# ini/multigrid

Hardware: AMD Instinct MI355X
Metric: agent-steps/sec (higher is better)
Workload: dtype u8

## Files before the change

### include/mgx.h

```cpp
#ifndef MGX_H
#define MGX_H

#if !defined(__HIPCC_RTC__)
#include <stddef.h>
#include <stdint.h>
#endif

#ifdef __cplusplus
extern "C" {
#endif

#define MGX_ABI_VERSION 11

enum {
    MGX_OK = 0,
    MGX_ERR_INVALID_ARGUMENT = -1,
    MGX_ERR_UNKNOWN_ACTION = -2,
    MGX_ERR_UNSUPPORTED = -3,
    MGX_ERR_LAUNCH = -4
};

enum { MGX_KIND_EMPTY = 0, MGX_KIND_BLOCKEDUNLOCKPICKUP = 1, MGX_KIND_REDBLUEDOORS = 2, MGX_KIND_LOCKEDHALLWAY = 3,
       MGX_KIND_RULES = 4 };

// ... 107 lines not shown
                          uint8_t *obs, uint8_t *dir, double *reward, uint8_t *terminated, uint8_t *truncated,
                          int32_t *err, void *stream);

enum { MGX_GEN_EMPTY_FIXED = 0, MGX_GEN_EMPTY_RANDOM = 1, MGX_GEN_BLOCKEDUNLOCKPICKUP = 2, MGX_GEN_REDBLUEDOORS = 3,
       MGX_GEN_LOCKEDHALLWAY = 4, MGX_GEN_PLAYGROUND = 5 };

typedef struct MgxGenStage {
    MgxCell *grid;
    uint8_t *agents;
    uint8_t *aux;
    uint64_t *words;
    int32_t *tag;
    int32_t phase;
    int32_t lead;
    int32_t external;
    int32_t candidates;
} MgxGenStage;

typedef struct MgxLayoutGen {
    int32_t kind;
    int32_t room_size;
    int32_t start_x, start_y, start_dir;
    int32_t max_hallway_keys;
    int32_t max_keys_per_room;
    const MgxCell *blank;
    uint64_t *gen_state;
    MgxGenStage stage;
} MgxLayoutGen;

int mgx_reset_generate(const MgxSpec *spec, int64_t batch, const MgxLayoutGen *gen, MgxCell *grid, uint8_t *agents,
                       uint64_t *rng, int32_t *step_count, uint8_t *aux, int32_t *episode, uint8_t *was_reset, void *stream);

typedef struct MgxResetSelect {
    const uint8_t  *select;
    const uint64_t *rng_words;
} MgxResetSelect;

int mgx_reset_select(const MgxSpec *spec, int64_t batch, const MgxResetSelect *sel, const MgxAutoReset *pool, MgxCell *grid,
                     uint8_t *agents, uint64_t *rng, int32_t *step_count, uint8_t *aux, void *stream);
int mgx_reset_generate_select(const MgxSpec *spec, int64_t batch, const MgxResetSelect *sel, const MgxLayoutGen *gen, MgxCell *grid,
                              uint8_t *agents, uint64_t *rng, int32_t *step_count, uint8_t *aux, int32_t *episode,
                              uint8_t *was_reset, void *stream);

int mgx_stage_generate(const MgxSpec *spec, int64_t batch, const MgxLayoutGen *gen, const uint64_t *rng, const int32_t *episode,
                       void *stream);

int mgx_step_generate(const MgxSpec *spec, int64_t batch, const MgxLayoutGen *gen, MgxCell *grid, uint8_t *agents,
                      uint64_t *rng, int32_t *step_count, const int8_t *actions, uint8_t *aux,
                      uint8_t *obs, uint8_t *dir, double *reward, uint8_t *terminated, uint8_t *truncated,
                      int32_t *err, int32_t *episode, uint8_t *was_reset, void *stream);

int mgx_gen_obs_one_hot(const MgxSpec *spec, int64_t batch, const MgxCell *grid, const uint8_t *agents,
                        uint8_t *obs_one_hot, uint8_t *dir, void *stream);
int mgx_step_one_hot(const MgxSpec *spec, int64_t batch, const MgxAutoReset *ar, MgxCell *grid, uint8_t *agents,
                     uint64_t *rng, int32_t *step_count, const int8_t *actions, uint8_t *aux,
                     uint8_t *obs_one_hot, uint8_t *dir, double *reward, uint8_t *terminated, uint8_t *truncated,
                     int32_t *err, void *stream);

typedef struct MgxStepArgs {
    MgxCell *grid;
    uint8_t *agents;
    uint64_t *rng;
    int32_t *step_count;
    uint8_t *aux;
    const int8_t *actions;
    const uint8_t *hook_order;
    uint8_t *obs;
    uint8_t *dir;
    double *reward;
    uint8_t *terminated;
    uint8_t *truncated;
    int32_t *err;
    int32_t steps;
    int32_t one_hot;
    const MgxAutoReset *auto_reset;
    const MgxLayoutGen *generate;
    int32_t *episode;
    uint8_t *was_reset;
    int32_t *grid_bad;
} MgxStepArgs;

int mgx_step_ex(const MgxSpec *spec, int64_t batch, const MgxStepArgs *args, void *stream);

int mgx_step_chains(const MgxSpec *spec, int64_t batch, const MgxStepArgs *args, int32_t parts, void *const *streams,
                    void *fork_event);
int mgx_sub_shards(const MgxSpec *spec, int64_t batch, const MgxStepArgs *args, int32_t *parts);

#define MGX_SHAPE_RUNTIME_COMPILED 100
typedef struct MgxShapeKey {
    int32_t width, height, num_agents, envs_per_wavefront, hooks, view_size, dma, stream;
    int32_t kernel_args_bytes;
    int32_t built_in;
    int32_t registered;
} MgxShapeKey;
int mgx_shape_key(const MgxSpec *spec, int64_t batch, MgxShapeKey *key);
int mgx_shape_register(const MgxShapeKey *key, const void *code_object, size_t bytes);

#define MGX_PERSIST_CTRL_WORDS 8
typedef struct MgxPersistent {
    const uint64_t *action_granules;
    uint32_t *done;
    uint32_t *ctrl;
    int32_t max_steps;
    int32_t timeout_ms;
} MgxPersistent;

int mgx_persistent_waves(const MgxSpec *spec, int64_t batch, const MgxStepArgs *args, int32_t *waves);
int mgx_step_persistent(const MgxSpec *spec, int64_t batch, const MgxStepArgs *args, const MgxPersistent *p, void *stream);
int mgx_persistent_post(const MgxSpec *spec, int64_t batch, const int8_t *actions, uint32_t step, uint64_t *action_granules,
                        void *stream);
int mgx_persistent_wait(const uint32_t *done, int32_t waves, uint32_t step, uint32_t *ctrl, int32_t timeout_ms, void *stream);
int mgx_persistent_feed(const MgxSpec *spec, int64_t batch, const int8_t *actions, int32_t steps, const MgxPersistent *p,
                        int32_t waves, uint64_t *trace, void *stream);

int mgx_render_atlas(int32_t tile_size, uint8_t *atlas, void *stream);
int mgx_render(const MgxSpec *spec, int64_t n, const MgxCell *grid, const uint8_t *agents, const uint8_t *obs, const uint8_t *atlas,
               int32_t tile_size, uint8_t *frames, void *stream);

#ifdef __cplusplus
}
#endif
#endif
```

### multigrid_amd/_lib.py

```python
from __future__ import annotations

import ctypes as C
import os

from .spec import MgxSpecC

HERE = os.path.dirname(os.path.abspath(__file__))
PRODUCT_LIB_PATH = os.path.join(HERE, "lib", "libmgx.so")
LIB_PATH = os.environ.get("MGX_LIBMGX") or PRODUCT_LIB_PATH


def is_product_lib() -> bool:
    return os.path.realpath(LIB_PATH) == os.path.realpath(PRODUCT_LIB_PATH)

ABI_VERSION = 11
OK, ERR_INVALID_ARGUMENT, ERR_UNKNOWN_ACTION, ERR_UNSUPPORTED, ERR_LAUNCH = 0, -1, -2, -3, -4

EXPORTS = ("mgx_abi_version", "mgx_error_string", "mgx_last_hip_error", "mgx_gen_obs", "mgx_step",
           "mgx_launch_info", "mgx_one_hot", "mgx_full_obs", "mgx_reset_done", "mgx_rollout", "mgx_step_autoreset",
           "mgx_rollout_autoreset", "mgx_gen_obs_one_hot", "mgx_step_one_hot",
           "mgx_reset_generate", "mgx_step_generate", "mgx_pack_grid", "mgx_unpack_grid",
           "mgx_step_ex", "mgx_step_chains", "mgx_sub_shards",
           "mgx_pack_grid_env", "mgx_check_grid", "mgx_pack_grid8_env", "mgx_unpack_grid8", "mgx_shape_key", "mgx_shape_register", "mgx_stage_generate",
           "mgx_persistent_waves", "mgx_step_persistent", "mgx_persistent_post", "mgx_persistent_wait", "mgx_persistent_feed",
           "mgx_rollout_info", "mgx_render_atlas", "mgx_render", "mgx_reset_select", "mgx_reset_generate_select")


class MgxLaunchInfo(C.Structure):
    _fields_ = [(n, C.c_int32) for n in ("envs_per_wavefront", "envs_per_workgroup", "threads_per_workgroup", "workgroups",
                                          "lds_bytes", "slots_per_group", "fixed_shape")]


class MgxRolloutInfo(C.Structure):
    _fields_ = [(n, C.c_int32) for n in ("envs_per_slice", "slices", "wavefronts", "threads_per_workgroup", "workgroups", "lds_bytes",
                                          "resident_shape")]


class MgxAutoReset(C.Structure):
    _fields_ = [("first_env", C.c_int64), ("pool_size", C.c_int32), ("pool_grid", C.c_void_p),
                ("pool_agents", C.c_void_p), ("pool_aux", C.c_void_p), ("episode", C.c_void_p), ("was_reset", C.c_void_p)]


class MgxResetSelect(C.Structure):
    _fields_ = [("select", C.c_void_p), ("rng_words", C.c_void_p)]


class MgxGenStage(C.Structure):
    _fields_ = [("grid", C.c_void_p), ("agents", C.c_void_p), ("aux", C.c_void_p), ("words", C.c_void_p), ("tag", C.c_void_p),
                ("phase", C.c_int32), ("lead", C.c_int32), ("external", C.c_int32), ("candidates", C.c_int32)]


class MgxLayoutGen(C.Structure):
    _fields_ = [("kind", C.c_int32), ("room_size", C.c_int32), ("start_x", C.c_int32), ("start_y", C.c_int32),
                ("start_dir", C.c_int32), ("max_hallway_keys", C.c_int32), ("max_keys_per_room", C.c_int32),
                ("blank", C.c_void_p), ("gen_state", C.c_void_p), ("stage", MgxGenStage)]


class MgxStepArgs(C.Structure):
    _fields_ = [("grid", C.c_void_p), ("agents", C.c_void_p), ("rng", C.c_void_p), ("step_count", C.c_void_p),
                ("aux", C.c_void_p), ("actions", C.c_void_p), ("hook_order", C.c_void_p),
                ("obs", C.c_void_p), ("dir", C.c_void_p), ("reward", C.c_void_p), ("terminated", C.c_void_p),
                ("truncated", C.c_void_p), ("err", C.c_void_p),
                ("steps", C.c_int32), ("one_hot", C.c_int32),
                ("auto_reset", C.POINTER(MgxAutoReset)), ("generate", C.POINTER(MgxLayoutGen)),
                ("episode", C.c_void_p), ("was_reset", C.c_void_p), ("grid_bad", C.c_void_p)]


class MgxPersistent(C.Structure):
    _fields_ = [("action_granules", C.c_void_p), ("done", C.c_void_p), ("ctrl", C.c_void_p), ("max_steps", C.c_int32),
                ("timeout_ms", C.c_int32)]


PERSIST_CTRL_WORDS = 8

GEN_KINDS = {"empty_fixed": 0, "empty_random": 1, "blockedunlockpickup": 2, "redbluedoors": 3, "lockedhallway": 4, "playground": 5}


class MgxError(RuntimeError):
    def __init__(self, code: int, what: str):
        self.code = code
        super().__init__(f"{what}: {error_string(code)} (code {code}, hip error {lib().mgx_last_hip_error()})")


_lib = None


def lib() -> C.CDLL:
    global _lib
    if _lib is not None:
        return _lib
    if not os.path.exists(LIB_PATH):
        raise ImportError(
            f"{LIB_PATH} is missing: the HIP extension has not been built. Run `python -m multigrid_amd.build` "
            "(or __graft_entry__.build()). multigrid_amd has no CPU fallback.")
    L = C.CDLL(LIB_PATH)
    vp, i64 = C.c_void_p, C.c_int64
    L.mgx_abi_version.restype = C.c_int
    L.mgx_error_string.restype = C.c_char_p
    L.mgx_error_string.argtypes = [C.c_int]
    L.mgx_last_hip_error.restype = C.c_int
    L.mgx_gen_obs.restype = C.c_int
    L.mgx_gen_obs.argtypes = [C.POINTER(MgxSpecC), i64, vp, vp, vp, vp, vp]
    L.mgx_step.restype = C.c_int
    L.mgx_step.argtypes = [C.POINTER(MgxSpecC), i64] + [vp] * 13
    L.mgx_rollout.restype = C.c_int
    L.mgx_rollout.argtypes = [C.POINTER(MgxSpecC), i64, C.c_int32] + [vp] * 13
    L.mgx_step_autoreset.restype = C.c_int
    L.mgx_step_autoreset.argtypes = [C.POINTER(MgxSpecC), i64, C.POINTER(MgxAutoReset)] + [vp] * 13
    L.mgx_rollout_autoreset.restype = C.c_int
    L.mgx_rollout_autoreset.argtypes = [C.POINTER(MgxSpecC), i64, C.c_int32, C.POINTER(MgxAutoReset)] + [vp] * 13
    L.mgx_gen_obs_one_hot.restype = C.c_int
    L.mgx_gen_obs_one_hot.argtypes = [C.POINTER(MgxSpecC), i64, vp, vp, vp, vp, vp]
    L.mgx_step_one_hot.restype = C.c_int
    L.mgx_step_one_hot.argtypes = [C.POINTER(MgxSpecC), i64, C.POINTER(MgxAutoReset)] + [vp] * 13
    L.mgx_one_hot.restype = C.c_int
    L.mgx_one_hot.argtypes = [vp, i64, C.POINTER(C.c_int32), vp, vp]
    L.mgx_full_obs.restype = C.c_int
    L.mgx_full_obs.argtypes = [C.POINTER(MgxSpecC), i64, vp, vp, vp, vp]
    L.mgx_reset_done.restype = C.c_int
    L.mgx_reset_done.argtypes = [C.POINTER(MgxSpecC), i64, i64, C.c_int32] + [vp] * 10
    L.mgx_reset_generate.restype = C.c_int
    L.mgx_reset_generate.argtypes = [C.POINTER(MgxSpecC), i64, C.POINTER(MgxLayoutGen)] + [vp] * 8
    L.mgx_reset_select.restype = C.c_int
    L.mgx_reset_select.argtypes = [C.POINTER(MgxSpecC), i64, C.POINTER(MgxResetSelect), C.POINTER(MgxAutoReset)] + [vp] * 6
    L.mgx_reset_generate_select.restype = C.c_int
    L.mgx_reset_generate_select.argtypes = [C.POINTER(MgxSpecC), i64, C.POINTER(MgxResetSelect), C.POINTER(MgxLayoutGen)] + [vp] * 8
    L.mgx_stage_generate.restype = C.c_int
    L.mgx_stage_generate.argtypes = [C.POINTER(MgxSpecC), i64, C.POINTER(MgxLayoutGen), vp, vp, vp]
    L.mgx_step_generate.restype = C.c_int
    L.mgx_step_generate.argtypes = [C.POINTER(MgxSpecC), i64, C.POINTER(MgxLayoutGen)] + [vp] * 15
    L.mgx_pack_grid.restype = C.c_int
    L.mgx_pack_grid.argtypes = [vp, i64, vp, vp, vp]
    L.mgx_unpack_grid.restype = C.c_int
    L.mgx_unpack_grid.argtypes = [vp, i64, vp, vp]
    L.mgx_pack_grid_env.restype = C.c_int
    L.mgx_pack_grid_env.argtypes = [vp, i64, C.c_int32, C.c_int32, vp, vp, vp]
    L.mgx_pack_grid8_env.restype = C.c_int
    L.mgx_pack_grid8_env.argtypes = [vp, i64, C.c_int32, C.c_int32, vp, vp, vp]
    L.mgx_unpack_grid8.restype = C.c_int
    L.mgx_unpack_grid8.argtypes = [vp, i64, vp, vp]
    L.mgx_check_grid.restype = C.c_int
    L.mgx_check_grid.argtypes = [C.POINTER(MgxSpecC), i64, vp, vp, vp, vp]
    L.mgx_launch_info.restype = C.c_int
    L.mgx_launch_info.argtypes = [C.POINTER(MgxSpecC), i64, C.POINTER(MgxLaunchInfo)]
    L.mgx_step_ex.restype = C.c_int
    L.mgx_step_ex.argtypes = [C.POINTER(MgxSpecC), i64, C.POINTER(MgxStepArgs), vp]
    L.mgx_step_chains.restype = C.c_int
    L.mgx_step_chains.argtypes = [C.POINTER(MgxSpecC), i64, C.POINTER(MgxStepArgs), C.c_int32, C.POINTER(vp), vp]
    L.mgx_sub_shards.restype = C.c_int
    L.mgx_sub_shards.argtypes = [C.POINTER(MgxSpecC), i64, C.POINTER(MgxStepArgs), C.POINTER(C.c_int32)]
    L.mgx_persistent_waves.restype = C.c_int
    L.mgx_persistent_waves.argtypes = [C.POINTER(MgxSpecC), i64, C.POINTER(MgxStepArgs), C.POINTER(C.c_int32)]
    L.mgx_step_persistent.restype = C.c_int
    L.mgx_step_persistent.argtypes = [C.POINTER(MgxSpecC), i64, C.POINTER(MgxStepArgs), C.POINTER(MgxPersistent), vp]
    L.mgx_persistent_post.restype = C.c_int
    L.mgx_persistent_post.argtypes = [C.POINTER(MgxSpecC), i64, vp, C.c_uint32, vp, vp]
    L.mgx_persistent_wait.restype = C.c_int
    L.mgx_persistent_wait.argtypes = [vp, C.c_int32, C.c_uint32, vp, C.c_int32, vp]
    L.mgx_persistent_feed.restype = C.c_int
    L.mgx_persistent_feed.argtypes = [C.POINTER(MgxSpecC), i64, vp, C.c_int32, C.POINTER(MgxPersistent), C.c_int32, vp, vp]
    L.mgx_render_atlas.restype = C.c_int
    L.mgx_render_atlas.argtypes = [C.c_int32, vp, vp]
    L.mgx_render.restype = C.c_int
    L.mgx_render.argtypes = [C.POINTER(MgxSpecC), i64, vp, vp, vp, vp, C.c_int32, vp, vp]
    if L.mgx_abi_version() != ABI_VERSION:
        raise ImportError(f"{LIB_PATH}: ABI version {L.mgx_abi_version()} != {ABI_VERSION}; rebuild it")
    _lib = L
    return L


def error_string(code: int) -> str:
    return lib().mgx_error_string(code).decode()


def check(code: int, what: str):
    if code != OK:
        raise MgxError(code, what)


def launch_info(spec, batch: int, roll: bool = False, persistent: bool = False) -> dict:
    sc = spec.to_c()
    if roll or persistent:
        ri = MgxRolloutInfo()
        L = lib()
        L.mgx_rollout_info.restype = C.c_int
        L.mgx_rollout_info.argtypes = [C.POINTER(MgxSpecC), C.c_int64, C.c_int32, C.POINTER(MgxRolloutInfo)]
        check(L.mgx_rollout_info(C.byref(sc), batch, int(bool(persistent)), C.byref(ri)), "mgx_rollout_info")
        out = {n: getattr(ri, n) for n, _ in MgxRolloutInfo._fields_}
        out["envs_per_wavefront"] = ri.envs_per_slice * ri.slices
        return out
    info = MgxLaunchInfo()
    check(lib().mgx_launch_info(C.byref(sc), batch, C.byref(info)), "mgx_launch_info")
    return {n: getattr(info, n) for n, _ in MgxLaunchInfo._fields_}
```

### multigrid_amd/batched.py

```python
from __future__ import annotations

import os

import numpy as np
import torch

from . import _lib, layouts, rng as rnglib
from .constants import NO_ACTION, Action, Type
from .spec import EnvSpec

INT32_MAX = 2 ** 31 - 1


class StepGraph:

    def __init__(self, env, graph, sub_shards, keep):
        self.env, self.graph, self.sub_shards = env, graph, sub_shards
        self._version = env._layout_version
        self._keep = keep

    def replay(self):
        if self.env._layout_version != self._version:
            raise RuntimeError("this graph was captured before set_layout_pool() / set_layout_generator() replaced the layout "
                               "tensors it holds pointers to: capture_steps() again")
        self.graph.replay()


class PersistentSession:

    def __init__(self, env, max_steps: int, auto_reset: bool, timeout_ms: int):
        be = env.backend
        if not hasattr(be, "persistent_launch"):
            raise RuntimeError("persistent stepping needs the HIP backend")
        if auto_reset and getattr(env, "_gen", None) is not None:
            raise RuntimeError("persistent stepping restarts finished envs from a layout pool (set_layout_pool), not from the "
                               "device generator")
        self.env, self.max_steps, self.timeout_ms = env, int(max_steps), int(timeout_ms)
        self.auto_reset = bool(auto_reset)
        B, A, dev = env.batch, env.spec.num_agents, env.device
        self.waves = be.persistent_waves(B, self.auto_reset)
        self.granules = torch.zeros((B, (A + 3) // 4), dtype=torch.int64, device=dev)
        self.done = torch.zeros((self.waves,), dtype=torch.int32, device=dev)
        self.ctrl = torch.tensor([0, 0, 0, -1] + [0] * 4, dtype=torch.int32, device=dev)
        self.stream = torch.cuda.Stream(dev, priority=-1)
        self.t = 0
        self.waited = 0
        self.open = False
        ar = env._auto_reset_args(self.auto_reset, getattr(env, "was_reset", None))
        self._sa, self._keep = be.step_args(env.cells, env.agents, env.rng, env.step_count,
                                            env.aux if env.spec.env_kind != "empty" else None, env.err, env.obs, env.dir,
                                            env.reward, env.terminated, env.truncated, auto_reset=ar)
        self._pers = be.persistent_struct(self.granules, self.done, self.ctrl, self.max_steps, self.timeout_ms)

    def __enter__(self):
        env = self.env
        env._need_state()
        env.join()
        if env._session is not None:
            raise RuntimeError("this env already has a persistent session open")
        cur = torch.cuda.current_stream(env.device)
        self.stream.wait_stream(cur)
        env.backend.persistent_launch(env.batch, self._sa, self._pers, self.stream.cuda_stream)
        env._session = self
        self.open = True
        return self

    def post(self, actions: torch.Tensor):
        env = self.env
        if not self.open or self.t >= self.max_steps:
            raise RuntimeError("the persistent session is closed or has used up its max_steps")
        if actions.dtype is not torch.int8 or actions.shape != env._act_shape or actions.device != env.cells.device \
                or not actions.is_contiguous():
            raise ValueError(f"actions must be a contiguous int8 tensor of shape {tuple(env._act_shape)} on {env.cells.device}")
        self.t += 1
        env.backend.persistent_post(env.batch, actions, self.t, self.granules)

    def wait(self):
        self.env.backend.persistent_wait(self.done, self.waves, self.t, self.ctrl, self.timeout_ms)
        self.waited = self.t
        env = self.env
        return env.obs, env.dir, env.reward, env.terminated, env.truncated

    def step(self, actions: torch.Tensor):
        self.post(actions)
        return self.wait()

    def feed(self, actions: torch.Tensor, trace: bool = False):
        env = self.env
        T = int(actions.shape[0])
        if self.t != 0 or T != self.max_steps:
            raise RuntimeError("feed() plays a whole session: max_steps == len(actions), nothing posted before")
        if actions.dtype is not torch.int8 or tuple(actions.shape[1:]) != tuple(env._act_shape) or not actions.is_contiguous():
            raise ValueError("actions must be a contiguous int8 tensor [T,B,A]")
        tr = torch.zeros((2 * T + 1,), dtype=torch.int64, device=env.device) if trace else None
        env.backend.persistent_feed(env.batch, actions, T, self._pers, self.waves, tr, torch.cuda.current_stream(env.device).cuda_stream)
        self.t = self.waited = T
        return tr

    def close(self):
        if not self.open:
            return
        env = self.env
        cur = torch.cuda.current_stream(env.device)
        if self.t < self.max_steps:
            if self.waited < self.t:
                self.wait()
            self.ctrl[0:1].fill_(1)
        cur.wait_stream(self.stream)
        self.open = False
        env._session = None
        c = [int(v) & 0xFFFFFFFF for v in self.ctrl.cpu()]
        self.timeouts, self.waves_left, self.steps_completed = c[1], c[2], c[3]
        if c[1]:
            raise RuntimeError(f"persistent stepping: {c[1]} wait(s) timed out after {self.timeout_ms} ms "
                               f"(steps completed by every wavefront: {c[3]})")

    def __exit__(self, *exc):
        try:
            self.close()
        except RuntimeError:
            if exc[0] is None:
                raise
        return False

    def __del__(self):
        try:
            if getattr(self, "open", False):
                self.ctrl[0:1].fill_(1)
        except Exception:
            pass


class BatchedMultiGridEnv:
    def __init__(self, spec: EnvSpec, batch: int, device="cuda", *, first_env: int = 0, backend=None, specialise=None):
        self.spec = spec
        self.batch = int(batch)
        self.first_env = int(first_env)
        self.device = torch.device(device)
        if backend is None:
            from .ops import HipBackend
            backend = HipBackend(spec, self.device)
        self.backend = backend
        B, A, dev = self.batch, spec.num_agents, self.device
        self.cells = torch.zeros(spec.cells_shape(B), dtype=torch.uint8 if spec.cell_bytes != 2 else torch.int16, device=dev)
        self.agents = torch.zeros(spec.agents_shape(B), dtype=torch.uint8, device=dev)
        self.rng = torch.zeros((B, 4), dtype=torch.int64, device=dev)
        self.step_count = torch.zeros((B,), dtype=torch.int32, device=dev)
        self.aux = torch.zeros((B, 16), dtype=torch.uint8, device=dev)
        obs_shape = tuple(spec.obs_shape(B))
        parts = (("reward", torch.float64, (B, A)), ("obs", torch.uint8, obs_shape), ("dir", torch.uint8, (B, A)),
                 ("terminated", torch.uint8, (B, A)), ("truncated", torch.uint8, (B,)), ("err", torch.int32, (2,)))
        offs, total = {}, 0
        for name, dt, shape in parts:
            offs[name] = total
            total += (int(np.prod(shape)) * torch.empty((), dtype=dt).element_size() + 15) & ~15
        self._out = torch.zeros(max(total, 16), dtype=torch.uint8, device=dev)
        self._out_parts, self._out_host = [(n, dt, sh, offs[n]) for n, dt, sh in parts], None
        for name, dt, shape in parts:
            nbytes = int(np.prod(shape)) * torch.empty((), dtype=dt).element_size()
            setattr(self, name, self._out[offs[name]:offs[name] + nbytes].view(dt).view(shape))
        self.err.copy_(torch.tensor([0, INT32_MAX], dtype=torch.int32))
        self._loaded = False
        self._seeded = False
        self._act_shape = torch.Size((B, A))
        self._bound = {}
        self._layout_version = 0
        self._parent = None
        self._chain_streams = []
        self._chains_pending, self._chains_P = False, 1
        self._session = None
        self.shape_kernel = None
        if specialise is None:
            specialise = os.environ.get("MGX_JIT", "0") not in ("", "0")
        if specialise and self.device.type == "cuda" and getattr(self.backend, "name", "") == "hip":
            self.specialise()

    def specialise(self) -> str:
        from . import jit
        self.shape_kernel = jit.ensure_shape(self.spec, self.batch, self.device)
        return self.shape_kernel

    @property
    def grid(self) -> torch.Tensor:
        if self.spec.cell_bytes == 3:
            return self.cells
        c = self.cells.to(torch.int32)
        if self.spec.cell_bytes == 1:
            tc = c & 0xF
            door = (tc == 11) | (tc == 12)
            t = torch.where(tc <= 10, tc, torch.where(door, torch.full_like(tc, 4), torch.full_like(tc, 10)))
            st = torch.where(tc <= 10, torch.zeros_like(tc), torch.where(door, tc - 10, tc - 12))
            return torch.stack((t, (c >> 4) & 0x7, st), dim=-1).to(torch.uint8)
        content = ((c >> 4) & 0xF) | (((c >> 11) & 1) << 4) | (((c >> 14) & 1) << 5)
        return torch.stack((c & 0xF, (c >> 8) & 0x7, ((c >> 12) & 0x3) | (content << 2)), dim=-1).to(torch.uint8)

    def load_state(self, grid, agents, rng=None, aux=None, step_count=None, validate: bool = True, target=None):
        self._no_session("load_state")
        sp, B = self.spec, self.batch

        def prep(x, shape, dtype):
            t = torch.as_tensor(np.asarray(x) if not torch.is_tensor(x) else x)
            if t.dim() == len(shape) - 1:
                t = t.unsqueeze(0).expand(shape)
            if tuple(t.shape) != tuple(shape):
                raise ValueError(f"expected shape {tuple(shape)}, got {tuple(t.shape)}")
            return t.to(dtype=dtype).contiguous()

        self.join()
        g = prep(grid, sp.grid_shape(B), torch.uint8)
        a = prep(agents, sp.agents_shape(B), torch.uint8)
        if validate:
            layouts.check_walled(g.cpu().numpy() if g.device.type != "cpu" else g.numpy())
            an = a.cpu().numpy()
            if (an[..., 2] >= sp.width).any() or (an[..., 3] >= sp.height).any() or (an[..., 1] > 3).any():
                raise ValueError("agent position / direction out of range")
        self._refuse_carried_contents(a)
        self.cells.copy_(torch.from_numpy(layouts.pack_cells_for(sp, g.cpu().numpy())))
        self.agents.copy_(a)
        if rng is not None:
            r = np.asarray(rng.cpu() if torch.is_tensor(rng) else rng)
            if r.dtype == np.uint64:
                r = r.view(np.int64)
            self.rng.copy_(prep(r, (B, 4), torch.int64))
            self._seeded = True
        if aux is None and target is not None:
            t = np.zeros(np.asarray(target).shape[:-1] + (16,), dtype=np.uint8)
            t[..., :min(4, np.asarray(target).shape[-1])] = np.asarray(target)[..., :4]
            aux = t
        if aux is not None:
            self.aux.copy_(prep(aux, (B, 16), torch.uint8))
        elif self.spec.env_kind != "empty":
            raise ValueError(f"env_kind {self.spec.env_kind!r} needs `aux` (the env's hook state, include/mgx.h)")
        if step_count is None:
            self.step_count.zero_()
        else:
            self.step_count.copy_(prep(step_count, (B,), torch.int32))
        self._reset_err()
        self._state_written()
        self._loaded = True

    def _refuse_carried_contents(self, agent_rows):
        if self.spec.cell_bytes == 1:
            rows = agent_rows.cpu().numpy() if torch.is_tensor(agent_rows) else np.asarray(agent_rows)
            if (rows[..., 7] >> 2).any():
                raise ValueError("compact cells (cell_bytes = 1) cannot hold a box's content: an agent carries a filled box; "
                                 "use cell_bytes = 2 for envs with Box(contains=...)")

    def seed(self, seed: int):
        self._no_session("seed")
        self.join()
        idx = self.first_env + np.arange(self.batch)
        self.rng.copy_(torch.from_numpy(rnglib.words_from_seed_and_index(seed, idx).view(np.int64)))
        self._seeded = True
        self._state_written()

    def seed_synthetic(self, seed: int):
        self._no_session("seed_synthetic")
        self.join()
        words = rnglib.synthetic_words(self.batch, seed, self.first_env)
        self.rng.copy_(torch.from_numpy(words.view(np.int64)))
        self._seeded = True
        self._state_written()

    def _reset_err(self):
        self.err.copy_(torch.tensor([0, INT32_MAX], dtype=torch.int32))

    def _state_written(self):
        st = (getattr(self, "_gen", None) or {}).get("stage")
        if st is not None and st.get("candidates"):
            st["tag"].fill_(-1)
        elif st is not None:
            st["tag"][:, 0] = -1
            st["tag"][:, 3] = 0

    def gen_obs(self, one_hot: bool = False):
        self._need_state()
        self.join()
        if one_hot:
            if self.spec.cell_bytes == 1:
                self.backend.gen_obs(self.batch, self.cells, self.agents, self.obs, self.dir)
                self.backend.one_hot(self.obs, self._one_hot_buffer())
                return self._one_hot, self.dir
            self._need_wide_cells("one-hot output")
            self.backend.gen_obs(self.batch, self.cells, self.agents, self._one_hot_buffer(), self.dir, one_hot=True)
            return self._one_hot, self.dir
        self.backend.gen_obs(self.batch, self.cells, self.agents, self.obs, self.dir)
        return self.obs, self.dir

    def _one_hot_buffer(self):
        if getattr(self, "_one_hot", None) is None:
            self._one_hot = torch.zeros(tuple(self.obs.shape[:-1]) + (21,), dtype=torch.uint8, device=self.device)
        return self._one_hot

    def _auto_reset_args(self, auto_reset, was_reset):
        if not auto_reset:
            return None
        if getattr(self, "_pool", None) is None:
            raise RuntimeError("auto_reset needs set_layout_pool() first")
        return (self.first_env, self._pool, self.episode, was_reset)

    def step(self, actions: torch.Tensor, auto_reset: bool = False, one_hot: bool = False, hook_order=None, sub_shards=1):
        if not self._loaded or self._session is not None:
            self._need_state()
        if self._parent is not None:
            self._check_fresh()
        if actions.dtype is not torch.int8 or actions.shape != self._act_shape or actions.device != self.cells.device \
                or not actions.is_contiguous():
            raise ValueError(f"actions must be a contiguous int8 tensor of shape {tuple(self._act_shape)} "
                             f"on {self.cells.device}")
        if sub_shards == 1 and hook_order is None and not self._chains_pending:
            fast = self._bound.get((auto_reset, one_hot))
            if fast is not None:
                fast[0](actions)
                return fast[1]
        if hook_order is not None and (hook_order.dtype is not torch.uint8 or hook_order.shape != self._act_shape
                                       or hook_order.device != self.cells.device or not hook_order.is_contiguous()):
            raise ValueError(f"hook_order must be a contiguous uint8 tensor of shape {tuple(self._act_shape)} on {self.cells.device}")
        if one_hot and not (self.spec.cell_bytes == 1 and self.spec.env_kind == "empty"):
            self._need_wide_cells("one-hot output")
        generate = bool(auto_reset) and getattr(self, "_gen", None) is not None
        if generate:
            auto_reset = False
        P = 1
        if sub_shards != 1:
            P = self.sub_shards_hint(auto_reset or generate, one_hot, form="eager") if sub_shards == "auto" else int(sub_shards)
            P = max(1, min(P, self.batch // self.SUB_SHARD_ALIGN))
        if self._chains_pending and P != self._chains_P:
            self.join()
        key = (bool(auto_reset), bool(one_hot), generate, P)
        if one_hot:
            self._one_hot_buffer()
        fast = self._bound.get(key)
        if fast is None:
            fast = self._bind_step(*key)
        out = (self._one_hot if one_hot else self.obs), self.dir, self.reward, self.terminated, self.truncated
        if fast is not False:
            if P > 1:
                ev = self._fork_event
                ev.record(torch.cuda.current_stream(self.device))
                fast(actions, ev.cuda_event, hook_order)
                for st in self._chain_streams[:P]:
                    actions.record_stream(st)
                    if hook_order is not None:
                        hook_order.record_stream(st)
                self._chains_pending, self._chains_P = True, P
                return out
            if isinstance(auto_reset, bool) and isinstance(one_hot, bool):
                self._bound[(auto_reset or generate, one_hot)] = (fast, out)
            fast(actions, hook_order)
            return out
        sp = self.spec
        ar = self._auto_reset_args(auto_reset, getattr(self, "was_reset", None))
        kw = {}
        if ar is not None:
            kw["auto_reset"] = ar
        if one_hot:
            kw["one_hot"] = True
        if hook_order is not None:
            kw["hook_order"] = hook_order
        obs = self._one_hot_buffer() if one_hot else self.obs
        self.backend.step(self.batch, self.cells, self.agents, self.rng, self.step_count, actions,
                          self.aux if sp.env_kind != "empty" else None, self.err,
                          obs, self.dir, self.reward, self.terminated, self.truncated, **kw)
        if generate:
            self.reset_done()
        return obs, self.dir, self.reward, self.terminated, self.truncated

    def join(self):
        if self._chains_pending:
            cur = torch.cuda.current_stream(self.device)
            for st in self._chain_streams:
                cur.wait_stream(st)
            self._chains_pending = False

    def sub_shards_hint(self, auto_reset: bool = False, one_hot: bool = False, form: str = "graph") -> int:
        if form not in ("graph", "eager"):
            raise ValueError("form must be 'graph' or 'eager'")
        if form == "eager":
            return 1
        hint = getattr(self.backend, "sub_shards", None)
        if hint is None:
            return 1
        generate = bool(auto_reset) and getattr(self, "_gen", None) is not None
        return hint(self.batch, bool(auto_reset), bool(one_hot), generate)

    def _bind_step(self, auto_reset: bool, one_hot: bool, generate: bool = False, parts: int = 1):
        key = (auto_reset, one_hot, generate, parts)
        bind = getattr(self.backend, "bind_step" if parts == 1 else "bind_chains", None)
        if bind is None:
            self._bound[key] = False
            return False
        ar = self._auto_reset_args(auto_reset, getattr(self, "was_reset", None))
        head = (self.batch,)
        if parts > 1:
            while len(self._chain_streams) < parts:
                self._chain_streams.append(torch.cuda.Stream(self.device))
            if getattr(self, "_fork_event", None) is None:
                self._fork_event = torch.cuda.Event()
                self._fork_event.record(torch.cuda.current_stream(self.device))
            head = (self.batch, parts, self._chain_streams[:parts])
        f = bind(*head, self.cells, self.agents, self.rng, self.step_count,
                 self.aux if self.spec.env_kind != "empty" else None, self.err,
                 self._one_hot_buffer() if one_hot else self.obs, self.dir, self.reward, self.terminated, self.truncated,
                 auto_reset=ar, one_hot=one_hot,
                 **({"generate": (self._gen, self.episode, self.was_reset)} if generate else {}))
        self._bound[key] = f
        return f

    def _check_fresh(self):
        if self._parent is not None and self._parent._layout_version != self._made_version:
            raise RuntimeError("this sub-shard was split off before its parent's set_layout_pool() / set_layout_generator() "
                               "replaced the layout tensors: split() / capture_steps() again")

    SUB_SHARD_ALIGN = 64

    def split(self, parts: int) -> list:
        self._need_state()
        self.join()
        B, al = self.batch, self.SUB_SHARD_ALIGN
        parts = max(1, min(int(parts), max(1, B // al)))
        cuts = [0] + [min(B, ((B * i // parts + al - 1) // al) * al) for i in range(1, parts)] + [B]
        out = []
        for lo, hi in zip(cuts[:-1], cuts[1:]):
            if hi <= lo:
                continue
            c = object.__new__(BatchedMultiGridEnv)
            c.spec, c.batch, c.first_env, c.device, c.backend = self.spec, hi - lo, self.first_env + lo, self.device, self.backend
            for name in ("cells", "agents", "rng", "step_count", "aux", "obs", "dir", "reward", "terminated", "truncated"):
                setattr(c, name, getattr(self, name)[lo:hi])
            c.err = self.err
            c._loaded, c._act_shape, c._bound = True, torch.Size((hi - lo, self.spec.num_agents)), {}
            c._parent, c._made_version, c._layout_version = self, self._layout_version, 0
            c._chain_streams, c._chains_pending, c._chains_P, c._session = [], False, 1, None
            c._seeded = self._seeded
            c._one_hot = self._one_hot[lo:hi] if getattr(self, "_one_hot", None) is not None else None
            c._pool = getattr(self, "_pool", None)
            c._gen = None
            if getattr(self, "_gen", None) is not None:
                c._gen = dict(self._gen, gen_state=self._gen["gen_state"][lo:hi])
                if self._gen.get("stage") is not None:
                    st = self._gen["stage"]
                    c._gen["stage"] = {k: (v[lo:hi] if torch.is_tensor(v) else v) for k, v in st.items()}
                    if st.get("external") and st.get("stream") is not None:
                        c._gen["stage"]["stream"] = torch.cuda.Stream(self.device)
                    c._gen["stage"]["phase"] = [st["phase"][0]]
            if getattr(self, "episode", None) is not None:
                c.episode, c.was_reset = self.episode[lo:hi], self.was_reset[lo:hi]
            c._range = (lo, hi)
            out.append(c)
        return out

    def capture_steps(self, actions: torch.Tensor, auto_reset: bool = False, one_hot: bool = False, sub_shards=1,
                      hook_order=None):
        self._need_state()
        self.join()
        if sub_shards == "auto":
            sub_shards = self.sub_shards_hint(auto_reset, one_hot)
        stream = torch.cuda.current_stream(self.device)
        graph = torch.cuda.CUDAGraph()
        side = torch.cuda.Stream(self.device)
        side.wait_stream(stream)
        if one_hot:
            self._one_hot_buffer()
        shards = self.split(sub_shards) if sub_shards > 1 else [self]
        others = [torch.cuda.Stream(self.device) for _ in shards[1:]]
        with torch.cuda.stream(side):
            with torch.cuda.graph(graph, stream=side):
                for s in others:
                    s.wait_stream(side)
                for i, sh in enumerate(shards):
                    lo, hi = getattr(sh, "_range", (0, self.batch))
                    with torch.cuda.stream(side if i == 0 else others[i - 1]):
                        st = (getattr(sh, "_gen", None) or {}).get("stage") if auto_reset else None
                        before = st.get("launches", 0) if st else 0
                        for t in range(actions.shape[0]):
                            ho = None if hook_order is None else (hook_order[t] if sh is self else hook_order[t, lo:hi])
                            sh.step(actions[t] if sh is self else actions[t, lo:hi], auto_reset=auto_reset, one_hot=one_hot,
                                    hook_order=ho)
                        if st and st.get("candidates") and st.get("launches", 0) == before:
                            sh.backend.stage_generate(sh.batch, sh._gen, sh.rng, sh.episode)
                for i, sh in enumerate(shards):
                    gs = ((getattr(sh, "_gen", None) or {}).get("stage") or {}).get("stream")
                    if gs is not None:
                        (side if i == 0 else others[i - 1]).wait_stream(gs)
                for s in others:
                    side.wait_stream(s)
        stream.wait_stream(side)
        return StepGraph(self, graph, len(shards), (shards, others, actions, hook_order))

    def rollout(self, actions: torch.Tensor, out: dict | None = None, auto_reset: bool = False, one_hot: bool = False) -> dict:
        self._need_state()
        generate = bool(auto_reset) and getattr(self, "_gen", None) is not None
        if not (self.spec.cell_bytes == 1 and self.spec.env_kind == "empty" and not one_hot and not generate):
            self._need_wide_cells("rollout (the steps of one launch)")
        self.join()
        sp, B = self.spec, self.batch
        if actions.dtype != torch.int8 or actions.dim() != 3 or tuple(actions.shape[1:]) != (B, sp.num_agents) \
                or actions.device != self.cells.device or not actions.is_contiguous():
            raise ValueError(f"actions must be a contiguous int8 tensor of shape (T, {B}, {sp.num_agents}) on {self.cells.device}")
        T, A, v, dev = actions.shape[0], sp.num_agents, sp.view_size, self.device
        if out is None:
            out = {"obs": torch.empty((T, B, A, v, v, 21 if one_hot else 3), dtype=torch.uint8, device=dev),
                   "dir": torch.empty((T, B, A), dtype=torch.uint8, device=dev),
                   "reward": torch.empty((T, B, A), dtype=torch.float64, device=dev),
                   "terminated": torch.empty((T, B, A), dtype=torch.uint8, device=dev),
                   "truncated": torch.empty((T, B), dtype=torch.uint8, device=dev)}
        if auto_reset and "was_reset" not in out:
            out["was_reset"] = torch.empty((T, B), dtype=torch.uint8, device=dev)
        generate = bool(auto_reset) and getattr(self, "_gen", None) is not None
        if generate:
            self.backend.rollout(B, T, self.cells, self.agents, self.rng, self.step_count, actions,
                                 self.aux if sp.env_kind != "empty" else None, self.err, out["obs"], out["dir"],
                                 out["reward"], out["terminated"], out["truncated"],
                                 generate=(self._gen, self.episode, out["was_reset"]), **({"one_hot": True} if one_hot else {}))
            return out
        ar = self._auto_reset_args(auto_reset, out.get("was_reset"))
        self.backend.rollout(B, T, self.cells, self.agents, self.rng, self.step_count, actions,
                             self.aux if sp.env_kind != "empty" else None, self.err, out["obs"], out["dir"],
                             out["reward"], out["terminated"], out["truncated"],
                             **({"auto_reset": ar} if ar is not None else {}), **({"one_hot": True} if one_hot else {}))
        return out

    def one_hot_obs(self) -> torch.Tensor:
        self.join()
        self.backend.one_hot(self.obs, self._one_hot_buffer())
        return self._one_hot

    def full_obs(self) -> torch.Tensor:
        self._need_state()
        self.join()
        if getattr(self, "_full", None) is None:
            self._full = torch.zeros((self.batch, self.spec.width, self.spec.height, 3), dtype=torch.uint8,
                                     device=self.device)
        try:
            self.backend.full_obs(self.batch, self.cells, self.agents, self._full)
        except _lib.MgxError as e:
            if e.code != _lib.ERR_UNSUPPORTED:
                raise
            img = self.grid.permute(0, 2, 1, 3) & torch.tensor([255, 255, 3], dtype=torch.uint8, device=self.device)
            ag = self.agents.long()
            env = torch.arange(self.batch, device=self.device)
            for a in range(self.spec.num_agents):
                img[env, ag[:, a, 2], ag[:, a, 3]] = torch.stack(
                    (torch.full_like(ag[:, a, 0], int(Type.agent)), ag[:, a, 0], ag[:, a, 1]), dim=-1).to(torch.uint8)
            self._full.copy_(img)
        return self._full

    def render(self, env_ids=None, tile_size: int = 32, highlight: bool = True, out: torch.Tensor | None = None) -> torch.Tensor:
        self._no_session("render")
        self._need_state()
        self.join()
        ts = int(tile_size)
        if not 1 <= ts <= 64:
            raise ValueError(f"render: tile_size must be in 1..64, got {tile_size}")
        cells, agents = self.cells, self.agents
        if env_ids is not None:
            ids = torch.as_tensor(env_ids)
            if ids.dtype.is_floating_point or ids.dtype.is_complex or ids.dtype == torch.bool:
                raise TypeError(f"render: env_ids must be an integer tensor, got {ids.dtype}")
            if ids.dim() != 1:
                raise ValueError(f"render: env_ids must be one-dimensional, got shape {tuple(ids.shape)}")
            if ids.numel():
                lo, hi = (int(v) for v in torch.stack((ids.min(), ids.max())).tolist())
                if lo < 0 or hi >= self.batch:
                    raise ValueError(f"render: env_ids must lie in [0, {self.batch}), got {lo}..{hi}")
            ids = ids.to(device=self.device, dtype=torch.long)
            cells, agents = cells.index_select(0, ids), agents.index_select(0, ids)
        n, sp = cells.shape[0], self.spec
        shape = (n, sp.height * ts, sp.width * ts, 3)
        if out is None:
            out = torch.empty(shape, dtype=torch.uint8, device=self.device)
        elif (tuple(out.shape) != shape or out.dtype != torch.uint8 or out.device != self.device or not out.is_contiguous()):
            raise ValueError(f"render: out must be a contiguous uint8 tensor of shape {shape} on {self.device}")
        if n == 0:
            return out
        obs = None
        if highlight:
            scratch = getattr(self, "_render_scratch", None)
            if scratch is None or scratch[0].shape[0] < n:
                scratch = (torch.empty((n,) + tuple(self.obs.shape[1:]), dtype=torch.uint8, device=self.device),
                           torch.empty((n, sp.num_agents), dtype=torch.uint8, device=self.device))
                self._render_scratch = scratch
            obs, dirs = scratch[0][:n], scratch[1][:n]
            self.backend.gen_obs(n, cells, agents, obs, dirs)
        self.backend.render(n, cells, agents, obs, ts, out)
        return out

    def set_layout_pool(self, grids, agents, auxs=None):
        self._no_session("set_layout_pool")
        sp = self.spec
        g = torch.as_tensor(np.asarray(grids), dtype=torch.uint8)
        a = torch.as_tensor(np.asarray(agents), dtype=torch.uint8)
        K = g.shape[0]
        if tuple(g.shape) != (K, sp.height, sp.width, 3) or tuple(a.shape) != (K, sp.num_agents, 8) or K < 1:
            raise ValueError("layout pool has the wrong shape")
        layouts.check_walled(g.numpy())
        self._refuse_carried_contents(a)
        t = None
        if auxs is not None:
            t = torch.as_tensor(np.asarray(auxs), dtype=torch.uint8)
            if tuple(t.shape) != (K, 16):
                raise ValueError("layout pool aux must be u8[K,16]")
            t = t.to(self.device).contiguous()
        elif sp.env_kind != "empty":
            raise ValueError(f"env_kind {sp.env_kind!r} needs per-layout aux")
        self.join()
        cells = torch.from_numpy(layouts.pack_cells_for(sp, g.numpy()))
        old = getattr(self, "_pool", None)
        if (getattr(self, "_gen", None) is None and old is not None and old[0].shape == cells.shape and old[1].shape == a.shape
                and (old[2] is None) == (t is None)):
            old[0].copy_(cells); old[1].copy_(a)
            if t is not None:
                old[2].copy_(t)
            self.episode.zero_(); self.was_reset.zero_()
            return
        self._gen = None
        self._pool = (cells.to(self.device).contiguous(), a.to(self.device).contiguous(), t)
        self.episode = torch.zeros((self.batch,), dtype=torch.int32, device=self.device)
        self.was_reset = torch.zeros((self.batch,), dtype=torch.uint8, device=self.device)
        self._bound.clear()
        self._layout_version += 1

    def set_layout_generator(self, kind: str, layout_seed: int = 0, *, room_size: int = 0, start=(1, 1, 0),
                             max_hallway_keys: int = 1, max_keys_per_room: int = 2, staged=True, lead: int | None = None):
        self._no_session("set_layout_generator")
        sp = self.spec
        self._need_wide_cells("set_layout_generator (device-side episode generation)")
        if kind == "blockedunlockpickup":
            if sp.env_kind != "blockedunlockpickup" or (sp.width, sp.height) != (2 * room_size - 1, room_size):
                raise ValueError("blockedunlockpickup generator: the spec must be a BlockedUnlockPickup grid of (2*room_size-1) x room_size")
            blank = layouts.roomgrid_blank(room_size, 1, 2)
        elif kind == "redbluedoors":
            if sp.env_kind != "redbluedoors" or sp.width != 2 * sp.height:
                raise ValueError("redbluedoors generator: the spec must be a RedBlueDoors grid of (2*size) x size")
            blank = layouts.redbluedoors_blank(sp.height)
        elif kind == "lockedhallway":
            rs = int(room_size)
            if sp.env_kind != "lockedhallway" or rs < 4 or sp.width != 3 * (rs - 1) + 1 or (sp.height - 1) % (rs - 1):
                raise ValueError("lockedhallway generator: the spec must be 3 columns of `room_size` rooms")
            blank = layouts.lockedhallway_blank(2 * ((sp.height - 1) // (rs - 1)), rs)
        elif kind == "playground":
            rs = int(room_size)
            if sp.env_kind != "empty" or rs < 4 or (sp.width - 1) % (rs - 1) or (sp.height - 1) % (rs - 1):
                raise ValueError("playground generator: the spec must be a hook-free grid of `room_size` rooms")
            blank = layouts.roomgrid_blank(rs, (sp.height - 1) // (rs - 1), (sp.width - 1) // (rs - 1))
        elif kind in ("empty_fixed", "empty_random"):
            if sp.env_kind != "empty" or sp.width != sp.height:
                raise ValueError("empty generator: the spec must be a square Empty grid")
            blank = layouts.empty_blank(sp.width)
        else:
            raise ValueError(f"unknown layout generator {kind!r}")
        self.join()
        idx = self.first_env + np.arange(self.batch)
        self._gen = {"kind": kind, "room_size": int(room_size), "start": tuple(int(v) for v in start),
                     "max_hallway_keys": int(max_hallway_keys), "max_keys_per_room": int(max_keys_per_room),
                     "blank": torch.from_numpy(layouts.pack_cells(blank).view(np.int16)).to(self.device).contiguous(),
                     "gen_state": torch.from_numpy(rnglib.layout_gen_state(layout_seed, idx).view(np.int64)).to(self.device)}
        cand = {"blockedunlockpickup": int(room_size) - 2, "redbluedoors": 1, "lockedhallway": 1, "empty_fixed": 1,
                "empty_random": 1}.get(kind, 0)
        if staged is True:
            staged = "candidates" if 1 <= cand <= 4 else "between"
        if staged not in (False, "candidates", "between", "side", "in_launch"):
            raise ValueError(f"staged must be True / 'candidates' / 'between' / 'side' / 'in_launch' / False, got {staged!r}")
        if staged == "candidates" and not 1 <= cand <= 4:
            raise ValueError(f"staged='candidates': the {kind!r} generator draws from env.np_random more than once (or has more than "
                             f"4 possible draws): use 'between'")
        if staged == "candidates" and sp.num_agents > 1:
            B, dev = self.batch, self.device
            lead = int(lead) if lead is not None else max(4, min(512, 2 * sp.max_steps // 3))
            lead = max(2, min(lead, sp.max_steps - 1))
            self._gen["stage"] = {"lead": lead, "external": 2, "stream": None, "candidates": cand,
                                  "grid": torch.zeros((B, cand, sp.height, sp.width), dtype=torch.int16, device=dev),
                                  "agents": torch.zeros((B, cand, sp.num_agents, 8), dtype=torch.uint8, device=dev),
                                  "aux": torch.zeros((B, cand, 16), dtype=torch.uint8, device=dev) if sp.env_kind != "empty" else None,
                                  "words": torch.zeros((B, cand, 6), dtype=torch.int64, device=dev),
                                  "tag": torch.full((B, 4), -1, dtype=torch.int32, device=dev), "phase": [0]}
        elif staged and sp.num_agents > 1:
            B, dev = self.batch, self.device
            tag = torch.zeros((B, 4), dtype=torch.int32, device=dev)
            tag[:, 0] = -1
            side = staged in ("side", "between")
            lead = int(lead) if lead is not None else (max(2, min(128, sp.max_steps // 4)) if side else 2)
            if not 2 <= lead < sp.max_steps or (side and lead < 4):
                side, lead, staged = False, 2, "in_launch"
            self._gen["stage"] = {"lead": lead, "external": (2 if staged == "between" else 1) if side else 0, "stream": torch.cuda.Stream(dev) if side and staged == "side" and dev.type == "cuda" else None,
                                  "grid": torch.zeros((B, sp.height, sp.width), dtype=torch.int16, device=dev),
                                  "agents": torch.zeros((B, sp.num_agents, 8), dtype=torch.uint8, device=dev),
                                  "aux": torch.zeros((B, 16), dtype=torch.uint8, device=dev) if sp.env_kind != "empty" else None,
                                  "words": torch.zeros((B, 12), dtype=torch.int64, device=dev), "tag": tag, "phase": [0]}
        self._pool = None
        self.episode = torch.zeros((self.batch,), dtype=torch.int32, device=self.device)
        self.was_reset = torch.zeros((self.batch,), dtype=torch.uint8, device=self.device)
        self._bound.clear()
        self._layout_version += 1

    def reset_done(self) -> torch.Tensor:
        self._need_state()
        self.join()
        if getattr(self, "_gen", None) is not None:
            self.backend.reset_generate(self.batch, self._gen, self.cells, self.agents, self.rng, self.step_count,
                                        self.aux if self.spec.env_kind != "empty" else None, self.episode, self.was_reset)
            return self.was_reset
        if getattr(self, "_pool", None) is None:
            raise RuntimeError("call set_layout_pool() or set_layout_generator() first")
        self.backend.reset_done(self.batch, self.first_env, self._pool, self.cells, self.agents, self.step_count,
                                self.aux, self.episode, self.was_reset)
        return self.was_reset

    def reset(self, seed: int | None = None, mask: torch.Tensor | None = None, one_hot: bool = False):
        self._no_session("reset")
        gen, pool = getattr(self, "_gen", None), getattr(self, "_pool", None)
        if gen is None and pool is None:
            raise RuntimeError("call set_layout_pool() or set_layout_generator() first")
        sel = None
        if mask is not None:
            self._need_state()
            if not torch.is_tensor(mask) or mask.dtype not in (torch.bool, torch.uint8) or tuple(mask.shape) != (self.batch,) \
                    or mask.device != self.cells.device or not mask.is_contiguous():
                raise ValueError(f"mask must be a contiguous bool or uint8 tensor of shape ({self.batch},) on {self.cells.device}")
            sel = mask.view(torch.uint8) if mask.dtype is torch.bool else mask
        if seed is None and not self._loaded and not self._seeded:
            raise ValueError("reset(): np_random has never been seeded (all-zero PCG64 words are not a generator): pass seed=, or "
                             "call seed() / seed_synthetic() first")
        self.join()
        words = None
        if seed is not None:
            idx = self.first_env + np.arange(self.batch)
            words = torch.from_numpy(rnglib.words_from_seed_and_index(int(seed), idx).view(np.int64)).to(self.device)
        aux = self.aux if self.spec.env_kind != "empty" else None
        if gen is not None:
            side = (gen.get("stage") or {}).get("stream")
            if side is not None:
                torch.cuda.current_stream(self.device).wait_stream(side)
            self.backend.reset_generate_select(self.batch, gen, sel, words, self.cells, self.agents, self.rng, self.step_count,
                                               aux, self.episode, self.was_reset)
        else:
            self.backend.reset_select(self.batch, self.first_env, pool, sel, words, self.cells, self.agents, self.rng,
                                      self.step_count, self.aux, self.episode, self.was_reset)
        if seed is not None:
            self._seeded = True
        self._loaded = True
        return self.gen_obs(one_hot)

    def outputs_to_host(self) -> dict:
        self.join()
        if self._out.device.type == "cpu":
            host = self._out
        else:
            if self._out_host is None:
                self._out_host = torch.empty(self._out.shape, dtype=torch.uint8, pin_memory=True)
            self._out_host.copy_(self._out, non_blocking=True)
            torch.cuda.current_stream(self.device).synchronize()
            host = self._out_host
        arr = host.numpy()
        out = {}
        for name, dt, shape, off in self._out_parts:
            npdt = {torch.float64: np.float64, torch.uint8: np.uint8, torch.int32: np.int32}[dt]
            n = int(np.prod(shape)) * np.dtype(npdt).itemsize
            out[name] = arr[off:off + n].view(npdt).reshape(shape)
        return out

    def check_errors(self):
        self.join()
        gb = getattr(self.backend, "_grid_bad", None)
        if gb is not None:
            unpackable, ring = (int(v) for v in gb.cpu())
            if unpackable or ring:
                gb.zero_()
                raise ValueError(f"the byte grid held {ring} outer-ring cell(s) that are not WALL = (wall, grey, 0) and {unpackable} "
                                 f"cell value(s) the packed format cannot hold (include/mgx.h)")
        count, first = (int(v) for v in self.err.cpu())
        if count:
            self._reset_err()
            raise ValueError(f"Unknown action in {count} env(s); first at local env {first} "
                             f"(valid: {int(Action.left)}..{int(Action.done)}, or {NO_ACTION} for no action)")

    def is_done(self) -> torch.Tensor:
        self._no_session("is_done")
        truncated = self.step_count >= self.spec.max_steps
        return truncated | (self.agents[:, :, 4] != 0).all(dim=1)

    def _no_session(self, what: str):
        if self._session is not None:
            raise RuntimeError(f"{what}: a persistent session is open -- the env state lives in its launch until it is closed")

    def _need_wide_cells(self, what: str):
        if self.spec.compact:
            raise NotImplementedError(f"{what} is not available on compact cells / byte grids (EnvSpec.cell_bytes = 1 or 3: step / "
                                      f"gen_obs / auto-reset from a layout pool / full_obs); build the env with cell_bytes = 2 for it")

    def _need_state(self):
        if not self._loaded:
            raise RuntimeError("no state loaded: call load_state() / reset() first")
        if self._session is not None:
            raise RuntimeError("a persistent session is open: the env state lives in its launch until it is closed")

    def persistent(self, max_steps: int, auto_reset: bool = False, timeout_ms: int = 2000) -> "PersistentSession":
        if not (self.spec.cell_bytes == 1 and self.spec.env_kind == "empty"):
            self._need_wide_cells("persistent stepping")
        return PersistentSession(self, max_steps, auto_reset, timeout_ms)

    def state_dict(self) -> dict:
        self._no_session("state_dict")
        self.join()
        sd = {"spec": self.spec.as_dict(), "first_env": self.first_env,
              "grid": self.grid.cpu().clone(), "agents": self.agents.cpu().clone(),
              "rng": self.rng.cpu().clone(), "step_count": self.step_count.cpu().clone(),
              "aux": self.aux.cpu().clone()}
        if getattr(self, "_gen", None) is not None:
            sd["generator"] = {"kind": self._gen["kind"], "room_size": self._gen["room_size"], "start": self._gen["start"],
                               "max_hallway_keys": self._gen["max_hallway_keys"], "max_keys_per_room": self._gen["max_keys_per_room"],
                               "gen_state": self._gen["gen_state"].cpu().clone()}
            sd["episode"] = self.episode.cpu().clone()
            sd["was_reset"] = self.was_reset.cpu().clone()
        if getattr(self, "_pool", None) is not None:
            pg, pa, pt = self._pool
            sd["pool"] = {"grid": torch.from_numpy(layouts.unpack_cells_for(self.spec, pg.cpu().numpy())), "agents": pa.cpu().clone(),
                          "aux": pt.cpu().clone() if pt is not None else None}
            sd["episode"] = self.episode.cpu().clone()
            sd["was_reset"] = self.was_reset.cpu().clone()
        return sd
# ... 22 lines not shown
```

### multigrid_amd/csrc/mgx_fused.h

```cpp
#pragma once
#if !defined(__HIPCC_RTC__)
#include <hip/hip_runtime.h>
#include <limits.h>
#include <stdint.h>
#else
namespace __hip_internal {}
using namespace __hip_internal;
typedef unsigned long uintptr_t;
#ifndef offsetof
#define offsetof(t, m) __builtin_offsetof(t, m)
#endif
#ifndef INT_MAX
#define INT_MAX 2147483647
#endif
#ifndef INT64_MAX
#define INT64_MAX 9223372036854775807LL
#endif
#endif

#include "mgx_rules.h"
#include "mgx_layout_gen.h"

namespace mgx_fused {

using namespace mgx;

constexpr int kMaxThreads = 256;

struct KernelArgs {
    MgxSpec sp;
    int64_t batch;
    uint8_t *grid;
    uint8_t *agents;
    uint64_t *rng;
    int32_t *step_count;
    const int8_t *actions;
    const uint8_t *hook_order;
    uint8_t *aux;
    uint8_t *obs;
    uint8_t *dir;
    double *reward;
    uint8_t *terminated;
    uint8_t *truncated;
    int32_t *err;
    int32_t Gw;
    int32_t dbg;
    int32_t flags;
    int32_t T;
    int32_t wave_lds;
    int32_t vpw;
    int32_t grp;
    int32_t inv_A;
    int32_t ns;
    int32_t rshape;
    int32_t pool_size;
    int64_t first_env;
    uint64_t pool_magic;
    const uint8_t *pool_grid;
    const uint8_t *pool_agents;
    const uint8_t *pool_aux;
    int32_t *episode;
    uint8_t *was_reset;
    MgxLayoutGen gen;
    int64_t gen_first_wg;
    const uint64_t *granules;
    uint32_t *done;
    uint32_t *pctrl;
    uint32_t timeout_ticks;
    int32_t *grid_bad;
    int32_t *bounds;
    int32_t span_base;
};

#ifndef MGX_DEBUG_KNOBS
#define MGX_DEBUG_KNOBS 0
#endif
#if MGX_DEBUG_KNOBS
#define MGX_DBG(bits) (a.dbg & (bits))
#else
#define MGX_DBG(bits) 0
#endif

#ifndef MGX_BOUNDS_CHECK
#define MGX_BOUNDS_CHECK 0
#endif
#if MGX_BOUNDS_CHECK
#define MGX_CHECK_LDS_ADDR(site, addr, bytes)                                                              \
    do {                                                                                                   \
        const uint32_t a_ = (uint32_t)(addr), lo_ = (uint32_t)(wave * a.wave_lds);                         \
        if (a_ < lo_ || a_ + (uint32_t)(bytes) > lo_ + (uint32_t)a.wave_lds) {                             \
            atomicAdd(a.bounds, 1); a.bounds[1] = (site);                                                  \
        }                                                                                                  \
    } while (0)
#define MGX_CHECK_LDS_PTR(site, ptr, bytes) MGX_CHECK_LDS_ADDR(site, (uint32_t)(uintptr_t)(lds_u32_ptr)(const void *)(ptr) - (uint32_t)(uintptr_t)(lds_u32_ptr)(const void *)lds, bytes)
#else
#define MGX_CHECK_LDS_ADDR(site, addr, bytes) ((void)0)
#define MGX_CHECK_LDS_PTR(site, ptr, bytes) ((void)0)
#endif

template <typename T>
__device__ __forceinline__ T kernarg_at(size_t offset) {
    typedef const char __attribute__((address_space(4))) *cptr;
    typedef const T __attribute__((address_space(4))) *tptr;
    return *(tptr)((cptr)__builtin_amdgcn_kernarg_segment_ptr() + offset);
}
#define MGX_LATE(field) kernarg_at<decltype(KernelArgs::field)>(offsetof(KernelArgs, field))

#define MGX_RARE_PATH_PRIO() __builtin_amdgcn_s_setprio(3)

struct alignas(16) ViewRec { int32_t origin; uint32_t steps, lo, hi; };

typedef const uint32_t __attribute__((address_space(3))) *lds_u32_ptr;
typedef const uint16_t __attribute__((address_space(3))) *lds_u16_ptr;
typedef const int8_t __attribute__((address_space(3))) *lds_i8_ptr;
typedef uint32_t __attribute__((aligned(1))) u32_unaligned;
typedef const u32_unaligned __attribute__((address_space(3))) *lds_u32_ua_ptr;

#ifndef MGX_NO_BIG_PERSIST
#define MGX_NO_BIG_PERSIST 0
#endif
#ifndef MGX_NO_FIXED_SHAPES
#define MGX_NO_FIXED_SHAPES 0
#endif
constexpr int kSlotsSmallView = 64;
constexpr int kInAux = 0;
constexpr int kObsAux = 2;
constexpr int kOhAux = 0;
constexpr int kSmallOutAux = 2;
constexpr int kRound = 16;

inline int slots_per_wave(int view_size, bool narrow = false) { return (view_size <= 7 && !narrow) ? kSlotsSmallView : 32; }
constexpr int kSlotsLatency = 32;

constexpr int kLutBytes = 256 * 4;
struct LdsCarve {
    int vpw, nw, Gw, A, tile_bytes, round_bytes;
    bool roll;
    bool has_aux;
    bool c8;
    int ns = 1;
    bool sliced = false;
    __host__ __device__ __attribute__((always_inline)) int tile_pad() const { return (tile_bytes & 15) ? 32 : 0; }
    __host__ __device__ __attribute__((always_inline)) int sh_end() const { return 22 * vpw + 32 * A + 16; }
    __host__ __device__ __attribute__((always_inline)) int pstride() const {
        return 8 * vpw + 32 * Gw + ((4 * Gw + 15) & ~15) + (has_aux ? 16 * Gw : 0) + tile_bytes + tile_pad();
    }
    __host__ __device__ __attribute__((always_inline)) int pers(int s) const { return sh_end() + s * pstride(); }
    __host__ __device__ __attribute__((always_inline)) int rows(int s = 0) const { return sliced ? pers(s) : 0; }
    __host__ __device__ __attribute__((always_inline)) int rec() const { return sliced ? 0 : 8 * vpw; }
    __host__ __device__ __attribute__((always_inline)) int rnd() const { return rec(); }
    __host__ __device__ __attribute__((always_inline)) int rew() const { return rec() + 8 * vpw; }
    __host__ __device__ __attribute__((always_inline)) int woff() const { return rec() + 16 * vpw; }
    __host__ __device__ __attribute__((always_inline)) int temps_end() const { return woff() + 4 * vpw; }
    __host__ __device__ __attribute__((always_inline)) int act() const { return temps_end(); }
// ... 673 lines not shown
```

### multigrid_amd/csrc/mgx_fused_body.inc

```
    constexpr bool DO_STEP = MODE != 0;
    const int env_kind = HOOKS ? a.sp.env_kind : (int)MGX_KIND_EMPTY;
    constexpr bool PERSIST = MODE == 3;
    constexpr bool ROLL = MODE == 2 || PERSIST;
    constexpr int kOutAux = PERSIST ? 16 : kSmallOutAux;
#define MGX_PUB_STORE_U8(base, idx, n, val)                                                                            \
    do {                                                                                                               \
        if constexpr (PERSIST) __builtin_amdgcn_raw_buffer_store_b8((uint8_t)(val), make_rsrc((base), (n)), (idx), 0, 16); \
        else (base)[idx] = (uint8_t)(val);                                                                           \
    } while (0)
    constexpr int V2 = V * V;
    constexpr int NW = (V2 + 63) / 64;
    constexpr int CB = C8 ? 1 : kCellBytes;
    static_assert(!C8 || (!GEN && !DMA && (MODE < 2 ? (!OH || (MODE == 1 && !HOOKS)) : (!OH && !HOOKS))),
                  "compact cells: the plain step / gen_obs kernels, the step with one-hot output, the hook-free rollout / persistent kernels");
    static_assert(SHAPE == 0 || kShapes[SHAPE].cb == CB, "shape table entry of the other cell format");
    static_assert(!B3 || (!C8 && !OH && !GEN && !DMA && MODE < 2 && SHAPE == 0), "byte grids: the plain step / gen_obs kernels only");
    constexpr int CBG = B3 ? 3 : CB;
    constexpr bool RSHAPE = SHAPE != 0 && kShapes[SHAPE].ns > 0;
    constexpr int NS = RSHAPE ? kShapes[SHAPE].ns : 1;
    constexpr int PITCH = RSHAPE ? kShapes[SHAPE].pitch : 0;
    constexpr bool SLICED = RSHAPE && shape_sliced(kShapes[SHAPE]);
    static_assert(!RSHAPE || ((MODE == 2 || MODE == 3) && !OH && !GEN && !STREAM && !DMA && !C8 && !B3 && V <= 7), "resident shapes: rollout / persistent kernels");
    static_assert(NS <= 2, "slices: the (step, slice) sequence below is written for one or two");
    constexpr bool HALF = !DMA && (MODE == 1 || RSHAPE) && !C8;
    constexpr bool PK3 = kPack3<V>;
    constexpr bool LINES = view_line_lanes(V, ROLL, OH, C8, GRP);
    constexpr int kG = GRP, kR = SLICED ? kRoundResident : GRP;
    constexpr int kG4 = kR < kG ? kR : kG;
    constexpr int VPW = (DMA && GRP < kGroup) ? GRP : ((V <= 7 && HALF) ? kSlotsSmallView : 32);
    extern __shared__ __align__(16) uint8_t lds[];

    int lane_ = threadIdx.x & 63;
#define lane lane_

    const int wave = __builtin_amdgcn_readfirstlane(threadIdx.x >> 6);
    if constexpr (V <= 7) {
        const int64_t e_batch = a.batch;
        const uint8_t *e_grid = a.grid, *e_agents = a.agents, *e_aux = a.aux, *e_hord = a.hook_order;
        const uint64_t *e_rng = a.rng;
        const int32_t *e_sc = a.step_count;
        const int8_t *e_act = a.actions;
        const unsigned e_bd = blockDim.x;
        const int32_t *e_ep = (AR || GEN) ? a.episode : nullptr;
        const uint8_t *e_trunc = DO_STEP ? a.truncated : nullptr;
        const uint64_t *e_gs = GEN ? a.gen.gen_state : nullptr;
        const int32_t *e_tag = GEN ? a.gen.stage.tag : nullptr;
        asm volatile("" :: "s"(e_batch), "s"(e_grid), "s"(e_agents), "s"(e_rng), "s"(e_sc), "s"(e_act), "s"(e_hord), "s"(e_aux),
                     "s"(e_bd), "s"(e_ep), "s"(e_trunc), "s"(e_gs), "s"(e_tag));
    }
    constexpr bool FIXED = SHAPE != 0;
    constexpr bool PREFIX = FIXED ? (kShapes[SHAPE].A > 4) : (V > 7 && MODE == 1);
    constexpr bool BIGCOPY = FIXED ? (kShapes[SHAPE].W * kShapes[SHAPE].H * CB >= 4096) : (V > 7 && MODE == 1);
    const int W = FIXED ? kShapes[SHAPE].W : a.sp.width, H = FIXED ? kShapes[SHAPE].H : a.sp.height,
              A = FIXED ? kShapes[SHAPE].A : a.sp.num_agents;
    const int Gw_ = FIXED ? kShapes[SHAPE].Gw : a.Gw;
    const int vpw_ = FIXED ? shape_slots(kShapes[SHAPE]) : a.vpw;
    const int inv_A_ = FIXED ? (65536 + kShapes[SHAPE].A - 1) / (FIXED ? kShapes[SHAPE].A : 1) : a.inv_A;
    const int HWB = H * W * CB;
    const int HWG = H * W * CBG;
#define MGX_LATE_GEN(f) kernarg_at<decltype(MgxLayoutGen::f)>(offsetof(KernelArgs, gen) + offsetof(MgxLayoutGen, f))
#define MGX_LATE_STAGE(f) kernarg_at<decltype(MgxGenStage::f)>(offsetof(KernelArgs, gen) + offsetof(MgxLayoutGen, stage) + offsetof(MgxGenStage, f))
    if constexpr (GEN && MODE == 1) {
        if ((int64_t)blockIdx.x >= a.gen_first_wg) {
            const int64_t gw = ((int64_t)blockIdx.x - a.gen_first_wg) * (blockDim.x >> 6) + wave;
            const int64_t b = gw * 64 + lane;
            int32_t *const tag = MGX_LATE_STAGE(tag);
            const int32_t phase1 = MGX_LATE_STAGE(phase) + 1;
            const bool serial = MGX_LATE_STAGE(external) == 2;
            int32_t req = b >= a.batch ? 0 : serial ? tag[b * 4 + 3]
                                                    : __hip_atomic_load(tag + b * 4 + 3, __ATOMIC_ACQUIRE, __HIP_MEMORY_SCOPE_AGENT);
            if (req != 0 && req != phase1 && tag[b * 4 + 1] != a.episode[b]) { tag[b * 4 + 3] = 0; req = 0; }
            const bool go = req != 0 && req != phase1;
            const uint64_t gom = __builtin_amdgcn_ballot_w64(go);
#if MGX_SPANS
            const int64_t wid_g = a.gen_first_wg * (blockDim.x >> 6) + gw;
            const unsigned long long t_g0 = __builtin_amdgcn_s_memrealtime();
            if (gom == 0 && lane == 0 && a.span_base + wid_g < kSpanCap) {
                g_span[2 * (a.span_base + wid_g)] = t_g0;
                g_span[2 * (a.span_base + wid_g) + 1] = __builtin_amdgcn_s_memrealtime() & 0x0fffffffffffffffull;
            }
#endif
            if (gom == 0) return;
            MGX_RARE_PATH_PRIO();
            MgxLayoutGen gen;
            gen.kind = MGX_LATE_GEN(kind); gen.room_size = MGX_LATE_GEN(room_size);
            gen.start_x = MGX_LATE_GEN(start_x); gen.start_y = MGX_LATE_GEN(start_y); gen.start_dir = MGX_LATE_GEN(start_dir);
            gen.max_hallway_keys = MGX_LATE_GEN(max_hallway_keys); gen.max_keys_per_room = MGX_LATE_GEN(max_keys_per_room);
            gen.blank = MGX_LATE_GEN(blank); gen.gen_state = MGX_LATE_GEN(gen_state);
            uint8_t *const st_grid = reinterpret_cast<uint8_t *>(MGX_LATE_STAGE(grid));
            mgx_gen::copy_blank(gen, st_grid, gw * 64, HWB, gom, lane);
            __builtin_amdgcn_fence(__ATOMIC_RELEASE, "wavefront");
            __builtin_amdgcn_s_waitcnt(0x0F70);
            wave_sync();
            if (go) {
                const int32_t ep_s = tag[b * 4 + 1], sc_s = tag[b * 4 + 2];
                uint64_t *const words = MGX_LATE_STAGE(words) + b * 12;
                const uint64_t *gs = gen.gen_state + b * 6, *rg = a.rng + b * 4;
                mgx_gen::NpGen lay, npr;
                for (int k = 0; k < 4; ++k) lay.s[k] = gs[k];
                lay.buf = gs[4]; npr.buf = gs[5];
                uint64_t s0 = words[10], s1 = words[11];
                const uint64_t i0 = rg[2], i1 = rg[3];
                const uint64_t jA[4] = {kJump.w[A][0], kJump.w[A][1], kJump.w[A][2], kJump.w[A][3]};
                if (A > 1 && a.sp.max_steps > sc_s) pcg64_advance(s0, s1, i0, i1, jA, (uint32_t)(a.sp.max_steps - sc_s));
                npr.s[0] = s0; npr.s[1] = s1; npr.s[2] = i0; npr.s[3] = i1;
                uint8_t *apos = lds + wave * a.wave_lds + lane * (2 * A);
                const uint4 naux = mgx_gen::generate_episode(gen, W, H, A, lay, npr, apos, st_grid + b * HWB,
                                                             reinterpret_cast<uint64_t *>(MGX_LATE_STAGE(agents)) + b * A);
                uint8_t *const st_aux = MGX_LATE_STAGE(aux);
                if (st_aux) reinterpret_cast<uint4 *>(st_aux)[b] = naux;
                for (int k = 0; k < 4; ++k) { words[k] = lay.s[k]; words[6 + k] = npr.s[k]; }
                words[4] = lay.buf; words[5] = npr.buf;
                if (serial) {
                    tag[b * 4 + 3] = 0;
                    tag[b * 4] = ep_s;
                } else {
                    const bool same = __hip_atomic_load(tag + b * 4 + 3, __ATOMIC_ACQUIRE, __HIP_MEMORY_SCOPE_AGENT) == req
                                      && tag[b * 4 + 1] == ep_s && tag[b * 4 + 2] == sc_s;
                    if (same) {
                        tag[b * 4 + 3] = 0;
                        __builtin_amdgcn_fence(__ATOMIC_RELEASE, "agent");
                        __hip_atomic_store(tag + b * 4, ep_s, __ATOMIC_RELEASE, __HIP_MEMORY_SCOPE_AGENT);
                    }
                }
            }
#if MGX_SPANS
            if (lane == 0 && a.span_base + wid_g < kSpanCap) {
                g_span[2 * (a.span_base + wid_g)] = t_g0;
                g_span[2 * (a.span_base + wid_g) + 1] = (__builtin_amdgcn_s_memrealtime() & 0x0fffffffffffffffull) | (8ull << 60);
            }
#endif
            return;
        }
    }
    const int64_t wid = (int64_t)blockIdx.x * (blockDim.x >> 6) + wave;
    const int64_t e0w = wid * (Gw_ * NS);
    const int64_t e0 = e0w;
    if (e0 >= a.batch) return;
    [[maybe_unused]] const int ns_act = NS > 1 ? (int)min((int64_t)NS, (a.batch - e0w + Gw_ - 1) / Gw_) : 1;
    const int Gc = (int)min((int64_t)Gw_, a.batch - e0);
    const int NVc = Gc * A;
    const int64_t v0 = e0 * A;

#if MGX_TIMESTAMPS
    int stamp_i = 0;
    MGX_MARK("start");
#endif
#if MGX_SPANS
    if (!PERSIST && lane == 0 && a.span_base + wid < kSpanCap) g_span[2 * (a.span_base + wid)] = __builtin_amdgcn_s_memrealtime();
    unsigned long long span_flags = 0;
#define MGX_SPAN_FLAG(bit, cond) do { if (!GEN && (cond)) span_flags |= (unsigned long long)(bit); } while (0)
#define MGX_SPAN_GFLAG(bit, cond) do { if (cond) span_flags |= (unsigned long long)(bit); } while (0)
#else
#define MGX_SPAN_FLAG(bit, cond) ((void)0)
#define MGX_SPAN_GFLAG(bit, cond) ((void)0)
#endif
#if MGX_DEBUG_KNOBS
    if (a.dbg >> 16) {
        const uint32_t hw = __builtin_amdgcn_s_getreg((31 << 11) | 4);
        const int k = ((a.dbg >> 24) & 1) ? (int)(hw & 1u) : (int)(hw & 3u);
        for (int i = 0; i < k * ((a.dbg >> 16) & 0xff); ++i) __builtin_amdgcn_s_sleep(1);
    }
    if (a.dbg & (3 << 25)) {
        const uint32_t hw = __builtin_amdgcn_s_getreg((31 << 11) | 4);
        const uint32_t pr = (a.dbg & (1 << 26)) ? (hw & 3u) : ((hw & 1u) * 2u);
        if (pr == 1) __builtin_amdgcn_s_setprio(1); else if (pr == 2) __builtin_amdgcn_s_setprio(2); else if (pr == 3) __builtin_amdgcn_s_setprio(3);
    }
#endif
    const LdsCarve cv = make_carve(W, H, A, V, Gw_, vpw_, ROLL, HOOKS, OH, kR, CB, NS, SLICED, PITCH);
    const int TSB = PITCH ? PITCH * (H - 1) * CB : HWB;
    const int wave_lds_ = FIXED ? cv.total() : a.wave_lds;
    uint8_t *L = lds + wave * wave_lds_;
    uint64_t *rows = reinterpret_cast<uint64_t *>(L + cv.rows());
    ViewRec *rec = reinterpret_cast<ViewRec *>(L + cv.rec());
    int8_t *acts = reinterpret_cast<int8_t *>(L + cv.act());
    uint64_t *rngs = reinterpret_cast<uint64_t *>(L + cv.rng());
    uint64_t *rnd = reinterpret_cast<uint64_t *>(L + cv.rnd());
    uint8_t *ord = L + cv.ord();
    double *rew = reinterpret_cast<double *>(L + cv.rew());
    int32_t *scnt = reinterpret_cast<int32_t *>(L + cv.scnt());
    uint4 *auxl = reinterpret_cast<uint4 *>(L + cv.aux());
    uint64_t *jump = reinterpret_cast<uint64_t *>(L + cv.jump());

    [[maybe_unused]] int32_t *const stage_tag = (GEN && MODE == 1 && A > 1) ? a.gen.stage.tag : nullptr;
    [[maybe_unused]] const int cand_K = (GEN && MODE == 1 && A > 1 && a.gen.stage.tag) ? a.gen.stage.candidates : 0;
    [[maybe_unused]] uint64_t *const gen_state_p = GEN ? a.gen.gen_state : nullptr;

    MGX_MARK("P0");
    const int64_t g0 = e0 * HWB, g1 = g0 + (int64_t)Gc * HWB;
    const int64_t gtotal = a.batch * (int64_t)HWB;
    const int64_t ga = B3 ? g0 : (g0 & ~(int64_t)15);
    uint8_t *tile_raw = L + cv.tile();
    const int tile_skew = (int)(g0 - ga);
    [[maybe_unused]] uint8_t *tile = tile_raw + tile_skew;
    constexpr int U = 8;
    const uint8_t *gsrc = a.grid + ga;
    const int len = (int)(g1 - ga);
    const int avail = (int)min(gtotal - ga, (int64_t)INT_MAX);
    const int grec = MGX_DBG(1) ? 0 : MGX_DBG(1024) ? min((len / 2 + 15) & ~15, avail) : min((len + 15) & ~15, avail);
    const __amdgpu_buffer_rsrc_t grsrc = make_rsrc(gsrc, grec);
    const int lane16 = 16 * lane;
    const int env_of_lane = (lane * inv_A_) >> 16, agent_of_lane = lane - env_of_lane * A;
    u32x4 in_rngA = {0, 0, 0, 0}, in_rngB = {0, 0, 0, 0};
    u32x4 in_jmpA = {0, 0, 0, 0}, in_jmpB = {0, 0, 0, 0};
    if (DO_STEP && A > 1) {
        const __amdgpu_buffer_rsrc_t rr = make_rsrc(a.rng + e0 * 4, Gc * 32);
        if (ROLL) {
            in_rngA = __builtin_amdgcn_raw_buffer_load_b128(rr, lane16, 0,kInAux);
            for (int t = lane; t < A * 4; t += 64) jump[t] = kJump.w[1][t];
        } else {
            in_rngA = __builtin_amdgcn_raw_buffer_load_b128(rr, env_of_lane * 32, 0,kInAux);
            in_rngB = __builtin_amdgcn_raw_buffer_load_b128(rr, env_of_lane * 32 + 16, 0,kInAux);
            const u32x4 *jk = reinterpret_cast<const u32x4 *>(&kJump.w[1 + agent_of_lane][0]);
            in_jmpA = jk[0]; in_jmpB = jk[1];
        }
    }
    u32x2 in_row = {0, 0};
    uint32_t in_scnt = 0;
    u32x4 in_aux = {0, 0, 0, 0};
    uint8_t in_act = 0;
    [[maybe_unused]] uint8_t in_hord = 0;
    in_row = __builtin_amdgcn_raw_buffer_load_b64(make_rsrc(a.agents + v0 * 8, NVc * 8), lane * 8, 0,kInAux);
    uint32_t in_ep = 0;
    [[maybe_unused]] int32_t in_tag = -1, in_tag_sc = -1;
    [[maybe_unused]] u32x4 in_tags = {0, 0, 0, 0};
    [[maybe_unused]] u32x2 in_nbuf = {0, 0};
    if (DO_STEP) {
        if ((AR || GEN) && !ROLL) in_ep = __builtin_amdgcn_raw_buffer_load_b32(make_rsrc(a.episode + e0, Gc * 4), lane * 4, 0, 0);
        in_scnt = __builtin_amdgcn_raw_buffer_load_b32(make_rsrc(a.step_count + e0, Gc * 4), lane * 4, 0,kInAux);
        if (!PERSIST) in_act = __builtin_amdgcn_raw_buffer_load_b8(make_rsrc(a.actions + v0, NVc), lane, 0,kInAux);
        if (HOOKS && !ROLL && a.hook_order) in_hord = __builtin_amdgcn_raw_buffer_load_b8(make_rsrc(a.hook_order + v0, NVc), lane, 0, 0);
        if (cv.has_aux) in_aux = __builtin_amdgcn_raw_buffer_load_b128(make_rsrc(a.aux + e0 * MGX_AUX_BYTES, Gc * MGX_AUX_BYTES), lane16, 0, 0);
    }
    [[maybe_unused]] u32x4 tv[U], tv2[U];
    const bool big_tile = len > 1024 * U;
    constexpr int kTileAux = STREAM ? 2 : 0;
    typedef __attribute__((address_space(3))) void *lds_void_ptr;
#define MGX_TILE_BURST(dst, base)                                                                                     \
    if constexpr (DMA) {                                                                                              \
        _Pragma("unroll") for (int u = 0; u < U; ++u)                                                                 \
            if (lane16 + (base) + 1024 * u < len)                                                                     \
                __builtin_amdgcn_raw_ptr_buffer_load_lds(grsrc, (lds_void_ptr)(tile_raw + (base) + 1024 * u), 16, lane16, \
                                                         (base) + 1024 * u, 0, kTileAux);                            \
    } else {                                                                                                          \
        _Pragma("unroll") for (int u = 0; u < U; ++u)                                                                 \
            dst[u] = __builtin_amdgcn_raw_buffer_load_b128(grsrc, lane16 + 1024 * (u & 3), (base) + 4096 * (u >> 2), kTileAux); \
    }
    if constexpr (!B3 && PITCH == 0) { MGX_TILE_BURST(tv, 0) }
    typedef uint32_t u32x3 __attribute__((ext_vector_type(3)));
    constexpr int NR3 = 16;
    [[maybe_unused]] u32x3 w3[B3 ? NR3 : 1];
    [[maybe_unused]] const __amdgpu_buffer_rsrc_t brs3 =
        make_rsrc(a.grid + e0 * (int64_t)HWG, !B3 ? 0 : (e0 + Gc == a.batch) ? Gc * HWG : ((Gc * HWG + 3) & ~3));
    if constexpr (B3) {
#pragma unroll
        for (int k = 0; k < NR3; ++k) w3[k] = __builtin_amdgcn_raw_buffer_load_b96(brs3, 3 * (4 * lane + 256 * k), 0, kTileAux);
    }
    uint64_t my_rng[4];
    my_rng[0] = ((uint64_t)in_rngA.y << 32) | in_rngA.x; my_rng[1] = ((uint64_t)in_rngA.w << 32) | in_rngA.z;
    my_rng[2] = ((uint64_t)in_rngB.y << 32) | in_rngB.x; my_rng[3] = ((uint64_t)in_rngB.w << 32) | in_rngB.z;
    uint64_t my_draw = 0;
    [[maybe_unused]] uint64_t post_lo = 0, post_hi = 0;
    if (DO_STEP && !ROLL && A > 1 && !MGX_DBG((2 | 128)) && lane < NVc) {
        uint64_t jk[4];
        jk[0] = ((uint64_t)in_jmpA.y << 32) | in_jmpA.x; jk[1] = ((uint64_t)in_jmpA.w << 32) | in_jmpA.z;
        jk[2] = ((uint64_t)in_jmpB.y << 32) | in_jmpB.x; jk[3] = ((uint64_t)in_jmpB.w << 32) | in_jmpB.z;
        uint64_t s_lo, s_hi;
        my_draw = pcg64_draw_at(my_rng, jk, s_lo, s_hi);
        if (GEN) { post_lo = s_lo; post_hi = s_hi; }
        if (agent_of_lane == A - 1) { uint64_t *dst = a.rng + (e0 + env_of_lane) * 4; dst[0] = s_lo; dst[1] = s_hi; }
    }
    if (big_tile && !B3) {
        MGX_TILE_BURST(tv2, 1024 * U)
    }
#undef MGX_TILE_BURST
    if constexpr (GEN && MODE == 1) {
        const bool on = DO_STEP && stage_tag != nullptr;
        asm volatile("" ::: "memory");
        const u32x4 tg = __builtin_amdgcn_raw_buffer_load_b128(make_rsrc(stage_tag + e0 * 4, on ? Gc * 16 : 0), lane * 16, 0, 0);
        in_nbuf = __builtin_amdgcn_raw_buffer_load_b64(make_rsrc(gen_state_p + e0 * 6, (on && cand_K > 1) ? Gc * 48 : 0), lane * 48 + 40, 0, 0);
        asm volatile("" ::: "memory");
        in_tag = on ? (int32_t)tg.x : -1; in_tag_sc = on ? (int32_t)tg.z : -1;
        in_tags = tg;
    }
    uint64_t reset_mask0 = 0;
    if (AR && DO_STEP && !ROLL) {
        const uint64_t row0 = ((uint64_t)in_row.y << 32) | in_row.x;
        const uint64_t alive = __builtin_amdgcn_ballot_w64(lane < NVc && !row_term(row0));
        bool done = false;
        if (lane < Gc) {
            const uint64_t amask = (A >= 64) ? ~0ull : ((1ull << A) - 1ull);
            done = (((alive >> mad24(lane, A, 0)) & amask) == 0) | ((int32_t)in_scnt >= a.sp.max_steps);
            if (a.was_reset) a.was_reset[e0 + lane] = (uint8_t)done;
        }
        reset_mask0 = __builtin_amdgcn_ballot_w64(done);
    }
    const uint32_t wall_addr = (uint32_t)(wave * wave_lds_ + cv.wall());
    if (lane == 0) *reinterpret_cast<uint32_t *>(L + cv.wall()) = C8 ? CELL8_WALL : CELL16_WALL;
    if constexpr (C8) {
        u32x4 e;
        e.x = cell8_unpack(4u * lane); e.y = cell8_unpack(4u * lane + 1u); e.z = cell8_unpack(4u * lane + 2u); e.w = cell8_unpack(4u * lane + 3u);
        if constexpr (OH) {
            e.x = one_hot_mask21(e.x); e.y = one_hot_mask21(e.y); e.z = one_hot_mask21(e.z); e.w = one_hot_mask21(e.w);
        }
        *reinterpret_cast<u32x4 *>(L + cv.lut() + ((16 * lane + 512) & 1023)) = e;
    }
    if (lane < NVc) {
        if (DO_STEP && !ROLL && A > 1) rnd[lane] = my_draw;
        reinterpret_cast<u32x2 *>(rows)[lane] = in_row;
        rew[lane] = 0.0;
        if (DO_STEP) acts[lane] = (int8_t)in_act;
    }
    if (DO_STEP) {
        if (A > 1 && ROLL && lane < Gc * 2) reinterpret_cast<u32x4 *>(rngs)[lane] = in_rngA;
        if (lane < Gc) { scnt[lane] = (int32_t)in_scnt; if (cv.has_aux) reinterpret_cast<u32x4 *>(auxl)[lane] = in_aux; }
    }
    __builtin_amdgcn_s_waitcnt(0x0F70);
    if constexpr (B3) {
        const int ncell = Gc * H * W;
        const bool tensor_end = e0 + Gc == a.batch;
        int nbad = 0;
        constexpr int NR = NR3;
        for (int c0 = 4 * lane; c0 < ncell; c0 += 256 * NR) {
            if (c0 != 4 * lane) {
#pragma unroll
                for (int k = 0; k < NR; ++k) w3[k] = __builtin_amdgcn_raw_buffer_load_b96(brs3, 3 * (c0 + 256 * k), 0, kTileAux);
            }
            uint32_t cont = 0;
#pragma unroll
            for (int k = 0; k < NR; ++k) {
                if (c0 + 256 * k - 4 * lane >= ncell) break;
                const uint32_t w0 = w3[k].x, w1 = w3[k].y, w2 = w3[k].z;
                const uint32_t T4 = __builtin_amdgcn_perm(w2, __builtin_amdgcn_perm(w1, w0, 0x00060300u), 0x05020100u);
                const uint32_t C4 = __builtin_amdgcn_perm(w2, __builtin_amdgcn_perm(w1, w0, 0x00070401u), 0x06020100u);
                const uint32_t S4 = __builtin_amdgcn_perm(w2, __builtin_amdgcn_perm(w1, w0, 0x00000502u), 0x07040100u);
                auto zero80 = [](const uint32_t x) { return ~(((x & 0x7f7f7f7fu) + 0x7f7f7f7fu) | x | 0x7f7f7f7fu); };
                const uint32_t S3 = S4 & 0x03030303u;
                const uint32_t shut = (S3 + 0x7f7f7f7fu) & 0x80808080u;
                const uint32_t opq = zero80(T4 ^ (0x01010101u * (uint32_t)T_WALL))
                                   | (zero80(T4 ^ (0x01010101u * (uint32_t)T_DOOR)) & shut);
                const uint32_t L4 = T4 & 0x0f0f0f0fu;
                const uint32_t H4 = (C4 & 0x07070707u) | (S3 << 4) | opq;
                nbad += ((T4 & 0xf0f0f0f0u) | (C4 & 0xf8f8f8f8u)) != 0;
                cont |= S4 & 0xfcfcfcfcu;
                const int cc = c0 + 256 * k;
                if (2 * cc < Gc * HWB) {
                    MGX_CHECK_LDS_PTR(1, tile_raw + 2 * cc, 8);
                    *reinterpret_cast<u32x2 *>(tile_raw + 2 * cc) =
                        u32x2{__builtin_amdgcn_perm(H4, L4, 0x05010400u), __builtin_amdgcn_perm(H4, L4, 0x07030602u)};
                }
            }
            if (MGX_ANY_LANE(cont != 0)) {
#pragma unroll
                for (int k = 0; k < NR; ++k) {
                    if (c0 + 256 * k - 4 * lane >= ncell) break;
                    const uint32_t w0 = w3[k].x, w1 = w3[k].y, w2 = w3[k].z;
                    const uint32_t c[4] = {w0 & 0xffffffu, __builtin_amdgcn_alignbyte(w1, w0, 3) & 0xffffffu,
                                           __builtin_amdgcn_alignbyte(w2, w1, 2) & 0xffffffu, w2 >> 8};
                    if (!MGX_ANY_LANE(((c[0] | c[1] | c[2] | c[3]) >> 18) != 0)) continue;
                    uint32_t p[4];
#pragma unroll
                    for (int j = 0; j < 4; ++j) {
                        p[j] = cell_pack(c[j]);
                        nbad += ((c[j] >> 18) != 0) & (((c[j] & 0xffu) != (uint32_t)T_BOX) | (((c[j] >> 18) & 7u) == 0) | ((c[j] >> 21) > 5u));
                    }
                    const int cc = c0 + 256 * k;
                    if (2 * cc < Gc * HWB) *reinterpret_cast<u32x2 *>(tile_raw + 2 * cc) = u32x2{p[0] | (p[1] << 16), p[2] | (p[3] << 16)};
                }
            }
        }
        if (tensor_end && ((Gc * HWG) & 3) != 0 && lane < 2) {
            const int cell = ncell - 1 - lane;
            if (cell >= 0) store_cell16(tile_raw + 2 * cell, cell_pack(load_obs_cell(a.grid + e0 * (int64_t)HWG + 3 * cell)));
        }
        int32_t *const gbad = MGX_LATE(grid_bad);
        if (gbad) {
            wave_sync();
            int nring = 0;
            const int ringN = 2 * W + 2 * (H - 2);
            for (int p = lane; p < ringN; p += 64) {
                const int q = p - 2 * W;
                const int y = p < W ? 0 : (q < 0 ? H - 1 : 1 + (q >> 1));
                const int x = p < W ? p : (q < 0 ? p - W : ((q & 1) ? W - 1 : 0));
                const uint8_t *cp = tile_raw + 2 * (y * W + x);
                int e = 0;
                for (; e + 4 <= Gc; e += 4) {
                    const uint32_t r0 = load_cell16(cp + e * HWB), r1 = load_cell16(cp + (e + 1) * HWB),
                                   r2 = load_cell16(cp + (e + 2) * HWB), r3 = load_cell16(cp + (e + 3) * HWB);
                    nring += (r0 != CELL16_WALL) + (r1 != CELL16_WALL) + (r2 != CELL16_WALL) + (r3 != CELL16_WALL);
                }
                for (; e < Gc; ++e) nring += load_cell16(cp + e * HWB) != CELL16_WALL;
            }
            if (nbad) atomicAdd(gbad, nbad);
            if (nring) atomicAdd(gbad + 1, nring);
        }
    } else
    if constexpr (!DMA && PITCH == 0) {
#pragma unroll
        for (int u = 0; u < U; ++u)
            if (lane16 + 1024 * u < len) {
                MGX_CHECK_LDS_PTR(1, tile_raw + lane16 + 1024 * u, 16);
                *reinterpret_cast<u32x4 *>(tile_raw + lane16 + 1024 * u) = tv[u];
            }
    }
    if (big_tile && !B3) {
        if constexpr (!DMA) {
#pragma unroll
            for (int u = 0; u < U; ++u)
                if (lane16 + 1024 * (U + u) < len) *reinterpret_cast<u32x4 *>(tile_raw + lane16 + 1024 * (U + u)) = tv2[u];
        }
        for (int rel = lane16 + 2048 * U; rel < len; rel += 1024)
            *reinterpret_cast<u32x4 *>(tile_raw + rel) = __builtin_amdgcn_raw_buffer_load_b128(grsrc, rel, 0, kTileAux);
    }
    if (!B3 && g1 == gtotal && (gtotal & 15)) {
        const int64_t t0 = gtotal & ~(int64_t)15;
        for (int k = lane; k < (int)(gtotal & 15); k += 64) tile_raw[(int)(t0 - ga) + k] = a.grid[t0 + k];
    }
    if (GEN && MODE == 1 && cand_K > 0) __builtin_amdgcn_s_waitcnt(0x0F72);
    else __builtin_amdgcn_s_waitcnt(0x0F70);
    wave_sync();

#define MGX_SLICE_VARS(S)                                                                                               \
    [[maybe_unused]] const int64_t e0 = e0w + (int64_t)(S) * Gw_;                                                       \
    [[maybe_unused]] const int Gc = (int)min((int64_t)Gw_, a.batch - e0);                                               \
    [[maybe_unused]] const int NVc = Gc * A;                                                                            \
    [[maybe_unused]] const int64_t v0 = e0 * A;                                                                         \
    [[maybe_unused]] uint64_t *const rows = reinterpret_cast<uint64_t *>(L + cv.rows(S));                               \
    [[maybe_unused]] uint64_t *const rngs = reinterpret_cast<uint64_t *>(L + cv.rng(S));                                \
    [[maybe_unused]] int32_t *const scnt = reinterpret_cast<int32_t *>(L + cv.scnt(S));                                 \
    [[maybe_unused]] uint4 *const auxl = reinterpret_cast<uint4 *>(L + cv.aux(S));                                      \
    [[maybe_unused]] const int64_t g0 = e0 * HWB, g1 = g0 + (int64_t)Gc * HWB;                                          \
    [[maybe_unused]] const int64_t ga = B3 ? g0 : (g0 & ~(int64_t)15);                                                  \
    [[maybe_unused]] uint8_t *const tile_raw = L + cv.tile(S);                                                          \
    [[maybe_unused]] const int tile_skew = (int)(g0 - ga);                                                              \
    [[maybe_unused]] uint8_t *const tile = tile_raw + tile_skew;                                                        \
    [[maybe_unused]] const int len = (int)(g1 - ga);
    [[maybe_unused]] auto load_pitch_tile = [&](uint8_t *const t_raw, const int64_t env0, const int nenv) {
        const uint16_t *src = reinterpret_cast<const uint16_t *>(a.grid + env0 * HWB);
        const int HW = H * W;
        for (int c = lane; c < nenv * HW; c += 64) {
            const int e = c / HW, r = c - e * HW, y = r / W, x = r - y * W;
            reinterpret_cast<uint16_t *>(t_raw)[e * PITCH * (H - 1) + y * PITCH + x] = src[c];
        }
    };
    if constexpr (PITCH != 0) {
        static_assert(PITCH == 0 || (CB == 2 && ROLL), "ring-sharing tiles: 16-bit cells, rollout / persistent kernels");
        load_pitch_tile(tile_raw, e0, Gc);
        wave_sync();
    }
    if constexpr (NS > 1) {
        static_assert(NS == 1 || (kShapes[SHAPE].W * kShapes[SHAPE].H * CB * kShapes[SHAPE].Gw) % 16 == 0, "slices: whole 16-byte vectors per slice");
        for (int s1 = 1; s1 < ns_act; ++s1) {
            MGX_SLICE_VARS(s1)
            if constexpr (PITCH != 0) {
                load_pitch_tile(tile_raw, e0, Gc);
            } else {
                const __amdgpu_buffer_rsrc_t gr1 = make_rsrc(a.grid + g0, Gc * HWB);
                for (int rel = lane16; rel < len; rel += 1024)
                    *reinterpret_cast<u32x4 *>(tile_raw + rel) = __builtin_amdgcn_raw_buffer_load_b128(gr1, rel, 0, 0);
            }
            if (lane < NVc) rows[lane] = reinterpret_cast<const uint64_t *>(a.agents)[v0 + lane];
            if (DO_STEP) {
                if (A > 1 && lane < Gc * 2)
                    reinterpret_cast<u32x4 *>(rngs)[lane] = __builtin_amdgcn_raw_buffer_load_b128(make_rsrc(a.rng + e0 * 4, Gc * 32), lane16, 0, 0);
                if (lane < Gc) {
                    scnt[lane] = a.step_count[e0 + lane];
                    if (cv.has_aux) auxl[lane] = reinterpret_cast<const uint4 *>(a.aux)[e0 + lane];
                }
            }
        }
        wave_sync();
    }

    [[maybe_unused]] int pre_e = -1;
    [[maybe_unused]] uint32_t pre_grid[4] = {0, 0, 0, 0};
    [[maybe_unused]] uint64_t pre_row = 0, pre_word = 0;
    [[maybe_unused]] uint4 pre_aux = {0, 0, 0, 0};
    if constexpr (GEN && MODE == 1) {
        if (stage_tag && cand_K == 0) {
            const int32_t lead0 = MGX_LATE_STAGE(lead);
            const bool will = lane < Gc && in_tag == (int32_t)in_ep && (int32_t)in_scnt + 1 == a.sp.max_steps
                              && in_tag_sc == a.sp.max_steps - lead0;
            const uint64_t pm = __builtin_amdgcn_ballot_w64(will);
            if (pm != 0 && (HWB & 3) == 0 && HWB <= 1024) {
                pre_e = __builtin_ctzll(pm);
                const int64_t b = e0 + pre_e;
// ... 73 lines not shown
    const int64_t tv0 = (PERSIST ? (int64_t)t_out : (int64_t)t * BA) + v0;
    const int64_t tb0 = PERSIST ? (int64_t)t_out : (int64_t)t * a.batch;
    if constexpr (PERSIST) {
        const int gpe = (A + 3) >> 2, ng = Gc * gpe;
        const uint64_t *gr = a.granules + e0 * gpe;
        const uint32_t want = (uint32_t)t + 1u;
        uint64_t g = 0;
        bool leave = false;
        const uint64_t t_wait0 = __builtin_amdgcn_s_memrealtime();
        for (uint32_t spin = 1;; ++spin) {
            if (lane < ng) g = __hip_atomic_load(gr + lane, __ATOMIC_RELAXED, __HIP_MEMORY_SCOPE_AGENT);
            if (__builtin_amdgcn_ballot_w64(lane < ng && (uint32_t)(g >> 32) != want) == 0) break;
            if ((spin & 15u) == 0) {
                const uint32_t stop = __hip_atomic_load(a.pctrl + 0, __ATOMIC_RELAXED, __HIP_MEMORY_SCOPE_AGENT);
                const bool late = __builtin_amdgcn_s_memrealtime() - t_wait0 > (uint64_t)a.timeout_ticks;
                if (__builtin_amdgcn_readfirstlane(stop) != 0 || late) {
                    if (late && lane == 0) atomicAdd(a.pctrl + 1, 1u);
                    leave = true;
                    break;
                }
            }
            __builtin_amdgcn_s_sleep(1);
        }
        if (leave) break;
#if MGX_SPANS
        const int64_t span_rec = a.span_base + (int64_t)t * gridDim.x * (blockDim.x >> 6) + wid;
        if (lane == 0 && span_rec < kSpanCap) g_span[2 * span_rec] = __builtin_amdgcn_s_memrealtime();
#endif
        if (lane < ng) {
            const int e = lane / gpe, q = lane - e * gpe;
#pragma unroll
            for (int j = 0; j < 4; ++j)
                if (4 * q + j < A) acts[e * A + 4 * q + j] = (int8_t)(g >> (8 * j));
        }
        if (lane < NVc) rew[lane] = 0.0;
        wave_sync();
    } else if (ROLL) {
        if (lane < NVc) { acts[lane] = next_act; rew[lane] = 0.0; }
        if constexpr (NS > 1) {
            const bool wrap = sl_s + 1 >= ns_act;
            const int t_n = wrap ? t + 1 : t;
            const int64_t e0_n = e0w + (wrap ? 0 : (int64_t)(sl_s + 1) * Gw_);
            const int NVc_n = (int)min((int64_t)Gw_, a.batch - e0_n) * A;
            if (t_n < T && lane < NVc_n) next_act = a.actions[(int64_t)t_n * BA + e0_n * A + lane];
        } else {
            if (t + 1 < T && lane < NVc) next_act = a.actions[(int64_t)(t + 1) * BA + v0 + lane];
        }
        wave_sync();
    }
    uint32_t ovl_saved = 0;
    int ovl_off = -1;
    uint64_t cur_row = ROLL ? (lane < NVc ? rows[lane] : 0ull) : (((uint64_t)in_row.y << 32) | in_row.x);
    MGX_MARK("AR");
    uint64_t reset_mask = 0;
    if (AR && DO_STEP) {
        if (ROLL) {
            const uint64_t alive = __builtin_amdgcn_ballot_w64(lane < NVc && !row_term(cur_row));
            bool done = false;
            if (lane < Gc) {
                const uint64_t amask = (A >= 64) ? ~0ull : ((1ull << A) - 1ull);
                done = (((alive >> mad24(lane, A, 0)) & amask) == 0) | (scnt[lane] >= cf.max_steps);
                if (a.was_reset) MGX_PUB_STORE_U8(a.was_reset + tb0 + e0, lane, Gc, done);
            }
            reset_mask = __builtin_amdgcn_ballot_w64(done);
        } else {
            reset_mask = reset_mask0;
        }
        MGX_SPAN_FLAG(1, reset_mask != 0);
        if (reset_mask != 0) {
            MGX_RARE_PATH_PRIO();
            int32_t *p_ep = MGX_LATE(episode);
            int32_t my_ep = 0, my_lay = 0;
            if (lane < Gc && ((reset_mask >> lane) & 1ull)) {
                my_ep = ROLL ? p_ep[e0 + lane] : (int32_t)in_ep;
                my_lay = pool_index(MGX_LATE(first_env), e0 + lane, my_ep, MGX_LATE(pool_size), MGX_LATE(pool_magic));
            }
            for (uint64_t m = reset_mask; m != 0; m &= m - 1) {
                const int e = __builtin_ctzll(m);
                const int64_t b = e0 + e;
                const int32_t ep = (int32_t)__builtin_amdgcn_readlane(my_ep, e);
                const int lay = (int)__builtin_amdgcn_readlane(my_lay, e);
                wave_sync();
                if (lane == 0) p_ep[b] = ep + 1;
                const uint8_t *sg = MGX_LATE(pool_grid) + (int64_t)lay * HWG;
                uint8_t *etile = tile + e * TSB;
                uint8_t *gg = MGX_LATE(grid) + b * HWG;
                const uint32_t etile_addr = (uint32_t)(uintptr_t)(lds_u32_ptr)etile;
                const uint64_t *sa = reinterpret_cast<const uint64_t *>(MGX_LATE(pool_agents)) + (int64_t)lay * A;
                const uint64_t nrow = lane < A ? sa[lane] : 0ull;
                uint4 naux = {0, 0, 0, 0};
                if (HOOKS) naux = reinterpret_cast<const uint4 *>(MGX_LATE(pool_aux))[lay];
                if constexpr (PITCH != 0) {
                    for (int i = lane; i < H * W; i += 64) {
                        const int y = i / W, x = i - y * W;
                        reinterpret_cast<uint16_t *>(etile)[y * PITCH + x] = reinterpret_cast<const uint16_t *>(sg)[i];
                    }
                } else
                if constexpr (B3) {
                    if (((HWG | (uint32_t)reinterpret_cast<uintptr_t>(sg) | (uint32_t)reinterpret_cast<uintptr_t>(gg)) & 3u) == 0) {
                        const int nd = HWG / 4;
                        for (int i = lane; i < nd; i += 64) reinterpret_cast<uint32_t *>(gg)[i] = reinterpret_cast<const uint32_t *>(sg)[i];
                    } else {
                        for (int i = lane; i < HWG; i += 64) gg[i] = sg[i];
                    }
                    for (int i = lane; i < H * W; i += 64) store_cell16(etile + 2 * i, cell_pack(load_obs_cell(sg + 3 * i)));
                } else
                if (BIGCOPY && HWB >= 4096 && ((HWB | etile_addr | (uint32_t)reinterpret_cast<uintptr_t>(sg) | (uint32_t)reinterpret_cast<uintptr_t>(gg)) & 15u) == 0) {
                    const int nv = HWB / 16;
                    for (int base = lane; base < nv; base += 256) {
                        uint4 v4[4];
#pragma unroll
                        for (int k = 0; k < 4; ++k)
                            v4[k] = (base + 64 * k < nv) ? reinterpret_cast<const uint4 *>(sg)[base + 64 * k] : uint4{0, 0, 0, 0};
#pragma unroll
                        for (int k = 0; k < 4; ++k)
                            if (base + 64 * k < nv) {
                                reinterpret_cast<uint4 *>(etile)[base + 64 * k] = v4[k];
                                if (!ROLL) reinterpret_cast<uint4 *>(gg)[base + 64 * k] = v4[k];
                            }
                    }
                } else if (((HWB | etile_addr | (uint32_t)reinterpret_cast<uintptr_t>(sg) | (uint32_t)reinterpret_cast<uintptr_t>(gg)) & 3u) == 0) {
                    const int nd = HWB / 4;
                    uint32_t v[4];
#pragma unroll
                    for (int k = 0; k < 4; ++k) v[k] = (lane + 64 * k < nd) ? reinterpret_cast<const uint32_t *>(sg)[lane + 64 * k] : 0u;
#pragma unroll
                    for (int k = 0; k < 4; ++k)
                        if (lane + 64 * k < nd) {
                            reinterpret_cast<uint32_t *>(etile)[lane + 64 * k] = v[k];
                            if (!ROLL) reinterpret_cast<uint32_t *>(gg)[lane + 64 * k] = v[k];
                        }
#pragma unroll 4
                    for (int i = lane + 256; i < nd; i += 64) {
                        const uint32_t w = reinterpret_cast<const uint32_t *>(sg)[i];
                        reinterpret_cast<uint32_t *>(etile)[i] = w;
                        if (!ROLL) reinterpret_cast<uint32_t *>(gg)[i] = w;
                    }
                } else {
                    for (int i = lane; i < HWB; i += 64) {
                        const uint8_t w = sg[i];
                        etile[i] = w;
                        if (!ROLL) gg[i] = w;
                    }
                }
                if (lane < A) rows[e * A + lane] = nrow;
                if (lane == 0) {
                    scnt[e] = 0;
                    if (HOOKS) {
                        auxl[e] = naux;
                        if (!ROLL) reinterpret_cast<uint4 *>(MGX_LATE(aux))[b] = naux;
                    }
                }
            }
            wave_sync();
            if (!ROLL && lane < Gc && ((reset_mask >> lane) & 1ull)) in_scnt = 0;
        }
    }
    if (AR && reset_mask != 0 && lane < NVc) cur_row = rows[lane];
    double my_rew = 0.0;
    if (DO_STEP && !MGX_DBG(2)) {
        const bool in = lane < NVc;
        int32_t *const p_step_count = ROLL ? nullptr : MGX_LATE(step_count);
        uint8_t *const p_truncated = MGX_LATE(truncated);
        MGX_MARK("P1a");
        if (ROLL && A > 1 && !MGX_DBG(128)) {
            if (in) {
                const int e = env_of_lane, ai = agent_of_lane;
                uint64_t s_lo, s_hi;
                rnd[lane] = pcg64_draw_at(rngs + e * 4, jump + ai * 4, s_lo, s_hi);
                if (ai == A - 1) { rngs[e * 4 + 0] = s_lo; rngs[e * 4 + 1] = s_hi; }
            }
        }
        MGX_MARK("P1s");
        int32_t *woff = reinterpret_cast<int32_t *>(L + cv.woff());
        AgentEval ev{};
        uint8_t *mytile = tile + env_of_lane * TSB;
        if (in) MGX_CHECK_LDS_PTR(2, mytile, TSB);
        if (in && !MGX_DBG(64)) {
            const int so = (env_kind == MGX_KIND_REDBLUEDOORS)
                               ? stale_offset(cf, reinterpret_cast<const uint8_t *>(auxl + env_of_lane), env_kind) : -1;
            ev = eval_agent(cf, mytile, rows + env_of_lane * A, ROLL ? (int)acts[lane] : (int)(int8_t)in_act, cur_row, true, so);
        }
        bool conf = false;
        MGX_SPAN_FLAG(8, __builtin_amdgcn_ballot_w64(in && ev.writes) != 0);
        const bool any_writes = __builtin_amdgcn_ballot_w64(in && ev.writes) != 0;
        if (any_writes) {
            if (in) woff[lane] = ev.writes ? ev.off : -1;
            wave_sync();
            conf = in && spec_cell_conflict(woff + env_of_lane * A, A, agent_of_lane, ev);
        }
        bool fb = false, does_act = in;
        uint64_t m_ends = 0, m_evt = 0, genv = 0;
        if (__builtin_amdgcn_ballot_w64(in && (ev.bad | conf | ev.used_presence | ev.success | ev.failure)) != 0) {
            MGX_RARE_PATH_PRIO();
            const uint64_t m_bad = __builtin_amdgcn_ballot_w64(in && ev.bad);
            const uint64_t m_conf = __builtin_amdgcn_ballot_w64(conf);
            const uint64_t m_pres = __builtin_amdgcn_ballot_w64(in && ev.used_presence);
            const uint64_t m_moved = __builtin_amdgcn_ballot_w64(in && ev.moved);
            m_ends = __builtin_amdgcn_ballot_w64(in && event_ends_all(cf, ev));
            m_evt = __builtin_amdgcn_ballot_w64(in && (ev.success | ev.failure));
            const uint64_t amask = (A >= 64) ? ~0ull : ((1ull << A) - 1ull);
            genv = in ? (amask << (env_of_lane * A)) : 0ull;
            fb = in && spec_needs_fallback(m_bad & genv, m_conf & genv, m_pres & genv, m_moved & genv);
            does_act = in && !fb;
            const uint64_t m_fb = __builtin_amdgcn_ballot_w64(fb);
            if (A > 1 && (m_ends | m_fb) != 0) {
                int my_rank = 0;
                if (in) {
                    my_rank = draw_rank(rnd + env_of_lane * A, A, agent_of_lane);
                    ord[env_of_lane * A + my_rank] = (uint8_t)agent_of_lane;
                }
                wave_sync();
                if (in && (m_ends & genv) != 0)
                    does_act = does_act && my_rank <= event_cutoff(ord + env_of_lane * A, (m_ends & genv) >> (env_of_lane * A), A);
                if constexpr (PREFIX) {
                    if (m_fb != 0 && A > 2) {
                        const bool block = fb && prefix_blocked(ev, my_rank, ord + env_of_lane * A, woff + env_of_lane * A, any_writes,
                                                                (m_moved & genv) >> (env_of_lane * A), A);
                        wave_sync();
                        if (block) ord[env_of_lane * A + my_rank] = (uint8_t)(agent_of_lane | 0x40);
                        wave_sync();
                        bool prefix_ok = fb;
                        if (fb)
                            for (int k = 0; k < my_rank; ++k) prefix_ok &= (ord[env_of_lane * A + k] & 0x40) == 0;
                        prefix_ok = prefix_ok && !block;
                        wave_sync();
                        if (in) ord[env_of_lane * A + my_rank] = (uint8_t)(agent_of_lane | (prefix_ok ? 0x80 : 0));
                        does_act = does_act || prefix_ok;
                    }
                }
                if (!PREFIX || A <= 2) {
                    const bool first_ok = fb && my_rank == 0 && !(ev.bad | ev.success | ev.failure);
                    if (first_ok) ord[env_of_lane * A] = (uint8_t)(agent_of_lane | 0x80);
                    does_act = does_act || first_ok;
                }
            }
        }
        if (does_act) {
            if (ev.go) { rows[lane] = ev.nrow; cur_row = ev.nrow; }
            if (ev.unstale) reinterpret_cast<uint8_t *>(auxl + env_of_lane)[4] = 0;
            if (ev.writes) {
                store_cell(CB, mytile + ev.off, ev.ncell);
                if (!ROLL) {
                    if constexpr (B3) store_obs_cell(MGX_LATE(grid) + (e0 + env_of_lane) * (int64_t)HWG + (ev.off >> 1) * 3, ev.ncell);
                    else store_cell(CB, MGX_LATE(grid) + (e0 + env_of_lane) * HWB + ev.off, ev.ncell);
                }
            }
        }
        if (m_evt != 0) {
            const uint64_t m_succ = __builtin_amdgcn_ballot_w64(does_act && ev.success);
            if (in && !fb) {
                if (cf.joint_reward ? (m_succ & genv) != 0 : (does_act && ev.success))
                    my_rew = reward_value(scnt[env_of_lane] + 1, cf.max_steps);
                if ((does_act && event_ends_self(cf, ev)) || (m_ends & genv) != 0) {
                    cur_row |= 1ull << 32;
                    rows[lane] = cur_row;
                }
            }
        }
        MGX_MARK("P1s_end");
        const uint64_t fbw = __builtin_amdgcn_ballot_w64(fb);
        MGX_SPAN_FLAG(2, fbw != 0);
        MGX_SPAN_FLAG(4, m_evt != 0);
        wave_sync();
        if (fbw != 0) {
            const bool mine = lane < Gc && (lane * A < 64) && ((fbw >> (lane * A)) & 1ull);
            if (mine) {
                const int e = lane;
                const int64_t b = e0 + e;
                uint8_t *etile = tile + e * TSB;
                uint8_t *ggrid = MGX_LATE(grid) + b * HWG;
                auto dirty = [=](int off) {
                    if constexpr (B3) store_obs_cell(ggrid + (off >> 1) * 3, cell_unpack_full(load_cell16(etile + off)));
                    else if (!ROLL) store_cell_raw(CB, ggrid + off, load_cell_raw(CB, etile + off));
                };
                int k0 = 0;
                if constexpr (PREFIX) { if (A > 1) while (k0 < A && (ord[e * A + k0] & 0x80)) ++k0; }
                else k0 = (A > 1 && (ord[e * A] & 0x80)) ? 1 : 0;
                const int rc = handle_actions(cf, etile, rows + e * A, acts + e * A, ord + e * A, rew + e * A,
                                              scnt[e] + 1, dirty, reinterpret_cast<uint8_t *>(auxl + e), env_kind, k0);
                int32_t *errp = MGX_LATE(err);
                if (rc != 0 && errp) { atomicAdd(errp, 1); atomicMin(errp + 1, (int32_t)min(b, (int64_t)INT_MAX)); }
            }
            wave_sync();
        }
        MGX_MARK("P1hook");
        const int ovl = (in && !MGX_DBG(512)) ? overlay_offset(cf, rows + env_of_lane * A, agent_of_lane) : -1;
        if (HOOKS && in && !fb) rew[lane] = my_rew;
        const uint8_t *const p_hord = HOOKS ? MGX_LATE(hook_order) : nullptr;
        if (HOOKS && p_hord && in) ord[lane] = ROLL ? p_hord[tv0 + lane] : in_hord;
        wave_sync();
        if (lane < Gc) {
            const int e = lane;
            const int64_t b = e0 + e;
            const int32_t sc = (ROLL ? scnt[e] : (int32_t)in_scnt) + 1;
            if (ROLL) scnt[e] = sc; else p_step_count[b] = sc;
            uint8_t *etile = tile + e * TSB;
            uint8_t *ggrid = MGX_LATE(grid) + b * HWG;
            auto dirty = [=](int off) {
                if constexpr (B3) store_obs_cell(ggrid + (off >> 1) * 3, cell_unpack_full(load_cell16(etile + off)));
                else if (!ROLL) store_cell_raw(CB, ggrid + off, load_cell_raw(CB, etile + off));
            };
            uint8_t *eaux = reinterpret_cast<uint8_t *>(auxl + e);
            post_step_hook(cf, env_kind, etile, rows + e * A, acts + e * A, eaux, sc, rew + e * A, dirty, p_hord ? ord + e * A : nullptr);
            if (!ROLL && cv.has_aux) {
                uint8_t *gaux = MGX_LATE(aux) + b * MGX_AUX_BYTES;
                if (env_kind == MGX_KIND_LOCKEDHALLWAY) { gaux[1] = eaux[1]; gaux[2] = eaux[2]; gaux[15] = eaux[15]; }
                if (env_kind == MGX_KIND_REDBLUEDOORS) gaux[4] = eaux[4];
            }
            MGX_PUB_STORE_U8(p_truncated + tb0 + e0, e, Gc, sc >= cf.max_steps);
        }
        wave_sync();
        if ((HOOKS || fbw != 0) && in) {
            cur_row = rows[lane];
            if (HOOKS || fb) my_rew = rew[lane];
        }
        if (ROLL && ovl >= 0) ovl_saved = load_cell_raw(CB, mytile + ovl);
        ovl_off = ovl;
        wave_sync();
        if (ovl >= 0) {
            MGX_CHECK_LDS_PTR(3, mytile + ovl, CB);
            store_cell_raw(CB, mytile + ovl, agent_cell_raw(CB, cur_row));
        }
    } else {
        const int off = (lane < NVc) ? overlay_offset(cf, rows + env_of_lane * A, agent_of_lane) : -1;
        wave_sync();
        if (off >= 0) store_cell_raw(CB, tile + env_of_lane * TSB + off, agent_cell_raw(CB, cur_row));
    }
    wave_sync();

    MGX_MARK("P1d");
    const uint32_t tile_addr = (uint32_t)(wave * wave_lds_ + cv.tile(sl_s) + tile_skew);
    uint32_t my_carry = 0;
    uint8_t *const p_dir = MGX_LATE(dir);
    uint8_t *const p_agents = DO_STEP ? MGX_LATE(agents) : nullptr;
    double *const p_reward = DO_STEP ? MGX_LATE(reward) : nullptr;
    uint8_t *const p_term = DO_STEP ? MGX_LATE(terminated) : nullptr;
    if (lane < NVc) {
        const int e = env_of_lane;
        const uint64_t row = cur_row;
        const ViewGeom g = view_geom<V>(W, H, row_x(row), row_y(row), row_dir(row), CB, PITCH);
        const ViewClamp vc = view_clamp<V>(g, W, H, row_x(row), row_y(row));
        ViewRec r;
        r.origin = vc.valid ? (int32_t)tile_addr + e * TSB + g.origin : (int32_t)wall_addr;
        r.steps = vc.valid ? vc.steps : 0u; r.lo = vc.valid ? vc.lo : 0u; r.hi = vc.valid ? vc.hi : 0u;
        my_carry = row_carry(row) & kCellShown;
        rec[lane] = r;
        if (DO_STEP) {
            const u32x2 rowv = {(uint32_t)row, (uint32_t)(row >> 32)};
            if (!ROLL) __builtin_amdgcn_raw_buffer_store_b64(rowv, make_rsrc(p_agents + v0 * 8, NVc * 8), lane * 8, 0, kSmallOutAux);
            const uint64_t rbits = __builtin_bit_cast(uint64_t, my_rew);
            const u32x2 rewv = {(uint32_t)rbits, (uint32_t)(rbits >> 32)};
            __builtin_amdgcn_raw_buffer_store_b64(rewv, make_rsrc(p_reward + tv0, NVc * 8), lane * 8, 0, kOutAux);
            const bool forced = env_kind == MGX_KIND_LOCKEDHALLWAY && reinterpret_cast<const uint8_t *>(auxl + e)[15];
            __builtin_amdgcn_raw_buffer_store_b8((uint8_t)(row_term(row) | forced),
                                                 make_rsrc(p_term + tv0, NVc), lane, 0, kOutAux);
        }
        if (p_dir) __builtin_amdgcn_raw_buffer_store_b8((uint8_t)row_dir(row), make_rsrc(p_dir + tv0, NVc), lane, 0, kOutAux);
    } else if (lane < ((NVc + kG - 1) & ~(kG - 1))) {
        ViewRec r;
        r.origin = (int32_t)wall_addr; r.steps = 0; r.lo = 0; r.hi = 0;
        rec[lane] = r;
    }
    wave_sync();

    if constexpr (GEN && MODE == 1) {
        const uint64_t alive_now = __builtin_amdgcn_ballot_w64(lane < NVc && !row_term(cur_row));
        if (lane < Gc) {
            const uint64_t amask = (A >= 64) ? ~0ull : ((1ull << A) - 1ull);
            done_now = (((alive_now >> mad24(lane, A, 0)) & amask) == 0) | ((int32_t)in_scnt + 1 >= cf.max_steps);
            uint8_t *wr = MGX_LATE(was_reset);
            if (wr) wr[e0 + lane] = (uint8_t)done_now;
        }
        done_mask = __builtin_amdgcn_ballot_w64(done_now);
        if (stage_tag && cand_K > 0) {
            const bool dn = done_now;
            if (done_mask != 0) {
                cand_r = cand_draw(cand_npr);
                const int r = cand_r;
                const int32_t tr = (int32_t)(r == 0 ? in_tags.x : r == 1 ? in_tags.y : r == 2 ? in_tags.z : in_tags.w);
                cand_mask = __builtin_amdgcn_ballot_w64(dn && tr == (int32_t)in_ep);
                if (cand_mask != 0 && (HWB & 3) == 0 && HWB <= 1024) {
                    pre_e = __builtin_ctzll(cand_mask);
                    const int64_t s = (e0 + pre_e) * cand_K + __builtin_amdgcn_readlane(r, pre_e);
// ... 618 lines not shown
```

### multigrid_amd/csrc/mgx_kernels.hip

```cpp
#include <algorithm>
#include <cstdlib>
#include <mutex>
#include <vector>

#include "mgx_fused.h"
#include "mgx_host.h"

#if MGX_SINGLE_TU
#define MGX_INST_V 3
#include "mgx_fused_inst.hip"
#define MGX_INST_V 5
#include "mgx_fused_inst.hip"
#define MGX_INST_V 7
#include "mgx_fused_inst.hip"
#define MGX_INST_V 9
#include "mgx_fused_inst.hip"
#define MGX_INST_V 11
#include "mgx_fused_inst.hip"
#define MGX_INST_V 13
#include "mgx_fused_inst.hip"
#define MGX_INST_V 15
#include "mgx_fused_inst.hip"
#endif

// ... 103 lines not shown
    if (batch <= 16384) return 0;
    if (persist) return batch <= 32768 ? kShapeResident1 : kShapeResident2;
    if (batch <= 49152) return kShapeResident1;
    return batch <= 65536 ? kShapeResident4 : kShapeResident1;
}

int plan_launch(LaunchPlan &lp, const MgxSpec &sp, int64_t batch, LaunchForm form) {
    KernelArgs &ka = lp.ka;
    lp.form = form;
    ka.sp = sp;
    ka.batch = batch;
    ka.Gw = g_debug_G > 0 ? g_debug_G : choose_Gw(sp, batch, form);
    const int max_gw = form_slots(sp, form) / sp.num_agents;
    if (ka.Gw > max_gw) ka.Gw = max_gw;
    if (ka.Gw < 1) ka.Gw = 1;
    while (ka.Gw > 1 && wave_lds_bytes(sp, ka.Gw, form, kGroup) > kLdsPerCU) --ka.Gw;
    ka.grp = kGroup;
    if (form.plain_step() && has_small_groups(sp.view_size, form.family, form.one_hot, form.generate) && sp.num_agents <= 8
        && sp.cell_bytes != 1 && sp.cell_bytes != 3) {
        const int g = g_debug_grp > 0 ? g_debug_grp : (g_debug_G > 0 ? kGroup : choose_group(sp, batch));
        if (g < kGroup && sp.num_agents <= g) { ka.grp = g; ka.Gw = g / sp.num_agents; }
    }
    ka.dbg = g_debug_skip;
    ka.flags = (batch * (int64_t)sp.width * sp.height * grid_cell_bytes_of(sp) > (int64_t)128 << 20) ? 1 : 0;
    ka.vpw = slots_in_use(sp, ka.Gw, form, ka.grp);
    ka.inv_A = (65536 + sp.num_agents - 1) / sp.num_agents;
    ka.wave_lds = wave_lds_bytes(sp, ka.Gw, form, ka.grp);
    ka.ns = 0; ka.rshape = 0;
    if (form.roll() && !form.one_hot && !MGX_NO_FIXED_SHAPES && g_debug_G <= 0) {
        const int rs = resident_shape(sp, batch, form.persist());
        if (rs > 0) {
            const FixedShape &f = kShapes[rs];
            ka.ns = f.ns; ka.rshape = rs; ka.Gw = f.Gw; ka.vpw = shape_slots(f);
            ka.wave_lds = shape_carve(f, true).total();
        }
    }
    int wpb = ((batch + ka.Gw - 1) / ka.Gw >= 16384) ? ((ka.wave_lds > 8192 && !form.one_hot && !form.obs_only()) ? 1 : 2) : 4;
    if (ka.ns > 0) wpb = ka.rshape == kShapeResident4 ? 4 : 2;
    while (wpb > 1 && wpb * ka.wave_lds > 64 * 1024) wpb >>= 1;
    if (g_debug_wpb > 0) wpb = g_debug_wpb;
    lp.threads = 64 * wpb;
    lp.lds_bytes = wpb * ka.wave_lds;
    const int64_t nwaves = lp.wavefronts();
    if ((nwaves <= 2048 || ka.grp < kGroup) && !(ka.flags & 1) && ka.Gw * sp.num_agents <= kSlotsLatency && sp.cell_bytes != 1
        && sp.cell_bytes != 3)
        ka.flags |= 2;
    if (!(ka.flags & 2) && ka.grp < kGroup) return MGX_ERR_UNSUPPORTED;
    lp.nwg = lp.workgroups_for(nwaves);
    if (lp.nwg > INT_MAX) return MGX_ERR_UNSUPPORTED;
    return MGX_OK;
}

int check_step_pointers(const MgxSpec &sp, const MgxStepArgs &sa, LaunchForm form) {
    if (!sa.grid || !sa.agents || !sa.step_count || (!sa.actions && !form.persist()) || !sa.obs || !sa.reward || !sa.terminated || !sa.truncated)
        return MGX_ERR_INVALID_ARGUMENT;
    if (sp.num_agents > 1 && !sa.rng) return MGX_ERR_INVALID_ARGUMENT;
    if (sp.env_kind != MGX_KIND_EMPTY && !sa.aux) return MGX_ERR_INVALID_ARGUMENT;
    if (misaligned(sa.grid, 16) || misaligned(sa.agents, 8) || misaligned(sa.obs, 16) || misaligned(sa.rng, 8)
        || misaligned(sa.reward, 8) || misaligned(sa.step_count, 4) || misaligned(sa.err, 4) || misaligned(sa.aux, 16))
        return MGX_ERR_INVALID_ARGUMENT;
    return MGX_OK;
}

void bind_step_pointers(KernelArgs &ka, const MgxStepArgs &sa, LaunchForm form) {
    ka.grid = reinterpret_cast<uint8_t *>(sa.grid); ka.agents = sa.agents; ka.rng = sa.rng; ka.step_count = sa.step_count;
    if (!form.persist()) { ka.actions = sa.actions; ka.hook_order = sa.hook_order; }
    ka.aux = sa.aux; ka.obs = sa.obs; ka.dir = sa.dir; ka.reward = sa.reward; ka.terminated = sa.terminated;
    ka.truncated = sa.truncated; ka.err = sa.err;
}

int check_auto_reset(const MgxSpec &sp, const MgxAutoReset &ar) {
    if (ar.pool_size < 1 || ar.first_env < 0 || !ar.pool_grid || !ar.pool_agents || !ar.episode) return MGX_ERR_INVALID_ARGUMENT;
    if (sp.env_kind != MGX_KIND_EMPTY && !ar.pool_aux) return MGX_ERR_INVALID_ARGUMENT;
    if (misaligned(ar.pool_agents, 8) || misaligned(ar.pool_aux, 16) || misaligned(ar.episode, 4)) return MGX_ERR_INVALID_ARGUMENT;
    return MGX_OK;
}

void bind_auto_reset(KernelArgs &ka, const MgxSpec *spec, const MgxAutoReset &ar, const int *occupancy = nullptr) {
    ka.pool_size = ar.pool_size; ka.first_env = ar.first_env;
    ka.pool_magic = ar.pool_size > 1 ? ~0ull / (uint64_t)ar.pool_size + 1ull : 0ull;
    ka.pool_grid = reinterpret_cast<const uint8_t *>(ar.pool_grid);
    ka.pool_agents = ar.pool_agents; ka.pool_aux = ar.pool_aux; ka.episode = ar.episode; ka.was_reset = ar.was_reset;
    if (occupancy && !ka.pool_grid) ka.pool_grid = reinterpret_cast<const uint8_t *>(spec);
}

bool stage_present(const MgxSpec &sp, const MgxGenStage &st) {
    return st.grid && st.agents && st.words && st.tag && (st.aux || sp.env_kind == MGX_KIND_EMPTY) && sp.num_agents > 1;
}
bool stage_misaligned(const MgxGenStage &st) {
    return misaligned(st.grid, 4) || misaligned(st.agents, 8) || misaligned(st.aux, 16) || misaligned(st.words, 8) || misaligned(st.tag, 16);
}
bool stage_fits(const LaunchPlan &lp) { return lp.ka.wave_lds >= 128 * lp.ka.sp.num_agents; }
bool stage_candidates_ok(const MgxLayoutGen *gen) {
    const MgxGenStage &st = gen->stage;
    return st.candidates == 0 || (st.candidates > 0 && st.external == 2 && st.candidates == mgx_gen::stage_candidates(gen));
}
int check_generator(const MgxSpec *spec, const MgxLayoutGen *gen) {
    if (spec->width > 254 || spec->height > 254) return MGX_ERR_UNSUPPORTED;
    return mgx_gen::check_layout_gen(spec, gen);
}

int device_cu_count(int &cus) {
    int dev = 0;
    hipDeviceProp_t prop;
    hipError_t e = hipGetDevice(&dev);
    if (e == hipSuccess) e = hipGetDeviceProperties(&prop, dev);
    if (e != hipSuccess) return hip_failed(e);
    cus = prop.multiProcessorCount > 0 ? prop.multiProcessorCount : 1;
    return MGX_OK;
}

struct JitNode { mgx_fused::JitShape s; int device; JitNode *next; };
std::mutex g_jit_mutex;
JitNode *g_jit_head = nullptr;

}

namespace mgx_fused {
const JitShape *jit_shape_lookup(const KernelArgs &ka, bool hooks) {
    if (!g_jit_head) return nullptr;
    int dev = 0;
    if (hipGetDevice(&dev) != hipSuccess) return nullptr;
    std::lock_guard<std::mutex> lock(g_jit_mutex);
    for (const JitNode *n = g_jit_head; n; n = n->next) {
        const FixedShape &f = n->s.f;
        if (n->device == dev && ka.sp.view_size == f.V && ((ka.flags & 2) != 0) == f.dma && ((ka.flags & 1) != 0) == f.stream
            && ka.sp.width == f.W && ka.sp.height == f.H && ka.sp.num_agents == f.A && ka.Gw == f.Gw && hooks == f.hooks
            && ka.vpw == n->s.vpw && ka.wave_lds == n->s.wave_lds && ka.grp == kGroup)
            return &n->s;
    }
    return nullptr;
}
}

extern "C" int mgx_internal_stage_candidates(const MgxSpec *spec, int64_t batch, const MgxLayoutGen *gen, const int32_t *episode,
                                             void *stream);

extern "C" {

int mgx_abi_version(void) {
#if MGX_BOUNDS_CHECK
    if (!g_bounds) {
        int32_t *p = nullptr;
        if (hipMalloc(reinterpret_cast<void **>(&p), 8) == hipSuccess) {
            if (hipMemset(p, 0, 8) == hipSuccess) g_bounds = p; else (void)hipFree(p);
        }
        (void)hipGetLastError();
    }
#endif
    return MGX_ABI_VERSION;
}

const char *mgx_error_string(int code) {
    switch (code) {
    case MGX_OK: return "ok";
    case MGX_ERR_INVALID_ARGUMENT: return "invalid argument";
    case MGX_ERR_UNKNOWN_ACTION: return "unknown action";
    case MGX_ERR_UNSUPPORTED: return "configuration outside compiled limits";
    case MGX_ERR_LAUNCH: return "HIP kernel launch failed";
    default: return "unknown error";
    }
}

int mgx_last_hip_error(void) { return g_last_hip_error; }

#if MGX_DEBUG_KNOBS
// ... 83 lines not shown

int mgx_shape_key(const MgxSpec *spec, int64_t batch, MgxShapeKey *key) {
    const LaunchForm form = LaunchForm::step();
    int rc = check_spec(spec, batch, form);
    if (rc) return rc;
    if (!key || batch < 1) return MGX_ERR_INVALID_ARGUMENT;
    if (spec->cell_bytes == 1 || spec->cell_bytes == 3) return MGX_ERR_UNSUPPORTED;
    LaunchPlan lp;
    rc = plan_launch(lp, *spec, batch, form);
    if (rc) return rc;
    const KernelArgs &ka = lp.ka;
    const bool hooks = spec->env_kind != MGX_KIND_EMPTY;
    key->width = spec->width; key->height = spec->height; key->num_agents = spec->num_agents; key->envs_per_wavefront = ka.Gw;
    key->hooks = hooks ? 1 : 0; key->view_size = spec->view_size; key->dma = (ka.flags & 2) ? 1 : 0; key->stream = (ka.flags & 1) ? 1 : 0;
    key->kernel_args_bytes = (int32_t)sizeof(KernelArgs);
    key->built_in = match_fixed_shape(ka, hooks);
    key->registered = jit_shape_lookup(ka, hooks) ? 1 : 0;
    return MGX_OK;
}

int mgx_shape_register(const MgxShapeKey *key, const void *code_object, size_t bytes) {
    if (!key || !code_object || bytes == 0) return MGX_ERR_INVALID_ARGUMENT;
    if (key->kernel_args_bytes != (int32_t)sizeof(KernelArgs)) return MGX_ERR_INVALID_ARGUMENT;
    if (key->view_size < 3 || key->view_size > MGX_MAX_VIEW || !(key->view_size & 1) || key->num_agents < 1
        || key->num_agents > MGX_MAX_AGENTS || key->envs_per_wavefront < 1)
        return MGX_ERR_INVALID_ARGUMENT;
    JitShape js{};
    js.f = FixedShape{key->width, key->height, key->num_agents, key->envs_per_wavefront, key->hooks != 0, key->view_size, key->dma != 0,
                      key->stream != 0};
    js.vpw = shape_slots(js.f);
    js.wave_lds = make_carve(js.f.W, js.f.H, js.f.A, js.f.V, js.f.Gw, js.vpw, false, js.f.hooks, false, kGroup).total();
    int dev = 0;
    hipModule_t mod = nullptr;
    hipError_t e = hipGetDevice(&dev);
    if (e == hipSuccess) e = hipModuleLoadData(&mod, code_object);
    if (e == hipSuccess) e = hipModuleGetFunction(&js.fn[0], mod, "mgx_jit_step");
    if (e == hipSuccess) e = hipModuleGetFunction(&js.fn[1], mod, "mgx_jit_step_ar");
    int32_t *d_size = nullptr; size_t gbytes = 0; int32_t built_for = 0;
    if (e == hipSuccess) e = hipModuleGetGlobal(reinterpret_cast<hipDeviceptr_t *>(&d_size), &gbytes, mod, "mgx_jit_kernel_args_bytes");
    if (e == hipSuccess) e = hipMemcpy(&built_for, d_size, sizeof built_for, hipMemcpyDeviceToHost);
    if (e != hipSuccess) {
        if (mod) (void)hipModuleUnload(mod);
        return hip_failed(e);
    }
    if (built_for != (int32_t)sizeof(KernelArgs)) { (void)hipModuleUnload(mod); return MGX_ERR_INVALID_ARGUMENT; }
    if (js.wave_lds * 4 > 64 * 1024)
        for (int k = 0; k < 2; ++k)
            (void)hipFuncSetAttribute(reinterpret_cast<const void *>(js.fn[k]), hipFuncAttributeMaxDynamicSharedMemorySize, 160 * 1024);
    std::lock_guard<std::mutex> lock(g_jit_mutex);
    g_jit_head = new JitNode{js, dev, g_jit_head};
    return MGX_OK;
}

static int gen_obs_common(bool one_hot, const MgxSpec *spec, int64_t batch, const MgxCell *grid, const uint8_t *agents,
                          uint8_t *obs, uint8_t *dir, void *stream) {
    const LaunchForm form = LaunchForm::gen_obs().with_one_hot(one_hot);
    int rc = check_spec(spec, batch, form);
    if (rc) return rc;
    if (batch == 0) return MGX_OK;
    if (!grid || !agents || !obs) return MGX_ERR_INVALID_ARGUMENT;
    if (misaligned(grid, 16) || misaligned(agents, 8) || misaligned(obs, 16)) return MGX_ERR_INVALID_ARGUMENT;
    LaunchPlan lp;
    rc = plan_launch(lp, *spec, batch, form);
    if (rc) return rc;
    KernelArgs &ka = lp.ka;
    ka.grid = reinterpret_cast<uint8_t *>(const_cast<MgxCell *>(grid));
    ka.agents = const_cast<uint8_t *>(agents);
    ka.obs = obs;
    ka.dir = dir;
    ka.T = 1;
    return launch(lp, static_cast<hipStream_t>(stream));
}

int mgx_gen_obs(const MgxSpec *spec, int64_t batch, const MgxCell *grid, const uint8_t *agents,
                uint8_t *obs, uint8_t *dir, void *stream) {
    return gen_obs_common(false, spec, batch, grid, agents, obs, dir, stream);
}

int mgx_gen_obs_one_hot(const MgxSpec *spec, int64_t batch, const MgxCell *grid, const uint8_t *agents,
                        uint8_t *obs_one_hot, uint8_t *dir, void *stream) {
    return gen_obs_common(true, spec, batch, grid, agents, obs_one_hot, dir, stream);
}

static int step_common(const MgxSpec *spec, int64_t batch, const MgxStepArgs &sa, void *stream, int *occupancy = nullptr) {
    const bool roll = sa.steps != 1, one_hot = sa.one_hot != 0;
    const MgxAutoReset *ar = sa.auto_reset;
    const MgxLayoutGen *gen = sa.generate;
    const LaunchForm form = roll ? LaunchForm::rollout().with_one_hot(one_hot)
                                 : LaunchForm::step().with_one_hot(one_hot).with_generate(gen != nullptr);
    int rc = check_spec(spec, batch, form);
    if (rc) return rc;
    if (sa.steps < 0) return MGX_ERR_INVALID_ARGUMENT;
    if (batch == 0 || sa.steps == 0) return MGX_OK;
    if (!occupancy) {
        rc = check_step_pointers(*spec, sa, form);
        if (!rc && ar) rc = check_auto_reset(*spec, *ar);
        if (rc) return rc;
    }
    LaunchPlan lp;
    rc = plan_launch(lp, *spec, batch, form);
    if (rc) return rc;
    KernelArgs &ka = lp.ka;
    if (ar) bind_auto_reset(ka, spec, *ar, occupancy);
    bind_step_pointers(ka, sa, form);
    ka.grid_bad = spec->cell_bytes == 3 ? sa.grid_bad : nullptr;
    if (misaligned(ka.grid_bad, 4)) return MGX_ERR_INVALID_ARGUMENT;
    ka.T = roll ? sa.steps : 1;
    if (gen) {
        if (ar) return MGX_ERR_INVALID_ARGUMENT;
        if (spec->cell_bytes == 1 || spec->cell_bytes == 3) return MGX_ERR_UNSUPPORTED;
        if (roll) {
            if (occupancy) { MgxStepArgs one = sa; one.steps = 1; return step_common(spec, batch, one, stream, occupancy); }
            const int64_t BA = batch * spec->num_agents, V2 = (int64_t)spec->view_size * spec->view_size * (one_hot ? 21 : 3);
            MgxLayoutGen gen_t = *gen;
            if (gen_t.stage.external) gen_t.stage.external = 2;
            for (int32_t t = 0; t < sa.steps; ++t) {
                MgxStepArgs one = sa;
                one.steps = 1;
                gen_t.stage.phase = gen->stage.phase + t;
                one.generate = &gen_t;
                one.actions = sa.actions + t * BA;
                one.hook_order = sa.hook_order ? sa.hook_order + t * BA : nullptr;
                one.obs = sa.obs + t * BA * V2;
                one.dir = sa.dir ? sa.dir + t * BA : nullptr;
                one.reward = sa.reward + t * BA;
                one.terminated = sa.terminated + t * BA;
                one.truncated = sa.truncated + t * batch;
                one.was_reset = sa.was_reset ? sa.was_reset + t * batch : nullptr;
                rc = step_common(spec, batch, one, stream, nullptr);
                if (rc) return rc;
                if (gen->stage.external && gen->stage.tag) {
                    const int every = gen->stage.lead >= 4 ? gen->stage.lead / 2 : 1;
                    if ((gen_t.stage.phase + 1) % every == 0) {
                        rc = mgx_stage_generate(spec, batch, &gen_t, sa.rng, sa.episode, stream);
                        if (rc) return rc;
                    }
                }
            }
            return MGX_OK;
        }
        if (!occupancy) {
            if (!gen->blank || !gen->gen_state || !sa.episode || !sa.rng) return MGX_ERR_INVALID_ARGUMENT;
            if (misaligned(gen->gen_state, 8) || misaligned(sa.episode, 4)) return MGX_ERR_INVALID_ARGUMENT;
        }
        rc = check_generator(spec, gen);
        if (rc) return rc;
        ka.gen = *gen; ka.episode = sa.episode; ka.was_reset = sa.was_reset;
        ka.gen_first_wg = INT64_MAX;
        MgxGenStage &st = ka.gen.stage;
        if (stage_present(*spec, st) && stage_fits(lp)) {
            if (stage_misaligned(st) || !stage_candidates_ok(gen)) return MGX_ERR_INVALID_ARGUMENT;
            if (st.lead < 0 || st.lead >= spec->max_steps) return MGX_ERR_INVALID_ARGUMENT;
            if (st.lead < 2) st.lead = 2;
            if (st.external < 0 || st.external > 2) return MGX_ERR_INVALID_ARGUMENT;
            if (!st.external) {
                ka.gen_first_wg = lp.nwg;
                lp.nwg += lp.workgroups_for((batch + 63) / 64);
                if (lp.nwg > INT_MAX) return MGX_ERR_UNSUPPORTED;
            }
        } else {
            st = MgxGenStage{};
        }
    }
    return launch(lp, static_cast<hipStream_t>(stream), occupancy);
}

static MgxStepArgs step_args(MgxCell *grid, uint8_t *agents, uint64_t *rng, int32_t *step_count, const int8_t *actions,
                             uint8_t *aux, uint8_t *obs, uint8_t *dir, double *reward, uint8_t *terminated, uint8_t *truncated,
                             int32_t *err) {
    MgxStepArgs sa{};
    sa.grid = grid; sa.agents = agents; sa.rng = rng; sa.step_count = step_count; sa.aux = aux; sa.actions = actions;
    sa.obs = obs; sa.dir = dir; sa.reward = reward; sa.terminated = terminated; sa.truncated = truncated; sa.err = err;
    sa.steps = 1;
    return sa;
}

int mgx_step_ex(const MgxSpec *spec, int64_t batch, const MgxStepArgs *args, void *stream) {
    if (!args) return MGX_ERR_INVALID_ARGUMENT;
    return step_common(spec, batch, *args, stream);
}

int mgx_step(const MgxSpec *spec, int64_t batch, MgxCell *grid, uint8_t *agents, uint64_t *rng,
             int32_t *step_count, const int8_t *actions, uint8_t *aux,
             uint8_t *obs, uint8_t *dir, double *reward, uint8_t *terminated, uint8_t *truncated,
             int32_t *err, void *stream) {
    return step_common(spec, batch, step_args(grid, agents, rng, step_count, actions, aux, obs, dir, reward, terminated, truncated, err), stream);
}

int mgx_rollout(const MgxSpec *spec, int64_t batch, int32_t steps, MgxCell *grid, uint8_t *agents, uint64_t *rng,
                int32_t *step_count, const int8_t *actions, uint8_t *aux,
                uint8_t *obs, uint8_t *dir, double *reward, uint8_t *terminated, uint8_t *truncated,
                int32_t *err, void *stream) {
    MgxStepArgs sa = step_args(grid, agents, rng, step_count, actions, aux, obs, dir, reward, terminated, truncated, err);
    if (steps == 0) return check_spec(spec, batch, LaunchForm::rollout());
    if (steps < 0) return MGX_ERR_INVALID_ARGUMENT;
    if (steps == 1) return step_common(spec, batch, sa, stream);
    sa.steps = steps;
    return step_common(spec, batch, sa, stream);
}

int mgx_step_autoreset(const MgxSpec *spec, int64_t batch, const MgxAutoReset *ar, MgxCell *grid, uint8_t *agents,
                       uint64_t *rng, int32_t *step_count, const int8_t *actions, uint8_t *aux,
                       uint8_t *obs, uint8_t *dir, double *reward, uint8_t *terminated, uint8_t *truncated,
                       int32_t *err, void *stream) {
    if (!ar) return MGX_ERR_INVALID_ARGUMENT;
    MgxStepArgs sa = step_args(grid, agents, rng, step_count, actions, aux, obs, dir, reward, terminated, truncated, err);
    sa.auto_reset = ar;
    return step_common(spec, batch, sa, stream);
}

int mgx_rollout_autoreset(const MgxSpec *spec, int64_t batch, int32_t steps, const MgxAutoReset *ar, MgxCell *grid,
                          uint8_t *agents, uint64_t *rng, int32_t *step_count, const int8_t *actions, uint8_t *aux,
                          uint8_t *obs, uint8_t *dir, double *reward, uint8_t *terminated, uint8_t *truncated,
                          int32_t *err, void *stream) {
    if (!ar || steps < 0) return MGX_ERR_INVALID_ARGUMENT;
    MgxStepArgs sa = step_args(grid, agents, rng, step_count, actions, aux, obs, dir, reward, terminated, truncated, err);
    sa.auto_reset = ar;
    if (steps == 0) return check_spec(spec, batch, LaunchForm::rollout());
    sa.steps = steps;
    return step_common(spec, batch, sa, stream);
}

int mgx_step_one_hot(const MgxSpec *spec, int64_t batch, const MgxAutoReset *ar, MgxCell *grid, uint8_t *agents,
                     uint64_t *rng, int32_t *step_count, const int8_t *actions, uint8_t *aux,
                     uint8_t *obs_one_hot, uint8_t *dir, double *reward, uint8_t *terminated, uint8_t *truncated,
                     int32_t *err, void *stream) {
    MgxStepArgs sa = step_args(grid, agents, rng, step_count, actions, aux, obs_one_hot, dir, reward, terminated, truncated, err);
    sa.auto_reset = ar; sa.one_hot = 1;
    return step_common(spec, batch, sa, stream);
}

int mgx_stage_generate(const MgxSpec *spec, int64_t batch, const MgxLayoutGen *gen, const uint64_t *rng, const int32_t *episode,
                       void *stream) {
    const LaunchForm form = LaunchForm::step().with_generate();
    int rc = check_spec(spec, batch, form);
    if (rc) return rc;
    if (batch == 0) return MGX_OK;
    if (spec->cell_bytes == 1 || spec->cell_bytes == 3) return MGX_ERR_UNSUPPORTED;
    if (!gen || !rng || !episode || !gen->blank || !gen->gen_state || !stage_present(*spec, gen->stage)) return MGX_ERR_INVALID_ARGUMENT;
    if (stage_misaligned(gen->stage) || misaligned(gen->gen_state, 8) || misaligned(rng, 8) || misaligned(episode, 4))
        return MGX_ERR_INVALID_ARGUMENT;
    rc = check_generator(spec, gen);
    if (rc) return rc;
    LaunchPlan lp;
    rc = plan_launch(lp, *spec, batch, form);
    if (rc) return rc;
    if (!stage_fits(lp)) return MGX_ERR_UNSUPPORTED;
    if (!stage_candidates_ok(gen)) return MGX_ERR_INVALID_ARGUMENT;
    if (gen->stage.candidates > 0) return mgx_internal_stage_candidates(spec, batch, gen, episode, stream);
    KernelArgs &ka = lp.ka;
    ka.rng = const_cast<uint64_t *>(rng);
    ka.episode = const_cast<int32_t *>(episode);
    ka.gen = *gen;
    ka.gen.stage.phase = -2;
    ka.gen.stage.lead = ka.gen.stage.lead < 2 ? 2 : ka.gen.stage.lead;
    ka.gen_first_wg = 0;
    ka.T = 1;
    lp.nwg = lp.workgroups_for((batch + 63) / 64);
    if (lp.nwg > INT_MAX) return MGX_ERR_UNSUPPORTED;
    return launch(lp, static_cast<hipStream_t>(stream));
}

int mgx_step_generate(const MgxSpec *spec, int64_t batch, const MgxLayoutGen *gen, MgxCell *grid, uint8_t *agents,
                      uint64_t *rng, int32_t *step_count, const int8_t *actions, uint8_t *aux,
// ... 166 lines not shown
```

### multigrid_amd/ops.py

```python
from __future__ import annotations

import ctypes as C
import os

import torch

from . import _lib
from .spec import EnvSpec, MgxSpecC

_SPEC_FIELDS = [n for n, _ in MgxSpecC._fields_]


def spec_to_ints(spec: EnvSpec) -> list[int]:
    c = spec.to_c()
    return [int(getattr(c, n)) for n in _SPEC_FIELDS]


_raw_stream = getattr(torch._C, "_cuda_getCurrentRawStream", None)
_cur_device = getattr(torch._C, "_cuda_getDevice", None) or torch.cuda.current_device


def _stream(device) -> int:
    if _raw_stream is not None:
        index = device.index
# ... 64 lines not shown

    name = "hip"

    def __init__(self, spec: EnvSpec, device):
        device = torch.device(device)
        if device.type != "cuda":
            raise RuntimeError(
                f"multigrid_amd runs on MI355X only: device must be a HIP ('cuda') device, got '{device}'. "
                "There is no CPU fallback.")
        if not torch.cuda.is_available():
            raise RuntimeError("multigrid_amd: no HIP device is visible (torch.cuda.is_available() is False)")
        _lib.lib()
        self.spec = spec
        self.sc = spec.to_c()
        self.device = device

    def gen_obs(self, B, grid, agents, obs, dirs, one_hot: bool = False):
        _gen_obs_into(self.sc, B, grid, agents, obs, dirs, one_hot)

    @staticmethod
    def _auto_reset_struct(auto_reset):
        first_env, (pg, pa, pt), episode, was_reset = auto_reset
        return _lib.MgxAutoReset(first_env, pg.shape[0], pg.data_ptr(), pa.data_ptr(),
                                 pt.data_ptr() if pt is not None else None, episode.data_ptr(),
                                 was_reset.data_ptr() if was_reset is not None else None)

    def step(self, B, grid, agents, rng, step_count, actions, target, err, obs, dirs, reward, terminated, truncated,
             auto_reset=None, one_hot: bool = False):
        if auto_reset is None and not one_hot:
            _step_into(self.sc, B, grid, agents, rng, step_count, actions, target, err, obs, dirs, reward,
                       terminated, truncated)
            return
        ar = self._auto_reset_struct(auto_reset) if auto_reset is not None else None
        fn = _lib.lib().mgx_step_one_hot if one_hot else _lib.lib().mgx_step_autoreset
        with torch.cuda.device(grid.device):
            rc = fn(
                C.byref(self.sc), B, C.byref(ar) if ar is not None else None, grid.data_ptr(), agents.data_ptr(),
                rng.data_ptr() if rng is not None else None, step_count.data_ptr(), actions.data_ptr(),
                target.data_ptr() if target is not None else None, obs.data_ptr(), dirs.data_ptr(), reward.data_ptr(),
                terminated.data_ptr(), truncated.data_ptr(), err.data_ptr() if err is not None else None,
                _stream(grid.device))
        _lib.check(rc, "mgx_step_one_hot" if one_hot else "mgx_step_autoreset")

    @staticmethod
    def _layout_gen_struct(gen):
        sx, sy, sd = gen.get("start", (0, 0, 0))
        g = _lib.MgxLayoutGen(_lib.GEN_KINDS[gen["kind"]], int(gen.get("room_size", 0)), int(sx), int(sy), int(sd),
                              int(gen.get("max_hallway_keys", 1)), int(gen.get("max_keys_per_room", 2)),
                              gen["blank"].data_ptr(), gen["gen_state"].data_ptr())
        st = gen.get("stage")
        if st is not None:
            g.stage = _lib.MgxGenStage(st["grid"].data_ptr(), st["agents"].data_ptr(), _ptr(st.get("aux")), st["words"].data_ptr(),
                                       st["tag"].data_ptr(), int(st["phase"][0]), int(st.get("lead", 2)), int(st.get("external") or 0),
                                       int(st.get("candidates") or 0))
        return g

    def step_args(self, grid, agents, rng, step_count, target, err, obs, dirs, reward, terminated, truncated,
                  auto_reset=None, one_hot: bool = False, generate=None):
        ar = self._auto_reset_struct(auto_reset) if auto_reset is not None else None
        sa = _lib.MgxStepArgs()
        sa.grid, sa.agents, sa.rng, sa.step_count = grid.data_ptr(), agents.data_ptr(), _ptr(rng), step_count.data_ptr()
        sa.aux, sa.err = _ptr(target), _ptr(err)
        sa.obs, sa.dir, sa.reward = obs.data_ptr(), _ptr(dirs), reward.data_ptr()
        sa.terminated, sa.truncated = terminated.data_ptr(), truncated.data_ptr()
        sa.steps, sa.one_hot = 1, int(bool(one_hot))
        if self.spec.cell_bytes == 3:
            sa.grid_bad = self.grid_bad().data_ptr()
        gen = None
        if ar is not None:
            sa.auto_reset = C.pointer(ar)
        if generate is not None:
            gd, episode, was_reset = generate
            gen = self._layout_gen_struct(gd)
            sa.generate = C.pointer(gen)
            sa.episode, sa.was_reset = episode.data_ptr(), _ptr(was_reset)
        return sa, (ar, gen, self.sc)

    def grid_bad(self):
        if getattr(self, "_grid_bad", None) is None:
            self._grid_bad = torch.zeros(2, dtype=torch.int32, device=self.device)
        return self._grid_bad

    def bind_step(self, B, grid, agents, rng, step_count, target, err, obs, dirs, reward, terminated, truncated,
                  auto_reset=None, one_hot: bool = False, generate=None):
        fn = _lib.lib().mgx_step_ex
        sa, keep = self.step_args(grid, agents, rng, step_count, target, err, obs, dirs, reward, terminated, truncated,
                                  auto_reset, one_hot, generate)
        spec_ref, args_ref = C.byref(self.sc), C.byref(sa)
        dev, index = grid.device, grid.device.index
        device_ctx = torch.cuda.device

        gen_c = keep[1]
        stage = generate[0].get("stage") if generate is not None else None
        phase = stage["phase"] if stage is not None else None
        side = stage is not None and bool(stage.get("external"))
        if side:
            gen_stream, every = stage["stream"], max(1, int(stage.get("lead", 2)) // 2)
            stage_fn, gen_ref = _lib.lib().mgx_stage_generate, C.byref(gen_c)
            rng_ptr, episode_ptr = rng.data_ptr(), generate[1].data_ptr()

        def step(actions, hook_order=None):
            sa.actions = actions.data_ptr()
            sa.hook_order = hook_order.data_ptr() if hook_order is not None else None
            if phase is not None:
                gen_c.stage.phase = phase[0]
                phase[0] = (phase[0] + 1) & 0x3fffffff
            if _cur_device() == index:
                rc = fn(spec_ref, B, args_ref, _stream(dev))
            else:
                with device_ctx(dev):
                    rc = fn(spec_ref, B, args_ref, _stream(dev))
            if rc:
                _lib.check(rc, "mgx_step_ex")
            if side and phase[0] % every == 0:
                if gen_stream is not None:
                    gen_stream.wait_stream(torch.cuda.current_stream(dev))
                    handle = gen_stream.cuda_stream
                else:
                    handle = _stream(dev)
                with device_ctx(dev):
                    rc = stage_fn(spec_ref, B, gen_ref, rng_ptr, episode_ptr, handle)
                if rc:
                    _lib.check(rc, "mgx_stage_generate")
                stage["launches"] = stage.get("launches", 0) + 1
        step._keep = (sa, keep)
        return step

    def stage_generate(self, B, gen, rng, episode):
        gen_c = self._layout_gen_struct(gen)
        with torch.cuda.device(rng.device):
            rc = _lib.lib().mgx_stage_generate(C.byref(self.sc), B, C.byref(gen_c), rng.data_ptr(), episode.data_ptr(), _stream(rng.device))
        _lib.check(rc, "mgx_stage_generate")
        gen["stage"]["launches"] = gen["stage"].get("launches", 0) + 1

    def bind_chains(self, B, parts, streams, grid, agents, rng, step_count, target, err, obs, dirs, reward, terminated,
                    truncated, auto_reset=None, one_hot: bool = False, generate=None):
        fn = _lib.lib().mgx_step_chains
        sa, keep = self.step_args(grid, agents, rng, step_count, target, err, obs, dirs, reward, terminated, truncated,
                                  auto_reset, one_hot, generate)
        spec_ref, args_ref = C.byref(self.sc), C.byref(sa)
        handles = (C.c_void_p * parts)(*[s.cuda_stream for s in streams])
        dev = grid.device

        gen_c = keep[1]
        phase = generate[0]["stage"]["phase"] if generate is not None and generate[0].get("stage") is not None else None
        cand = phase is not None and bool(gen_c.stage.candidates)
        if cand:
            stage = generate[0]["stage"]
            every = max(1, int(stage.get("lead", 2)) // 2)
            stage_fn, gen_ref = _lib.lib().mgx_stage_generate, C.byref(gen_c)
            rng_ptr, episode_ptr = rng.data_ptr(), generate[1].data_ptr()
        if phase is not None and not cand and gen_c.stage.external:
            gen_c.stage.external = 0

        def step(actions, fork_event, hook_order=None):
            sa.actions = actions.data_ptr()
            sa.hook_order = hook_order.data_ptr() if hook_order is not None else None
            if phase is not None:
                gen_c.stage.phase = phase[0]
                phase[0] = (phase[0] + 1) & 0x3fffffff
            with torch.cuda.device(dev):
                rc = fn(spec_ref, B, args_ref, parts, handles, fork_event)
                if rc:
                    _lib.check(rc, "mgx_step_chains")
                if cand and phase[0] % every == 0:
                    for s in streams[1:]:
                        streams[0].wait_stream(s)
                    rc = stage_fn(spec_ref, B, gen_ref, rng_ptr, episode_ptr, handles[0])
                    if rc:
                        _lib.check(rc, "mgx_stage_generate")
                    for s in streams[1:]:
                        s.wait_stream(streams[0])
                    stage["launches"] = stage.get("launches", 0) + 1
        step._keep = (sa, keep, handles, streams)
        return step

    def sub_shards(self, B, auto_reset: bool = False, one_hot: bool = False, generate: bool = False) -> int:
        sa = _lib.MgxStepArgs()
        sa.steps, sa.one_hot = 1, int(bool(one_hot))
        ar = _lib.MgxAutoReset()
        if auto_reset and not generate:
            sa.auto_reset = C.pointer(ar)
        out = C.c_int32(1)
        with torch.cuda.device(self.device):
            rc = _lib.lib().mgx_sub_shards(C.byref(self.sc), B, C.byref(sa), C.byref(out))
        _lib.check(rc, "mgx_sub_shards")
        return int(out.value)

    def rollout(self, B, T, grid, agents, rng, step_count, actions, target, err, obs, dirs, reward, terminated,
                truncated, auto_reset=None, one_hot: bool = False, generate=None):
        sa, keep = self.step_args(grid, agents, rng, step_count, target, err, obs, dirs, reward, terminated, truncated,
                                  auto_reset, one_hot, generate)
        sa.steps = T
        sa.actions = actions.data_ptr()
        with torch.cuda.device(grid.device):
            rc = _lib.lib().mgx_step_ex(C.byref(self.sc), B, C.byref(sa), _stream(grid.device))
        _lib.check(rc, "mgx_rollout")
        if generate is not None and generate[0].get("stage") is not None:
            ph = generate[0]["stage"]["phase"]
            ph[0] = (ph[0] + T) & 0x3fffffff

    def persistent_waves(self, B, auto_reset: bool = False) -> int:
        sa = _lib.MgxStepArgs()
        sa.steps = 1
        ar = _lib.MgxAutoReset()
        if auto_reset:
            sa.auto_reset = C.pointer(ar)
        out = C.c_int32(0)
# ... 104 lines not shown
```

Measured before the change: 16.09 billion.

## Track pristine pool-layout grids and load tiles from the shared layout

Adds a per-env marker that records when an env's grid still equals the single auto-reset pool layout. With that marker set, the step kernel loads the tile from the shared pool grid, broadcasting one 16-byte vector, instead of streaming each env's own grid from memory. The marker is cleared whenever the kernel writes a dirty cell, and the host disarms it whenever `cells` is exposed or an untracked path runs. This aims to cut global grid read traffic. The cost is extra marker bookkeeping and writes, plus correctness risk if any path mutates the grid without invalidating the marker.

```diff
diff --git a/include/mgx.h b/include/mgx.h
--- a/include/mgx.h
+++ b/include/mgx.h
@@ -213,6 +213,8 @@
 
 int mgx_step_ex(const MgxSpec *spec, int64_t batch, const MgxStepArgs *args, void *stream);
 
+int mgx_step_tracked(const MgxSpec *spec, int64_t batch, const MgxStepArgs *args, int32_t *grid_layout, void *stream);
+
 int mgx_step_chains(const MgxSpec *spec, int64_t batch, const MgxStepArgs *args, int32_t parts, void *const *streams,
                     void *fork_event);
 int mgx_sub_shards(const MgxSpec *spec, int64_t batch, const MgxStepArgs *args, int32_t *parts);
diff --git a/multigrid_amd/_lib.py b/multigrid_amd/_lib.py
--- a/multigrid_amd/_lib.py
+++ b/multigrid_amd/_lib.py
@@ -20,7 +20,7 @@
            "mgx_launch_info", "mgx_one_hot", "mgx_full_obs", "mgx_reset_done", "mgx_rollout", "mgx_step_autoreset",
            "mgx_rollout_autoreset", "mgx_gen_obs_one_hot", "mgx_step_one_hot",
            "mgx_reset_generate", "mgx_step_generate", "mgx_pack_grid", "mgx_unpack_grid",
-           "mgx_step_ex", "mgx_step_chains", "mgx_sub_shards",
+           "mgx_step_ex", "mgx_step_tracked", "mgx_step_chains", "mgx_sub_shards",
            "mgx_pack_grid_env", "mgx_check_grid", "mgx_pack_grid8_env", "mgx_unpack_grid8", "mgx_shape_key", "mgx_shape_register", "mgx_stage_generate",
            "mgx_persistent_waves", "mgx_step_persistent", "mgx_persistent_post", "mgx_persistent_wait", "mgx_persistent_feed",
            "mgx_rollout_info", "mgx_render_atlas", "mgx_render", "mgx_reset_select", "mgx_reset_generate_select")
@@ -145,6 +145,9 @@
     L.mgx_launch_info.argtypes = [C.POINTER(MgxSpecC), i64, C.POINTER(MgxLaunchInfo)]
     L.mgx_step_ex.restype = C.c_int
     L.mgx_step_ex.argtypes = [C.POINTER(MgxSpecC), i64, C.POINTER(MgxStepArgs), vp]
+    if is_product_lib() or hasattr(L, "mgx_step_tracked"):
+        L.mgx_step_tracked.restype = C.c_int
+        L.mgx_step_tracked.argtypes = [C.POINTER(MgxSpecC), i64, C.POINTER(MgxStepArgs), vp, vp]
     L.mgx_step_chains.restype = C.c_int
     L.mgx_step_chains.argtypes = [C.POINTER(MgxSpecC), i64, C.POINTER(MgxStepArgs), C.c_int32, C.POINTER(vp), vp]
     L.mgx_sub_shards.restype = C.c_int
diff --git a/multigrid_amd/batched.py b/multigrid_amd/batched.py
--- a/multigrid_amd/batched.py
+++ b/multigrid_amd/batched.py
@@ -23,6 +23,8 @@
         if self.env._layout_version != self._version:
             raise RuntimeError("this graph was captured before set_layout_pool() / set_layout_generator() replaced the layout "
                                "tensors it holds pointers to: capture_steps() again")
+        if not getattr(self, "_tracked", False):
+            self.env._disarm()
         self.graph.replay()
 
 
@@ -47,7 +49,7 @@
         self.waited = 0
         self.open = False
         ar = env._auto_reset_args(self.auto_reset, getattr(env, "was_reset", None))
-        self._sa, self._keep = be.step_args(env.cells, env.agents, env.rng, env.step_count,
+        self._sa, self._keep = be.step_args(env._cells, env.agents, env.rng, env.step_count,
                                             env.aux if env.spec.env_kind != "empty" else None, env.err, env.obs, env.dir,
                                             env.reward, env.terminated, env.truncated, auto_reset=ar)
         self._pers = be.persistent_struct(self.granules, self.done, self.ctrl, self.max_steps, self.timeout_ms)
@@ -58,6 +60,7 @@
         env.join()
         if env._session is not None:
             raise RuntimeError("this env already has a persistent session open")
+        env._disarm()
         cur = torch.cuda.current_stream(env.device)
         self.stream.wait_stream(cur)
         env.backend.persistent_launch(env.batch, self._sa, self._pers, self.stream.cuda_stream)
@@ -69,9 +72,9 @@
         env = self.env
         if not self.open or self.t >= self.max_steps:
             raise RuntimeError("the persistent session is closed or has used up its max_steps")
-        if actions.dtype is not torch.int8 or actions.shape != env._act_shape or actions.device != env.cells.device \
+        if actions.dtype is not torch.int8 or actions.shape != env._act_shape or actions.device != env._cells.device \
                 or not actions.is_contiguous():
-            raise ValueError(f"actions must be a contiguous int8 tensor of shape {tuple(env._act_shape)} on {env.cells.device}")
+            raise ValueError(f"actions must be a contiguous int8 tensor of shape {tuple(env._act_shape)} on {env._cells.device}")
         self.t += 1
         env.backend.persistent_post(env.batch, actions, self.t, self.granules)
 
@@ -142,7 +145,9 @@
             backend = HipBackend(spec, self.device)
         self.backend = backend
         B, A, dev = self.batch, spec.num_agents, self.device
-        self.cells = torch.zeros(spec.cells_shape(B), dtype=torch.uint8 if spec.cell_bytes != 2 else torch.int16, device=dev)
+        self._cells = torch.zeros(spec.cells_shape(B), dtype=torch.uint8 if spec.cell_bytes != 2 else torch.int16, device=dev)
+        self._marker = torch.full((B,), -1, dtype=torch.int32, device=dev)
+        self._mark = {"armed": False, "graphs": False, "root": self._marker}
         self.agents = torch.zeros(spec.agents_shape(B), dtype=torch.uint8, device=dev)
         self.rng = torch.zeros((B, 4), dtype=torch.int64, device=dev)
         self.step_count = torch.zeros((B,), dtype=torch.int32, device=dev)
@@ -181,10 +186,47 @@
         return self.shape_kernel
 
     @property
+    def cells(self) -> torch.Tensor:
+        self._disarm()
+        return self._cells
+
+    def _tracks(self) -> bool:
+        return getattr(self, "_pool", None) is not None and getattr(self, "_gen", None) is None and self.spec.cell_bytes == 2
+
+    def _disarm(self):
+        m = self._mark
+        if m["armed"]:
+            m["root"].fill_(-1)
+            if not m["graphs"] and not (self.device.type == "cuda" and torch.cuda.is_current_stream_capturing()):
+                m["armed"] = False
+
+    def _tracked_step(self):
+        m = self._mark
+        if not m["graphs"]:
+            m["armed"] = True
+            if torch.cuda.is_current_stream_capturing():
+                m["graphs"] = True
+
+    def _arm(self):
+        if not self._tracks() or self._pool[0].shape[0] != 1:
+            self._disarm()
+            return
+        same = (self._cells == self._pool[0][0]).flatten(1).all(dim=1)
+        self._marker.copy_(same.to(torch.int32) - 1)
+        self._mark["armed"] = True
+
+    def _restarted(self):
+        if self._tracks() and (self._mark["armed"] or self._pool[0].shape[0] == 1):
+            one = self._pool[0].shape[0] == 1
+            self._marker.masked_fill_(self.was_reset.bool(), 0 if one else -1)
+            if one:
+                self._mark["armed"] = True
+
+    @property
     def grid(self) -> torch.Tensor:
         if self.spec.cell_bytes == 3:
-            return self.cells
-        c = self.cells.to(torch.int32)
+            return self._cells
+        c = self._cells.to(torch.int32)
         if self.spec.cell_bytes == 1:
             tc = c & 0xF
             door = (tc == 11) | (tc == 12)
@@ -215,7 +257,8 @@
             if (an[..., 2] >= sp.width).any() or (an[..., 3] >= sp.height).any() or (an[..., 1] > 3).any():
                 raise ValueError("agent position / direction out of range")
         self._refuse_carried_contents(a)
-        self.cells.copy_(torch.from_numpy(layouts.pack_cells_for(sp, g.cpu().numpy())))
+        self._cells.copy_(torch.from_numpy(layouts.pack_cells_for(sp, g.cpu().numpy())))
+        self._arm()
         self.agents.copy_(a)
         if rng is not None:
             r = np.asarray(rng.cpu() if torch.is_tensor(rng) else rng)
@@ -278,13 +321,13 @@
         self.join()
         if one_hot:
             if self.spec.cell_bytes == 1:
-                self.backend.gen_obs(self.batch, self.cells, self.agents, self.obs, self.dir)
+                self.backend.gen_obs(self.batch, self._cells, self.agents, self.obs, self.dir)
                 self.backend.one_hot(self.obs, self._one_hot_buffer())
                 return self._one_hot, self.dir
             self._need_wide_cells("one-hot output")
-            self.backend.gen_obs(self.batch, self.cells, self.agents, self._one_hot_buffer(), self.dir, one_hot=True)
+            self.backend.gen_obs(self.batch, self._cells, self.agents, self._one_hot_buffer(), self.dir, one_hot=True)
             return self._one_hot, self.dir
-        self.backend.gen_obs(self.batch, self.cells, self.agents, self.obs, self.dir)
+        self.backend.gen_obs(self.batch, self._cells, self.agents, self.obs, self.dir)
         return self.obs, self.dir
 
     def _one_hot_buffer(self):
@@ -304,18 +347,22 @@
             self._need_state()
         if self._parent is not None:
             self._check_fresh()
-        if actions.dtype is not torch.int8 or actions.shape != self._act_shape or actions.device != self.cells.device \
+        if actions.dtype is not torch.int8 or actions.shape != self._act_shape or actions.device != self._cells.device \
                 or not actions.is_contiguous():
             raise ValueError(f"actions must be a contiguous int8 tensor of shape {tuple(self._act_shape)} "
-                             f"on {self.cells.device}")
+                             f"on {self._cells.device}")
         if sub_shards == 1 and hook_order is None and not self._chains_pending:
             fast = self._bound.get((auto_reset, one_hot))
             if fast is not None:
+                if fast[2]:
+                    self._tracked_step()
+                elif self._mark["armed"]:
+                    self._disarm()
                 fast[0](actions)
                 return fast[1]
         if hook_order is not None and (hook_order.dtype is not torch.uint8 or hook_order.shape != self._act_shape
-                                       or hook_order.device != self.cells.device or not hook_order.is_contiguous()):
-            raise ValueError(f"hook_order must be a contiguous uint8 tensor of shape {tuple(self._act_shape)} on {self.cells.device}")
+                                       or hook_order.device != self._cells.device or not hook_order.is_contiguous()):
+            raise ValueError(f"hook_order must be a contiguous uint8 tensor of shape {tuple(self._act_shape)} on {self._cells.device}")
         if one_hot and not (self.spec.cell_bytes == 1 and self.spec.env_kind == "empty"):
             self._need_wide_cells("one-hot output")
         generate = bool(auto_reset) and getattr(self, "_gen", None) is not None
@@ -334,6 +381,11 @@
         if fast is None:
             fast = self._bind_step(*key)
         out = (self._one_hot if one_hot else self.obs), self.dir, self.reward, self.terminated, self.truncated
+        tracked = fast is not False and getattr(fast, "tracked", False)
+        if tracked:
+            self._tracked_step()
+        else:
+            self._disarm()
         if fast is not False:
             if P > 1:
                 ev = self._fork_event
@@ -346,7 +398,7 @@
                 self._chains_pending, self._chains_P = True, P
                 return out
             if isinstance(auto_reset, bool) and isinstance(one_hot, bool):
-                self._bound[(auto_reset or generate, one_hot)] = (fast, out)
+                self._bound[(auto_reset or generate, one_hot)] = (fast, out, tracked)
             fast(actions, hook_order)
             return out
         sp = self.spec
@@ -359,7 +411,7 @@
         if hook_order is not None:
             kw["hook_order"] = hook_order
         obs = self._one_hot_buffer() if one_hot else self.obs
-        self.backend.step(self.batch, self.cells, self.agents, self.rng, self.step_count, actions,
+        self.backend.step(self.batch, self._cells, self.agents, self.rng, self.step_count, actions,
                           self.aux if sp.env_kind != "empty" else None, self.err,
                           obs, self.dir, self.reward, self.terminated, self.truncated, **kw)
         if generate:
@@ -399,11 +451,13 @@
                 self._fork_event = torch.cuda.Event()
                 self._fork_event.record(torch.cuda.current_stream(self.device))
             head = (self.batch, parts, self._chain_streams[:parts])
-        f = bind(*head, self.cells, self.agents, self.rng, self.step_count,
+        track = ar is not None and parts == 1 and not one_hot and not generate and self._tracks()
+        f = bind(*head, self._cells, self.agents, self.rng, self.step_count,
                  self.aux if self.spec.env_kind != "empty" else None, self.err,
                  self._one_hot_buffer() if one_hot else self.obs, self.dir, self.reward, self.terminated, self.truncated,
                  auto_reset=ar, one_hot=one_hot,
-                 **({"generate": (self._gen, self.episode, self.was_reset)} if generate else {}))
+                 **({"generate": (self._gen, self.episode, self.was_reset)} if generate else {}),
+                 **({"marker": self._marker} if track else {}))
         self._bound[key] = f
         return f
 
@@ -426,8 +480,9 @@
                 continue
             c = object.__new__(BatchedMultiGridEnv)
             c.spec, c.batch, c.first_env, c.device, c.backend = self.spec, hi - lo, self.first_env + lo, self.device, self.backend
-            for name in ("cells", "agents", "rng", "step_count", "aux", "obs", "dir", "reward", "terminated", "truncated"):
+            for name in ("_cells", "agents", "rng", "step_count", "aux", "obs", "dir", "reward", "terminated", "truncated"):
                 setattr(c, name, getattr(self, name)[lo:hi])
+            c._marker, c._mark = self._marker[lo:hi], self._mark
             c.err = self.err
             c._loaded, c._act_shape, c._bound = True, torch.Size((hi - lo, self.spec.num_agents)), {}
             c._parent, c._made_version, c._layout_version = self, self._layout_version, 0
@@ -486,7 +541,10 @@
                 for s in others:
                     side.wait_stream(s)
         stream.wait_stream(side)
-        return StepGraph(self, graph, len(shards), (shards, others, actions, hook_order))
+        sg = StepGraph(self, graph, len(shards), (shards, others, actions, hook_order))
+        ent = shards[0]._bound.get((bool(auto_reset), bool(one_hot)))
+        sg._tracked = bool(ent and ent[2])
+        return sg
 
     def rollout(self, actions: torch.Tensor, out: dict | None = None, auto_reset: bool = False, one_hot: bool = False) -> dict:
         self._need_state()
@@ -494,10 +552,11 @@
         if not (self.spec.cell_bytes == 1 and self.spec.env_kind == "empty" and not one_hot and not generate):
             self._need_wide_cells("rollout (the steps of one launch)")
         self.join()
+        self._disarm()
         sp, B = self.spec, self.batch
         if actions.dtype != torch.int8 or actions.dim() != 3 or tuple(actions.shape[1:]) != (B, sp.num_agents) \
-                or actions.device != self.cells.device or not actions.is_contiguous():
-            raise ValueError(f"actions must be a contiguous int8 tensor of shape (T, {B}, {sp.num_agents}) on {self.cells.device}")
+                or actions.device != self._cells.device or not actions.is_contiguous():
+            raise ValueError(f"actions must be a contiguous int8 tensor of shape (T, {B}, {sp.num_agents}) on {self._cells.device}")
         T, A, v, dev = actions.shape[0], sp.num_agents, sp.view_size, self.device
         if out is None:
             out = {"obs": torch.empty((T, B, A, v, v, 21 if one_hot else 3), dtype=torch.uint8, device=dev),
@@ -509,13 +568,13 @@
             out["was_reset"] = torch.empty((T, B), dtype=torch.uint8, device=dev)
         generate = bool(auto_reset) and getattr(self, "_gen", None) is not None
         if generate:
-            self.backend.rollout(B, T, self.cells, self.agents, self.rng, self.step_count, actions,
+            self.backend.rollout(B, T, self._cells, self.agents, self.rng, self.step_count, actions,
                                  self.aux if sp.env_kind != "empty" else None, self.err, out["obs"], out["dir"],
                                  out["reward"], out["terminated"], out["truncated"],
                                  generate=(self._gen, self.episode, out["was_reset"]), **({"one_hot": True} if one_hot else {}))
             return out
         ar = self._auto_reset_args(auto_reset, out.get("was_reset"))
-        self.backend.rollout(B, T, self.cells, self.agents, self.rng, self.step_count, actions,
+        self.backend.rollout(B, T, self._cells, self.agents, self.rng, self.step_count, actions,
                              self.aux if sp.env_kind != "empty" else None, self.err, out["obs"], out["dir"],
                              out["reward"], out["terminated"], out["truncated"],
                              **({"auto_reset": ar} if ar is not None else {}), **({"one_hot": True} if one_hot else {}))
@@ -533,7 +592,7 @@
             self._full = torch.zeros((self.batch, self.spec.width, self.spec.height, 3), dtype=torch.uint8,
                                      device=self.device)
         try:
-            self.backend.full_obs(self.batch, self.cells, self.agents, self._full)
+            self.backend.full_obs(self.batch, self._cells, self.agents, self._full)
         except _lib.MgxError as e:
             if e.code != _lib.ERR_UNSUPPORTED:
                 raise
@@ -553,7 +612,7 @@
         ts = int(tile_size)
         if not 1 <= ts <= 64:
             raise ValueError(f"render: tile_size must be in 1..64, got {tile_size}")
-        cells, agents = self.cells, self.agents
+        cells, agents = self._cells, self.agents
         if env_ids is not None:
             ids = torch.as_tensor(env_ids)
             if ids.dtype.is_floating_point or ids.dtype.is_complex or ids.dtype == torch.bool:
@@ -613,6 +672,7 @@
             if t is not None:
                 old[2].copy_(t)
             self.episode.zero_(); self.was_reset.zero_()
+            self._arm()
             return
         self._gen = None
         self._pool = (cells.to(self.device).contiguous(), a.to(self.device).contiguous(), t)
@@ -620,6 +680,7 @@
         self.was_reset = torch.zeros((self.batch,), dtype=torch.uint8, device=self.device)
         self._bound.clear()
         self._layout_version += 1
+        self._arm()
 
     def set_layout_generator(self, kind: str, layout_seed: int = 0, *, room_size: int = 0, start=(1, 1, 0),
                              max_hallway_keys: int = 1, max_keys_per_room: int = 2, staged=True, lead: int | None = None):
@@ -688,6 +749,7 @@
                                   "agents": torch.zeros((B, sp.num_agents, 8), dtype=torch.uint8, device=dev),
                                   "aux": torch.zeros((B, 16), dtype=torch.uint8, device=dev) if sp.env_kind != "empty" else None,
                                   "words": torch.zeros((B, 12), dtype=torch.int64, device=dev), "tag": tag, "phase": [0]}
+        self._disarm()
         self._pool = None
         self.episode = torch.zeros((self.batch,), dtype=torch.int32, device=self.device)
         self.was_reset = torch.zeros((self.batch,), dtype=torch.uint8, device=self.device)
@@ -698,13 +760,14 @@
         self._need_state()
         self.join()
         if getattr(self, "_gen", None) is not None:
-            self.backend.reset_generate(self.batch, self._gen, self.cells, self.agents, self.rng, self.step_count,
+            self.backend.reset_generate(self.batch, self._gen, self._cells, self.agents, self.rng, self.step_count,
                                         self.aux if self.spec.env_kind != "empty" else None, self.episode, self.was_reset)
             return self.was_reset
         if getattr(self, "_pool", None) is None:
             raise RuntimeError("call set_layout_pool() or set_layout_generator() first")
-        self.backend.reset_done(self.batch, self.first_env, self._pool, self.cells, self.agents, self.step_count,
+        self.backend.reset_done(self.batch, self.first_env, self._pool, self._cells, self.agents, self.step_count,
                                 self.aux, self.episode, self.was_reset)
+        self._restarted()
         return self.was_reset
 
     def reset(self, seed: int | None = None, mask: torch.Tensor | None = None, one_hot: bool = False):
@@ -716,8 +779,8 @@
         if mask is not None:
             self._need_state()
             if not torch.is_tensor(mask) or mask.dtype not in (torch.bool, torch.uint8) or tuple(mask.shape) != (self.batch,) \
-                    or mask.device != self.cells.device or not mask.is_contiguous():
-                raise ValueError(f"mask must be a contiguous bool or uint8 tensor of shape ({self.batch},) on {self.cells.device}")
+                    or mask.device != self._cells.device or not mask.is_contiguous():
+                raise ValueError(f"mask must be a contiguous bool or uint8 tensor of shape ({self.batch},) on {self._cells.device}")
             sel = mask.view(torch.uint8) if mask.dtype is torch.bool else mask
         if seed is None and not self._loaded and not self._seeded:
             raise ValueError("reset(): np_random has never been seeded (all-zero PCG64 words are not a generator): pass seed=, or "
@@ -732,11 +795,12 @@
             side = (gen.get("stage") or {}).get("stream")
             if side is not None:
                 torch.cuda.current_stream(self.device).wait_stream(side)
-            self.backend.reset_generate_select(self.batch, gen, sel, words, self.cells, self.agents, self.rng, self.step_count,
+            self.backend.reset_generate_select(self.batch, gen, sel, words, self._cells, self.agents, self.rng, self.step_count,
                                                aux, self.episode, self.was_reset)
         else:
-            self.backend.reset_select(self.batch, self.first_env, pool, sel, words, self.cells, self.agents, self.rng,
+            self.backend.reset_select(self.batch, self.first_env, pool, sel, words, self._cells, self.agents, self.rng,
                                       self.step_count, self.aux, self.episode, self.was_reset)
+            self._restarted()
         if seed is not None:
             self._seeded = True
         self._loaded = True
diff --git a/multigrid_amd/csrc/mgx_fused.h b/multigrid_amd/csrc/mgx_fused.h
--- a/multigrid_amd/csrc/mgx_fused.h
+++ b/multigrid_amd/csrc/mgx_fused.h
@@ -70,6 +70,7 @@
     int32_t *grid_bad;
     int32_t *bounds;
     int32_t span_base;
+    int32_t *grid_layout;
 };
 
 #ifndef MGX_DEBUG_KNOBS
diff --git a/multigrid_amd/csrc/mgx_fused_body.inc b/multigrid_amd/csrc/mgx_fused_body.inc
--- a/multigrid_amd/csrc/mgx_fused_body.inc
+++ b/multigrid_amd/csrc/mgx_fused_body.inc
@@ -8,6 +8,8 @@
         if constexpr (PERSIST) __builtin_amdgcn_raw_buffer_store_b8((uint8_t)(val), make_rsrc((base), (n)), (idx), 0, 16); \
         else (base)[idx] = (uint8_t)(val);                                                                           \
     } while (0)
+    constexpr bool MARK = AR && MODE == 1 && !GEN && !C8 && !B3;
+    constexpr bool MARK_RD = MARK && !DMA;
     constexpr int V2 = V * V;
     constexpr int NW = (V2 + 63) / 64;
     constexpr int CB = C8 ? 1 : kCellBytes;
@@ -45,8 +47,10 @@
         const uint8_t *e_trunc = DO_STEP ? a.truncated : nullptr;
         const uint64_t *e_gs = GEN ? a.gen.gen_state : nullptr;
         const int32_t *e_tag = GEN ? a.gen.stage.tag : nullptr;
+        const int32_t *e_lay = MARK_RD ? a.grid_layout : nullptr;
+        const uint8_t *e_pool = MARK_RD ? a.pool_grid : nullptr;
         asm volatile("" :: "s"(e_batch), "s"(e_grid), "s"(e_agents), "s"(e_rng), "s"(e_sc), "s"(e_act), "s"(e_hord), "s"(e_aux),
-                     "s"(e_bd), "s"(e_ep), "s"(e_trunc), "s"(e_gs), "s"(e_tag));
+                     "s"(e_bd), "s"(e_ep), "s"(e_trunc), "s"(e_gs), "s"(e_tag), "s"(e_lay), "s"(e_pool));
     }
     constexpr bool FIXED = SHAPE != 0;
     constexpr bool PREFIX = FIXED ? (kShapes[SHAPE].A > 4) : (V > 7 && MODE == 1);
@@ -201,10 +205,15 @@
     const __amdgpu_buffer_rsrc_t grsrc = make_rsrc(gsrc, grec);
     const int lane16 = 16 * lane;
     const int env_of_lane = (lane * inv_A_) >> 16, agent_of_lane = lane - env_of_lane * A;
+    [[maybe_unused]] const bool read_marker = MARK_RD && (a.flags & 4) != 0;
+    [[maybe_unused]] int32_t in_lay = -1;
+    if constexpr (MARK_RD) {
+        if (read_marker) in_lay = (int32_t)__builtin_amdgcn_raw_buffer_load_b32(make_rsrc(a.grid_layout + e0, Gc * 4), lane * 4, 0, 0);
+    }
     u32x4 in_rngA = {0, 0, 0, 0}, in_rngB = {0, 0, 0, 0};
     u32x4 in_jmpA = {0, 0, 0, 0}, in_jmpB = {0, 0, 0, 0};
-    if (DO_STEP && A > 1) {
-        const __amdgpu_buffer_rsrc_t rr = make_rsrc(a.rng + e0 * 4, Gc * 32);
+    if (MARK_RD || (DO_STEP && A > 1)) {
+        const __amdgpu_buffer_rsrc_t rr = make_rsrc(a.rng + e0 * 4, (MARK_RD && A <= 1) ? 0 : Gc * 32);
         if (ROLL) {
             in_rngA = __builtin_amdgcn_raw_buffer_load_b128(rr, lane16, 0,kInAux);
             for (int t = lane; t < A * 4; t += 64) jump[t] = kJump.w[1][t];
@@ -246,7 +255,29 @@
         _Pragma("unroll") for (int u = 0; u < U; ++u)                                                                 \
             dst[u] = __builtin_amdgcn_raw_buffer_load_b128(grsrc, lane16 + 1024 * (u & 3), (base) + 4096 * (u >> 2), kTileAux); \
     }
-    if constexpr (!B3 && PITCH == 0) { MGX_TILE_BURST(tv, 0) }
+    [[maybe_unused]] bool pristine = false;
+    [[maybe_unused]] __amdgpu_buffer_rsrc_t rs0 = grsrc, rs1 = grsrc;
+    [[maybe_unused]] int lane16_0 = lane16;
+    if constexpr (MARK_RD) {
+        if (read_marker) {
+            const int32_t k0 = __builtin_amdgcn_readfirstlane(in_lay);
+            pristine = k0 >= 0 && __builtin_amdgcn_ballot_w64(lane < Gc && in_lay != k0) == 0;
+            if (pristine) {
+                rs0 = make_rsrc(a.pool_grid + (int64_t)k0 * HWB, HWB);
+                rs1 = make_rsrc(gsrc, 0);
+                lane16_0 = lane16 & (HWB - 1);
+            }
+        }
+    }
+    if constexpr (!B3 && PITCH == 0) {
+        if constexpr (MARK_RD) {
+            tv[0] = __builtin_amdgcn_raw_buffer_load_b128(rs0, lane16_0, 0, kTileAux);
+            _Pragma("unroll") for (int u = 1; u < U; ++u)
+                tv[u] = __builtin_amdgcn_raw_buffer_load_b128(rs1, lane16 + 1024 * (u & 3), 4096 * (u >> 2), kTileAux);
+        } else {
+            MGX_TILE_BURST(tv, 0)
+        }
+    }
     typedef uint32_t u32x3 __attribute__((ext_vector_type(3)));
     constexpr int NR3 = 16;
     [[maybe_unused]] u32x3 w3[B3 ? NR3 : 1];
@@ -396,12 +427,21 @@
         }
     } else
     if constexpr (!DMA && PITCH == 0) {
-#pragma unroll
-        for (int u = 0; u < U; ++u)
-            if (lane16 + 1024 * u < len) {
-                MGX_CHECK_LDS_PTR(1, tile_raw + lane16 + 1024 * u, 16);
-                *reinterpret_cast<u32x4 *>(tile_raw + lane16 + 1024 * u) = tv[u];
-            }
+        if (MARK_RD && pristine) {
+#pragma unroll
+            for (int u = 0; u < U; ++u)
+                if (lane16 + 1024 * u < len) {
+                    MGX_CHECK_LDS_PTR(1, tile_raw + lane16 + 1024 * u, 16);
+                    *reinterpret_cast<u32x4 *>(tile_raw + lane16 + 1024 * u) = tv[0];
+                }
+        } else {
+#pragma unroll
+            for (int u = 0; u < U; ++u)
+                if (lane16 + 1024 * u < len) {
+                    MGX_CHECK_LDS_PTR(1, tile_raw + lane16 + 1024 * u, 16);
+                    *reinterpret_cast<u32x4 *>(tile_raw + lane16 + 1024 * u) = tv[u];
+                }
+        }
     }
     if (big_tile && !B3) {
         if constexpr (!DMA) {
@@ -641,6 +681,10 @@
                 const int lay = (int)__builtin_amdgcn_readlane(my_lay, e);
                 wave_sync();
                 if (lane == 0) p_ep[b] = ep + 1;
+                if constexpr (MARK) {
+                    int32_t *const p_lay = MGX_LATE(grid_layout);
+                    if (p_lay && lane == 0) p_lay[b] = lay;
+                }
                 const uint8_t *sg = MGX_LATE(pool_grid) + (int64_t)lay * HWG;
                 uint8_t *etile = tile + e * TSB;
                 uint8_t *gg = MGX_LATE(grid) + b * HWG;
@@ -803,6 +847,10 @@
                 if (!ROLL) {
                     if constexpr (B3) store_obs_cell(MGX_LATE(grid) + (e0 + env_of_lane) * (int64_t)HWG + (ev.off >> 1) * 3, ev.ncell);
                     else store_cell(CB, MGX_LATE(grid) + (e0 + env_of_lane) * HWB + ev.off, ev.ncell);
+                    if constexpr (MARK) {
+                        int32_t *const p_lay = MGX_LATE(grid_layout);
+                        if (p_lay) p_lay[e0 + env_of_lane] = -1;
+                    }
                 }
             }
         }
@@ -829,9 +877,11 @@
                 const int64_t b = e0 + e;
                 uint8_t *etile = tile + e * TSB;
                 uint8_t *ggrid = MGX_LATE(grid) + b * HWG;
+                [[maybe_unused]] int32_t *const p_lay = MARK ? MGX_LATE(grid_layout) : nullptr;
                 auto dirty = [=](int off) {
                     if constexpr (B3) store_obs_cell(ggrid + (off >> 1) * 3, cell_unpack_full(load_cell16(etile + off)));
                     else if (!ROLL) store_cell_raw(CB, ggrid + off, load_cell_raw(CB, etile + off));
+                    if constexpr (MARK) { if (p_lay) p_lay[b] = -1; }
                 };
                 int k0 = 0;
                 if constexpr (PREFIX) { if (A > 1) while (k0 < A && (ord[e * A + k0] & 0x80)) ++k0; }
@@ -859,6 +909,10 @@
             auto dirty = [=](int off) {
                 if constexpr (B3) store_obs_cell(ggrid + (off >> 1) * 3, cell_unpack_full(load_cell16(etile + off)));
                 else if (!ROLL) store_cell_raw(CB, ggrid + off, load_cell_raw(CB, etile + off));
+                if constexpr (MARK) {
+                    int32_t *const p_lay = MGX_LATE(grid_layout);
+                    if (p_lay) p_lay[b] = -1;
+                }
             };
             uint8_t *eaux = reinterpret_cast<uint8_t *>(auxl + e);
             post_step_hook(cf, env_kind, etile, rows + e * A, acts + e * A, eaux, sc, rew + e * A, dirty, p_hord ? ord + e * A : nullptr);
diff --git a/multigrid_amd/csrc/mgx_kernels.hip b/multigrid_amd/csrc/mgx_kernels.hip
--- a/multigrid_amd/csrc/mgx_kernels.hip
+++ b/multigrid_amd/csrc/mgx_kernels.hip
@@ -209,6 +209,15 @@
     ka.pool_grid = reinterpret_cast<const uint8_t *>(ar.pool_grid);
     ka.pool_agents = ar.pool_agents; ka.pool_aux = ar.pool_aux; ka.episode = ar.episode; ka.was_reset = ar.was_reset;
     if (occupancy && !ka.pool_grid) ka.pool_grid = reinterpret_cast<const uint8_t *>(spec);
+}
+
+void plan_marker_read(LaunchPlan &lp, const MgxAutoReset &ar, int32_t *grid_layout) {
+    KernelArgs &ka = lp.ka;
+    ka.grid_layout = grid_layout;
+    const int hwb = ka.sp.width * ka.sp.height * cell_bytes_of(ka.sp);
+    if (!(ka.flags & 2) && lp.wavefronts() > 2048 && ar.pool_size == 1 && hwb >= 16 && hwb <= 1024 && (hwb & (hwb - 1)) == 0
+        && ka.Gw * hwb <= 8192 && !misaligned(ar.pool_grid, 16))
+        ka.flags |= 4;
 }
 
 bool stage_present(const MgxSpec &sp, const MgxGenStage &st) {
@@ -458,7 +467,8 @@
     return gen_obs_common(true, spec, batch, grid, agents, obs_one_hot, dir, stream);
 }
 
-static int step_common(const MgxSpec *spec, int64_t batch, const MgxStepArgs &sa, void *stream, int *occupancy = nullptr) {
+static int step_common(const MgxSpec *spec, int64_t batch, const MgxStepArgs &sa, void *stream, int *occupancy = nullptr,
+                       int32_t *grid_layout = nullptr) {
     const bool roll = sa.steps != 1, one_hot = sa.one_hot != 0;
     const MgxAutoReset *ar = sa.auto_reset;
     const MgxLayoutGen *gen = sa.generate;
@@ -482,6 +492,11 @@
     ka.grid_bad = spec->cell_bytes == 3 ? sa.grid_bad : nullptr;
     if (misaligned(ka.grid_bad, 4)) return MGX_ERR_INVALID_ARGUMENT;
     ka.T = roll ? sa.steps : 1;
+    if (grid_layout) {
+        if (!ar || roll || gen || cell_bytes_of(*spec) != kCellBytes || spec->cell_bytes == 3) return MGX_ERR_UNSUPPORTED;
+        if (misaligned(grid_layout, 4)) return MGX_ERR_INVALID_ARGUMENT;
+        plan_marker_read(lp, *ar, grid_layout);
+    }
     if (gen) {
         if (ar) return MGX_ERR_INVALID_ARGUMENT;
         if (spec->cell_bytes == 1 || spec->cell_bytes == 3) return MGX_ERR_UNSUPPORTED;
@@ -556,6 +571,11 @@
     return step_common(spec, batch, *args, stream);
 }
 
+int mgx_step_tracked(const MgxSpec *spec, int64_t batch, const MgxStepArgs *args, int32_t *grid_layout, void *stream) {
+    if (!args) return MGX_ERR_INVALID_ARGUMENT;
+    return step_common(spec, batch, *args, stream, nullptr, grid_layout);
+}
+
 int mgx_step(const MgxSpec *spec, int64_t batch, MgxCell *grid, uint8_t *agents, uint64_t *rng,
              int32_t *step_count, const int8_t *actions, uint8_t *aux,
              uint8_t *obs, uint8_t *dir, double *reward, uint8_t *terminated, uint8_t *truncated,
diff --git a/multigrid_amd/ops.py b/multigrid_amd/ops.py
--- a/multigrid_amd/ops.py
+++ b/multigrid_amd/ops.py
@@ -170,11 +170,18 @@
         return self._grid_bad
 
     def bind_step(self, B, grid, agents, rng, step_count, target, err, obs, dirs, reward, terminated, truncated,
-                  auto_reset=None, one_hot: bool = False, generate=None):
-        fn = _lib.lib().mgx_step_ex
+                  auto_reset=None, one_hot: bool = False, generate=None, marker=None):
         sa, keep = self.step_args(grid, agents, rng, step_count, target, err, obs, dirs, reward, terminated, truncated,
                                   auto_reset, one_hot, generate)
         spec_ref, args_ref = C.byref(self.sc), C.byref(sa)
+        tracked = marker is not None and hasattr(_lib.lib(), "mgx_step_tracked")
+        if tracked:
+            tracked_fn, marker_ptr = _lib.lib().mgx_step_tracked, marker.data_ptr()
+
+            def fn(spec_ref, B, args_ref, stream):
+                return tracked_fn(spec_ref, B, args_ref, marker_ptr, stream)
+        else:
+            fn = _lib.lib().mgx_step_ex
         dev, index = grid.device, grid.device.index
         device_ctx = torch.cuda.device
 
@@ -211,7 +218,8 @@
                 if rc:
                     _lib.check(rc, "mgx_stage_generate")
                 stage["launches"] = stage.get("launches", 0) + 1
-        step._keep = (sa, keep)
+        step._keep = (sa, keep, marker)
+        step.tracked = tracked
         return step
 
     def stage_generate(self, B, gen, rng, episode):
```

After: 17.95 billion (median of 6 runs). 1.12x the previous value.
